# arnab39/equiadapt

Hardware: AMD Instinct MI355X
Metric: canonicalize+invert images/sec (224x224 C8) (higher is better)
Workload: dtype f32 (resampling / FFT / accumulation in fp32; the network's channel contraction as 2xfp16 split of every fp32 operand (within one fp32 ulp), 3 exact products, fp32 accumulate -- closer to fp64 than the fp32 matrix instruction, see step_ms_by_gemm_form); 1 GPU; configs[1]: 224x224x3 synthetic, C8, GroupEquivariantImageCanonicalization + ESCNNEquivariantNetwork in e2cnn's LAYER SHAPES (32 fields x 8 = 256 ch, k5, 3 layers, crop 0.8, resize 96) with this repository's own filter-bank parameterisation (bilinear-rotated banks; e2cnn's steerable basis is not restated -- e2cnn-trained weights enter via load_exported_dense), forward, then invert_canonicalization; batch_per_gpu=256, global_batch=256, parallelism=dp1 (no collective in the forward path)

## Files before the change

### equiadapt_amd/_lib.py

```python
import ctypes
import os
import subprocess
import threading

_HERE = os.path.dirname(os.path.abspath(__file__))
ROOT = os.path.dirname(_HERE)
CSRC = os.path.join(_HERE, "csrc")
SO_PATH = os.environ.get("EQA_LIB") or os.path.join(CSRC, "libeqa_hip.so")
SOURCES = [os.path.join(CSRC, f) for f in ("group_action.hip", "crop_resize.hip", "nearest_action.hip", "pooling.hip", "batchnorm.hip", "winograd.hip", "lift_conv.hip", "lift_conv_wide.hip", "lift_wgrad.hip", "pointcloud.hip", "vnsmall_fwd.hip", "nbody_frame.hip", "vnsmall_train.hip", "vnsmall_tail.hip", "fftconv.hip", "fft_filter.hip", "lift_fft.hip", "cgemm3m.hip", "cgemm3m_bf16.hip", "cgemm3m_c16.hip", "smallconv.hip", "planegemm.hip", "convnet_train.hip", "fourier_act.hip", "field_norm.hip", "nbody.hip", "vn_act.hip", "gconv1x1.hip", "steer_lift.hip")]
HEADERS = [os.path.join(CSRC, "eqa_common.hpp"), os.path.join(CSRC, "vn_common.hpp"), os.path.join(CSRC, "fourier_field.hpp"), os.path.join(CSRC, "fft48.inc"), os.path.join(CSRC, "fft_common.inc"), os.path.join(CSRC, "cgemm3m_common.inc")]
INCLUDE = os.path.join(ROOT, "include")

ABI_VERSION = 3

_c_f = ctypes.POINTER(ctypes.c_float)
_c_i = ctypes.POINTER(ctypes.c_int32)
_vp = ctypes.c_void_p
_int = ctypes.c_int

SIGNATURES = {
    "eqa_abi_version": (_int, []),
    "eqa_set_option": (_int, [_int, _int]),
    "eqa_get_option": (_int, [_int]),
    "eqa_fold_edge_pad_workspace_bytes": (ctypes.c_int64, [_int] * 4),
    "eqa_fold_edge_pad": (_int, [_vp, _vp, _vp, _int, _int, _int, _int, _vp]),
    "eqa_canon_transform_fwd": (_int, [_vp, _vp, _vp, _vp, _vp] + [_int] * 6 + [_vp]),
    "eqa_invert_action_fwd": (_int, [_vp, _vp, _vp, _vp, _vp, _vp] + [_int] * 6 + [_vp]),
    "eqa_group_action_pair": (_int, [_vp] * 4 + [_int, _int] + [_vp] * 5 + [_int, _int, _vp] + [_int] * 4 + [_vp]),
    "eqa_orbit_expand_fwd": (_int, [_vp, _vp, _vp, _vp] + [_int] * 5 + [_vp]),
    "eqa_group_action_fwd": (_int, [_vp, _vp, _vp, _vp, _vp, _vp] + [_int] * 12 + [_vp]),
    "eqa_group_action_fwd_hint": (_int, [_vp, _vp, _vp, _vp, _vp, _vp] + [_int] * 13 + [_vp]),
    "eqa_crop_resize_aa": (_int, [_vp] * 6 + [_int] * 9 + [_vp]),
    "eqa_mask_action_nearest": (_int, [_vp] * 5 + [_int] * 4 + [_vp]),
    "eqa_mask_action_nearest_planes": (_int, [_vp] * 5 + [_int] * 4 + [_vp]),
    "eqa_boxes_action": (_int, [_vp] * 5 + [_int, ctypes.c_float, _int, _vp]),
    "eqa_image_action_nearest": (_int, [_vp] * 5 + [_int] * 10 + [_vp]),
    "eqa_group_action_bwd_tiles": (_int, [_int, _int]),
    "eqa_group_action_bwd": (_int, [_vp] * 8 + [_int] * 12 + [_vp]),
    "eqa_group_action_bwd_theta": (_int, [_vp] * 8 + [_int] * 12 + [_vp]),
    "eqa_group_pool_workspace_bytes": (ctypes.c_int64, [_int] * 4),
    "eqa_group_pool_argmax": (_int, [_vp, _vp, _vp, _vp] + [_int] * 4 + [_vp]),
    "eqa_window_sums": (_int, [_vp, _vp, _vp, _int, _vp] + [_int] * 5 + [_vp]),
    "eqa_bn_partial_blocks": (ctypes.c_int64, [ctypes.c_int64]),
    "eqa_bn_stats_nhwc": (_int, [_vp, _vp, ctypes.c_int64, _int, _vp]),
    "eqa_bn_relu_dropout_nhwc": (_int, [_vp, _vp, _vp, _vp, ctypes.c_int64, _int, ctypes.c_float, ctypes.c_uint32, _vp]),
    "eqa_bn_bwd_reduce_nhwc": (_int, [_vp] * 5 + [ctypes.c_float, _vp, ctypes.c_int64, _int, _vp, _vp, ctypes.c_uint32, _vp]),
    "eqa_bn_bwd_apply_nhwc": (_int, [_vp] * 8 + [ctypes.c_float, _vp, ctypes.c_int64, _int, _vp, _vp, ctypes.c_uint32, _vp]),
    "eqa_window_sums_nhwc_act": (_int, [_vp, _vp, _vp, _int, ctypes.c_float, ctypes.c_uint32, _vp, _vp] + [_int] * 5 + [_vp]),
    "eqa_bn_bwd_reduce_nhwc_wsgrad": (_int, [_vp] * 4 + [ctypes.c_float, _vp] + [_int] * 5 + [_vp, _vp, ctypes.c_uint32, _vp]),
    "eqa_bn_bwd_apply_nhwc_wsgrad": (_int, [_vp] * 7 + [ctypes.c_float, _vp] + [_int] * 5 + [_vp, _vp, ctypes.c_uint32, _vp]),
    "eqa_vn_blocks": (_int, [_int]),
    "eqa_vn_knn": (_int, [_vp, _vp, _int, _int, _int, _vp]),
    "eqa_vn_convpos_stats": (_int, [_vp, _vp, _vp, _vp, _int, _int, _int, _vp]),
    "eqa_vn_convpos_fwd": (_int, [_vp] * 7 + [_int, _int, _int, _vp]),
    "eqa_vn_convpos_bwd_reduce": (_int, [_vp] * 10 + [_int, _int, _int, _vp]),
    "eqa_vn_convpos_bwd_apply": (_int, [_vp] * 12 + [_int, _int, _int, _vp]),
    "eqa_vn_convpos_max_fwd": (_int, [_vp] * 9 + [_int, _int, _int, _vp]),
    "eqa_vn_convpos_max_bwd_reduce": (_int, [_vp] * 11 + [_int, _int, _int, _vp]),
    "eqa_vn_convpos_max_bwd_apply": (_int, [_vp] * 13 + [_int, _int, _int, _vp]),
    "eqa_vn_tail_blocks": (_int, [_int]),
    "eqa_vn_tail_partial_floats": (_int, [_int]),
    "eqa_vn_tail_pass": (_int, [_int] + [_vp] * 8 + [_int, _int, _vp]),
    "eqa_vn_bn_finalize": (_int, [_vp, _int, _int, _int, ctypes.c_int64] + [_vp] * 5 + [ctypes.c_float, ctypes.c_float, _vp, _vp]),
    "eqa_vn_bn_bwd_finalize": (_int, [_vp, _int, _int, _int, ctypes.c_int64, _vp, _vp, _vp]),
    "eqa_window_grad_table": (_int, [_vp, _vp] + [_int] * 5 + [_vp]),
    "eqa_window_sums_gemv_bwd_workspace_bytes": (ctypes.c_int64, [_int, _int]),
    "eqa_window_sums_gemv_bwd": (_int, [_vp] * 6 + [_int, _int, _int, ctypes.c_double, _vp]),
    "eqa_window_sums_gemv": (_int, [_vp, _vp, _vp, _int, _int, _int, ctypes.c_double, ctypes.c_double, _vp]),
    "eqa_lift_conv_nhwc": (_int, [_vp, _vp, _vp, _int, _vp] + [_int] * 7 + [_vp]),
    "eqa_lift_conv_grouped": (_int, [_vp, _vp, _vp, _int, _vp] + [_int] * 7 + [_vp]),
    "eqa_lift_conv_stats_rows": (_int, [_int] * 7),
    "eqa_lift_conv_nhwc_stats": (_int, [_vp, _vp, _vp, _vp] + [_int] * 7 + [_vp]),
    "eqa_lift_conv_wgrad_supported": (_int, [_int] * 7),
    "eqa_lift_conv_wgrad_workspace_bytes": (ctypes.c_int64, [_int] * 7),
    "eqa_lift_conv_wgrad_nhwc": (_int, [_vp, _vp, _vp, _vp] + [_int] * 7 + [_vp]),
    "eqa_plane_gemm_supported": (_int, [_int, _int]),
    "eqa_plane_gemm": (_int, [_vp, _vp, _vp, ctypes.c_longlong, _int, _int, _int, _vp]),
    "eqa_winograd_f2k5_input": (_int, [_vp, _vp, _vp, _int, _int, _int, _int, _int, _vp]),
    "eqa_winograd_f2k5_output": (_int, [_vp, _vp, _int, _vp, _int, _int, _int, _int, _vp]),
    "eqa_winograd_f4k5_input": (_int, [_vp, _vp, _vp, _int, _int, _int, _int, _int, _vp]),
    "eqa_winograd_f4k5_output": (_int, [_vp, _vp, _int, _vp, _int, _int, _int, _int, _vp]),
    "eqa_winograd_f2k5_input_padded": (_int, [_vp, _vp, _int, _int, _int, _int, _int, _vp]),
    "eqa_winograd_f4k5_input_padded": (_int, [_vp, _vp, _int, _int, _int, _int, _int, _vp]),
    "eqa_winograd_f2k5_output_adjoint": (_int, [_vp, _vp, _int, _int, _int, _int, _vp]),
    "eqa_winograd_f4k5_output_adjoint": (_int, [_vp, _vp, _int, _int, _int, _int, _vp]),
# ... 30 lines not shown
    "eqa_fft48k5_filter_spectra3m_c16": (_int, [_vp, _vp, _int, _int, _int, _vp]),
    "eqa_fft48_filter_spectra3m_c16": (_int, [_vp, _vp, _int, _int, _int, _int, _vp]),
    "eqa_fft48_cgemm3m_c16": (_int, [_vp, _vp, _vp, ctypes.c_int64, _int, _int, _vp]),
    "eqa_fft48_wgrad3m_c16_supported": (_int, [_int, _int]),
    "eqa_fft48_wgrad3m_c16": (_int, [_vp, _vp, _vp, ctypes.c_int64, _int, _int, _vp]),
    "eqa_fft48k5_group": (_int, [_int, _int]),
    "eqa_fft48k5_workspace_bytes": (ctypes.c_int64, [_int] * 4),
    "eqa_fft48k5_input": (_int, [_vp, _vp, _vp, _vp] + [_int] * 5 + [_vp]),
    "eqa_fft48k5_input_grouped": (_int, [_vp, _vp, _vp, _vp] + [_int] * 5 + [_vp]),
    "eqa_fft48k5_input_grouped_supported": (_int, [_int]),
    "eqa_lift5_fft48k5_input_supported": (_int, [_int] * 4),
    "eqa_lift5_fft48k5_input": (_int, [_vp, _vp, _vp, _int, _vp] + [_int] * 4 + [_vp]),
    "eqa_lift5_fft48k5_input_dcmax": (_int, [_vp, _vp, _vp, _int, _vp, _vp] + [_int] * 4 + [_vp]),
    "eqa_lift5_pieces_f16_bytes": (ctypes.c_int64, [_int]),
    "eqa_absmax_slots": (_int, [_vp, ctypes.c_int64, _vp, _vp]),
    "eqa_lift5_fft48k5_input_f16x2": (_int, [_vp, _vp, ctypes.c_float, _vp, _int, _vp, _int, _vp, _vp] + [_int] * 4 + [_vp]),
    "eqa_lift5_pieces_bytes": (ctypes.c_int64, [_int]),
    "eqa_lift5_fft48k5_input_bf16x3": (_int, [_vp, _vp, _vp, _int, _vp] + [_int] * 4 + [_vp]),
    "eqa_fft48k5_output": (_int, [_vp, _vp, _vp, _int, _vp] + [_int] * 4 + [_vp]),
    "eqa_fft48k5_output_stats_rows": (ctypes.c_int64, [_int] * 4),
    "eqa_fft48k5_output_stats": (_int, [_vp, _vp, _vp, _vp] + [_int] * 4 + [_vp]),
    "eqa_fft48k5_output_sums": (_int, [_vp, _vp, _vp, _int, _vp, _vp] + [_int] * 5 + [_vp]),
    "eqa_fft48_supported": (_int, [_int]),
    "eqa_fft48_tiles": (ctypes.c_int64, [_int, _int]),
    "eqa_fft48_workspace_bytes": (ctypes.c_int64, [_int] * 5),
    "eqa_fft48_filter_spectra": (_int, [_vp, _vp, _int, _int, _int, _int, _vp]),
    "eqa_fft48_filter_spectra3m": (_int, [_vp, _vp, _int, _int, _int, _int, _vp]),
    "eqa_fft48_input": (_int, [_vp, _vp, _vp, _vp] + [_int] * 6 + [_vp]),
    "eqa_fft48_grad_transform": (_int, [_vp, _vp, _vp] + [_int] * 5 + [_vp]),
    "eqa_fft48_output": (_int, [_vp, _vp, _vp, _int, _vp] + [_int] * 5 + [_vp]),
    "eqa_fft48_input_grad": (_int, [_vp, _vp, _vp] + [_int] * 5 + [_vp]),
    "eqa_fft48_filter_grad": (_int, [_vp, _vp, _int, _int, _int, _int, _vp]),
    "eqa_conv_s2_supported": (_int, [_int] * 5),
    "eqa_conv_s2": (_int, [_vp, _vp, _vp, _int, _vp] + [_int] * 8 + [_vp]),
    "eqa_conv_s2_wgrad_supported": (_int, [_int] * 5),
    "eqa_conv_s2_wgrad_workspace_bytes": (ctypes.c_int64, [_int] * 8),
    "eqa_conv_s2_wgrad": (_int, [_vp] * 4 + [_int] * 8 + [_vp]),
    "eqa_conv_s2_dgrad_supported": (_int, [_int] * 4),
    "eqa_conv_s2_dgrad": (_int, [_vp] * 3 + [_int] * 7 + [_vp]),
    "eqa_bn_act_fwd": (_int, [_vp] * 5 + [ctypes.c_int64, _int, _int, _vp]),
    "eqa_bn_act_partial_blocks": (ctypes.c_int64, [ctypes.c_int64]),
    "eqa_bn_act_stats": (_int, [_vp, _vp, ctypes.c_int64, _int, _vp]),
    "eqa_bn_act_finalize": (_int, [_vp, ctypes.c_int64, _int, _vp, _vp, ctypes.c_double, ctypes.c_double] + [_vp] * 6 + [_vp]),
    "eqa_bn_act_bwd_finalize": (_int, [_vp, ctypes.c_int64, _int] + [_vp] * 7 + [_vp]),
    "eqa_bn_act_bwd_reduce": (_int, [_vp] * 8 + [ctypes.c_int64, _int, _int, _vp]),
    "eqa_bn_act_bwd_apply": (_int, [_vp] * 11 + [ctypes.c_int64, _int, _int, _vp]),
    "eqa_affine_relu_rows": (_int, [_vp, _vp, _vp, _vp, ctypes.c_int64, _int, _vp]),
    "eqa_cosine_group_activations": (_int, [_vp, _vp, _vp, _int, _int, _int, ctypes.c_float, _vp]),
    "eqa_bias_relu_nhwc": (_int, [_vp, _vp, ctypes.c_int64, _int, _vp]),
    "eqa_window_sums_nhwc_workspace_bytes": (ctypes.c_int64, [_int] * 4),
    "eqa_window_sums_nhwc": (_int, [_vp, _vp, _vp, _int, _vp, _vp] + [_int] * 5 + [_vp]),
    "eqa_window_sums_bwd_expand_nhwc": (_int, [_vp, _vp] + [_int] * 5 + [_vp]),
    "eqa_group_argmax": (_int, [_vp, _vp, _int, _int, _vp]),
    "eqa_vnsmall_workspace_bytes": (ctypes.c_int64, [_int, _int]),
    "eqa_vnsmall_fwd": (_int, [_vp, _vp, _vp, _vp, _int, _int, _int, _int, _vp]),
    "eqa_vnsmall_canonicalize": (_int, [_vp] * 6 + [_int] * 4 + [_vp]),
    "eqa_so3_rotate": (_int, [_vp, _vp, _vp, _int, _int, _int, _vp]),
    "eqa_gram_schmidt": (_int, [_vp, _vp, _int, _vp]),
    "eqa_gram_schmidt_bwd": (_int, [_vp, _vp, _vp, _int, _vp]),
    "eqa_modified_gram_schmidt": (_int, [_vp, _vp, _int, _vp]),
    "eqa_rigid_rows": (_int, [_vp, _vp, _vp, _vp, _int, _int, _vp]),
    "eqa_nbody_frame_fwd": (_int, [_vp] * 7 + [_int, _vp]),
    "eqa_nbody_frame_bwd": (_int, [_vp] * 12 + [_int, _vp]),
    "eqa_rigid_rows_bwd": (_int, [_vp] * 5 + [_int, _vp]),
    "eqa_fourier_elu_fwd": (_int, [_vp, _vp, _vp, _vp, ctypes.c_longlong, _int, _vp]),
    "eqa_fourier_elu_bwd": (_int, [_vp, _vp, _vp, _vp, _vp, ctypes.c_longlong, _int, _vp]),
    "eqa_field_norm_max_fields": (_int, []),
    "eqa_field_norm_blocks": (ctypes.c_longlong, [ctypes.c_longlong, _int]),
    "eqa_field_norm_stats": (_int, [_vp, _vp, ctypes.c_longlong, _int, _vp]),
    "eqa_field_norm_elu_bwd_reduce": (_int, [_vp] * 5 + [ctypes.c_longlong, _int, _vp]),
    "eqa_field_norm_elu_bwd_apply": (_int, [_vp] * 6 + [ctypes.c_longlong, _int, _vp]),
    "eqa_vndeepsets_param_count": (_int, [_int] * 3),
    "eqa_vndeepsets_bwd_blocks": (_int, [_int]),
    "eqa_nbody_adjacency": (_int, [_vp, _vp, ctypes.c_longlong, _int, _vp, _vp, _vp]),
    "eqa_vndeepsets_fwd": (_int, [_vp] * 7 + [_int] * 5 + [ctypes.c_float] + [_int] * 3 + [_vp]),
    "eqa_vndeepsets_train_fwd": (_int, [_vp] * 9 + [_int] * 5 + [ctypes.c_float] + [_int] * 3 + [_vp]),
    "eqa_vndeepsets_bwd": (_int, [_vp] * 10 + [_int] * 5 + [ctypes.c_float] + [_int] * 3 + [_vp]),
    "eqa_vn_act_max_channels": (_int, []),
    "eqa_vn_act_bwd_blocks": (_int, [ctypes.c_longlong]),
    "eqa_vn_act_fwd": (_int, [_vp] * 3 + [_int, _int, ctypes.c_longlong, _int, _int, ctypes.c_float, _vp]),
    "eqa_vn_act_bwd": (_int, [_vp] * 5 + [_int, _int, ctypes.c_longlong, _int, _int, ctypes.c_float, _vp]),
    "eqa_gconv1x1_supported": (_int, [ctypes.c_longlong, _int, _int]),
    "eqa_gconv1x1_nhwc": (_int, [_vp] * 6 + [_int, _vp, ctypes.c_longlong, _int, _int, _vp]),
    "eqa_gconv1x1_wgrad_supported": (_int, [ctypes.c_longlong, _int, _int]),
    "eqa_gconv1x1_wgrad_workspace_bytes": (ctypes.c_longlong, [ctypes.c_longlong, _int, _int]),
    "eqa_gconv1x1_wgrad": (_int, [_vp] * 5 + [ctypes.c_longlong, _int, _int, _vp]),
    "eqa_steer_lift_supported": (_int, [_int] * 3),
    "eqa_steer_lift_packed_floats": (ctypes.c_int64, [_int] * 3),
    "eqa_steer_lift_stat_rows": (ctypes.c_longlong, [_int]),
    "eqa_steer_lift_fwd": (_int, [_vp] * 4 + [_int] * 6 + [_vp]),
    "eqa_steer_lift_wgrad_workspace_bytes": (ctypes.c_int64, [_int] * 3),
    "eqa_steer_lift_wgrad": (_int, [_vp] * 4 + [_int] * 6 + [_vp]),
}

_lock = threading.Lock()
_lib = None


def source_hash(*names: str) -> str:
    import hashlib

    h = hashlib.sha1()
    for path in [os.path.join(CSRC, n) for n in names] + HEADERS:
        with open(path, "rb") as f:
            h.update(f.read())
    return h.hexdigest()[:16]
# ... 128 lines not shown
```

### equiadapt_amd/csrc/crop_resize.hip

```cpp
#include "eqa_common.hpp"

namespace {

constexpr int kAaBand = 8;
#ifndef EQA_AA_WIDE_MIN_K
#define EQA_AA_WIDE_MIN_K 8
#endif
constexpr int kAaMaxK = 20;

__global__ __launch_bounds__(kThreads) void crop_resize_aa_kernel(const float* __restrict__ x, float* __restrict__ y,
                                                                 const float* __restrict__ wx, const int32_t* __restrict__ x0,
                                                                 const float* __restrict__ wy, const int32_t* __restrict__ y0,
                                                                 int H, int W, int OH, int OW, int K, int max_rows) {
  extern __shared__ __attribute__((aligned(16))) float aa_tmp[];
  const int plane = blockIdx.y;
  const int r0 = blockIdx.x * kAaBand, r1 = min(r0 + kAaBand, OH);
  const int ybeg = y0[r0];
  const int yend = min(y0[r1 - 1] + K, H);
  const int nrows = min(yend - ybeg, max_rows);
  const float* src = x + (size_t)plane * H * W;
  const int rows_par = kThreads / OW;
  if (rows_par >= 1) {
    const int ox = threadIdx.x % OW, rsub = threadIdx.x / OW;
    if (rsub < rows_par) {
// ... 278 lines not shown
  auto wload = [&](int yc) {
    const int t = ybeg + yc + wq - ys_w;
    const bool ok = wr < nr_out && t >= 0 && t < K && yc + wq < span;
    return ok ? wy[(size_t)(r0 + wr) * K + min(max(t, 0), K - 1)] : 0.0f;
  };
  auto add8 = [&](const float4 (&v)[kAaStreamRows], float wv) {
#pragma unroll
    for (int q = 0; q < kAaStreamRows; ++q) {
#pragma unroll
      for (int r = 0; r < kAaBand; ++r) {
        const float w = __builtin_bit_cast(float, __builtin_amdgcn_readlane(__builtin_bit_cast(int, wv), 8 * q + r));
        acc[r].x += w * v[q].x; acc[r].y += w * v[q].y; acc[r].z += w * v[q].z; acc[r].w += w * v[q].w;
      }
    }
  };
  static_assert(kAaStreamRows == 8 && kAaBand == 8, "one weight per lane: 8 rows of a trip x 8 output rows = 64 lanes");
  float4 va[kAaStreamRows], vb[kAaStreamRows];
  float wa, wb = 0.0f;
  load8(va, 0);
  wa = wload(0);
  for (int yc = 0; yc < span; yc += 2 * kAaStreamRows) {
    if (yc + kAaStreamRows < span) { load8(vb, yc + kAaStreamRows); wb = wload(yc + kAaStreamRows); }
    add8(va, wa);
    if (yc + 2 * kAaStreamRows < span) { load8(va, yc + 2 * kAaStreamRows); wa = wload(yc + 2 * kAaStreamRows); }
    if (yc + kAaStreamRows < span) add8(vb, wb);
  }
  float* dst = y + (size_t)plane * OH * OW;
#pragma unroll
  for (int half = 0; half < 2; ++half) {
    if (e < xlen) {
#pragma unroll
      for (int rr = 0; rr < kAaBand / 2; ++rr) {
        float* lrow = aa_rows + rr * row_stride;
        const float4 v = acc[half * (kAaBand / 2) + rr];
        lrow[pos(e)] = v.x; lrow[pos(e + 1)] = v.y; lrow[pos(e + 2)] = v.z; lrow[pos(e + 3)] = v.w;
      }
    }
    __syncthreads();
    for (int idx = threadIdx.x; idx < (kAaBand / 2) * OW; idx += kThreads) {
      const int rr = idx / OW, ox = idx - rr * OW;
      const int r = half * (kAaBand / 2) + rr;
      if (r < nr_out) {
        const float* row = aa_rows + rr * row_stride;
        const int xs = x0[ox] - xbeg;
        float a = 0.0f;
        for (int j = 0; j < K; ++j) a += wx[ox * K + j] * row[pos(min(xs + j, xlen - 1))];
        dst[(size_t)(r0 + r) * OW + ox] = a;
      }
    }
    __syncthreads();
  }
}

}

extern "C" {

int eqa_crop_resize_aa(const float* x, float* y, const float* wx, const int32_t* x0, const float* wy, const int32_t* y0,
                       int planes, int H, int W, int OH, int OW, int K, int max_rows, int x_begin, int x_span, void* stream) {
  if (!x || !y || !wx || !x0 || !wy || !y0 || planes < 0 || H <= 0 || W <= 0 || OH <= 0 || OW <= 0 || K <= 0 || max_rows <= 0)
    return EQA_ERR_INVALID_ARG;
  const size_t lds = (size_t)max_rows * OW * sizeof(float);
  if (lds > 96 * 1024 || planes > 65535) return EQA_ERR_UNSUPPORTED;
  if (planes == 0) return EQA_OK;
  const dim3 grid((OH + kAaBand - 1) / kAaBand, planes);
  if (K > EQA_AA_WIDE_MIN_K && x_span > 0 && x_begin >= 0 && x_begin + x_span <= W) {
    const int stride = (x_span + OW / 2) / OW;
    const int pad_shift = (stride >= 2 && (stride & 1) == 0) ? __builtin_ctz((unsigned)stride) : 0;
    const int row_stride = x_span + (pad_shift ? (x_span >> pad_shift) : 0) + 1;
    const size_t row_bytes = (size_t)row_stride * sizeof(float);
    const int rpi = (int)std::min<size_t>(8, lds + row_bytes <= 96 * 1024 ? (96 * 1024 - lds) / row_bytes : 0);
    const size_t lds2 = lds + (size_t)rpi * row_bytes;
    static const bool stream_off = [] { const char* e = getenv("EQA_AA_STREAM"); return e && e[0] == '0'; }();
    if (!stream_off && x_span <= 4 * kThreads && (x_span & 3) == 0 && (x_begin & 3) == 0 && (W & 3) == 0 && (((uintptr_t)x) & 15) == 0 &&
        (size_t)(kAaBand / 2) * row_bytes <= 64 * 1024) {
      hipLaunchKernelGGL(crop_resize_aa_stream_kernel, grid, dim3(kThreads), (kAaBand / 2) * row_bytes, (hipStream_t)stream, x, y, wx, x0, wy,
                         y0, H, W, OH, OW, K, x_begin, x_span, pad_shift, row_stride);
      return launch_status();
    }
    if (rpi >= 1) {
      hipLaunchKernelGGL(crop_resize_aa_wide_kernel, grid, dim3(kThreads), lds2, (hipStream_t)stream, x, y, wx, x0, wy, y0, H, W, OH,
                         OW, K, max_rows, x_begin, x_span, pad_shift, row_stride, rpi);
      return launch_status();
    }
  }
  static const bool staged_off = [] { const char* e = getenv("EQA_AA_STAGED"); return e && e[0] == '0'; }();
  if (!staged_off && K <= EQA_AA_WIDE_MIN_K && (W & 3) == 0 && (((uintptr_t)x) & 15) == 0 && x_span > 0 && x_begin >= 0 &&
      x_begin + x_span <= W) {
    const int xb = x_begin & ~3, xl = std::min(W, (x_begin + x_span + 3) & ~3) - xb;
    static const int band_env = [] { const char* e = getenv("EQA_AA_BAND"); return e ? atoi(e) : 0; }();
    int band = band_env == 16 ? 16 : (band_env == 8 ? 8 : (OH >= 64 ? 16 : 8));
    auto staged_lds = [&](int bnd) { return ((size_t)(bnd / kAaBand) * max_rows * (xl + OW) + bnd * (EQA_AA_WIDE_MIN_K + 1)) * sizeof(float); };
    if (band == 16 && band_env != 16 && (staged_lds(16) > 64 * 1024 || 16 * K > kThreads)) band = 8;
    const int cap_rows = (band / kAaBand) * max_rows;
    const size_t lds3 = staged_lds(band);
    if (lds3 <= 64 * 1024 && band * K <= kThreads) {
      static const int per_cu = [] { const char* e = getenv("EQA_AA_BLOCKS_PER_CU"); return e ? std::max(1, atoi(e)) : 12; }();
      const int nbands = (OH + band - 1) / band;
      const int groups = std::max(1, (std::min(planes, (256 * per_cu + nbands - 1) / nbands) + kXcd - 1) / kXcd);
      const bool few = cap_rows <= 20;
#define EQA_AA_STAGED(K_)                                                                                                              \
  case K_:                                                                                                                             \
    if (band == 16)                                                                                                                    \
      hipLaunchKernelGGL((crop_resize_aa_staged_kernel<K_, 16, 10>), dim3(kXcd, nbands, groups), dim3(kThreads), lds3, (hipStream_t)stream, x, \
                         y, wx, x0, wy, y0, planes, H, W, OH, OW, cap_rows, xb, xl);                                                   \
    else if (few)                                                                                                                      \
      hipLaunchKernelGGL((crop_resize_aa_staged_kernel<K_, 8, 5>), dim3(kXcd, nbands, groups), dim3(kThreads), lds3, (hipStream_t)stream, x,  \
                         y, wx, x0, wy, y0, planes, H, W, OH, OW, cap_rows, xb, xl);                                                   \
    else                                                                                                                               \
// ... 19 lines not shown
```

### equiadapt_amd/csrc/fftconv.hip

```cpp
#include <cstdlib>

#include "eqa_common.hpp"

namespace {

#include "fft_common.inc"

typedef float f32x2 __attribute__((ext_vector_type(2)));
__device__ __forceinline__ void fft_ldg2(const float2* p, float& re, float& im) {
  const f32x2 v = __builtin_nontemporal_load(reinterpret_cast<const f32x2*>(p));
  re = v[0];
  im = v[1];
}

__device__ __forceinline__ void fft_load_column(const float2* __restrict__ p, size_t fpitch, bool edge, float (&re)[kFftN],
                                                float (&im)[kFftN]) {
#pragma unroll
  for (int ky = 0; ky < kFftH; ++ky) fft_ldg2(p + ky * fpitch, re[ky], im[ky]);
  const float2* base2 = edge ? p + (size_t)(kFftH - 2) * fpitch : p + (size_t)kFftH * fpitch;
  const ptrdiff_t step2 = edge ? -(ptrdiff_t)fpitch : (ptrdiff_t)fpitch;
  const unsigned flip = edge ? 0x80000000u : 0u;
#pragma unroll
  for (int ky = kFftH; ky < kFftN; ++ky) {
    fft_ldg2(base2 + (ky - kFftH) * step2, re[ky], im[ky]);
// ... 974 lines not shown

int eqa_fft48k5_input_grouped_supported(int C) { return C > 0 && C % kFusCh == 0 && !fft_two_pass(); }

int eqa_fft48k5_input_grouped(const float* x, float* T, float* V, const float* in_bias, int in_relu, int nimg, int H, int W, int C,
                              void* stream) {
  if (!fft_input_args_ok(x, T, V, nimg, H, W, C, 5)) return EQA_ERR_INVALID_ARG;
  if (!eqa_fft48k5_input_grouped_supported(C)) return EQA_ERR_UNSUPPORTED;
  if (nimg == 0) return EQA_OK;
  FftFwdOpts opt;
  opt.x_grouped = 1;
  opt.may_pipe = true;
  return FftK<5>::forward(x, T, V, in_bias, in_relu, nimg, H, W, C, fft_tiles_k(H, 5), fft_tiles_k(W, 5), kFftN, (hipStream_t)stream, opt);
}

int eqa_fft48k5_grad_transform(const float* dy, float* T, float* G, int nimg, int OH, int OW, int C, void* stream) {
  if (!fft_map_args_ok(dy, T, G, nimg, OH, OW, C)) return EQA_ERR_INVALID_ARG;
  if (nimg == 0) return EQA_OK;
  return FftK<5>::forward(dy, T, G, nullptr, 0, nimg, OH, OW, C, fft_ntiles(OH, kFftO), fft_ntiles(OW, kFftO), kFftO, (hipStream_t)stream);
}

int eqa_fft48k5_input_grad(const float* Cg, float* T2, float* dx, int nimg, int H, int W, int C, void* stream) {
  if (!fft_input_args_ok(Cg, T2, dx, nimg, H, W, C, 5)) return EQA_ERR_INVALID_ARG;
  if (nimg == 0) return EQA_OK;
  return FftK<5>::input_grad(Cg, T2, dx, nimg, H, W, C, (hipStream_t)stream);
}

int eqa_fft48k5_output(const float* Mo, float* T2, const float* bias, int relu, float* y, int nimg, int OH, int OW, int C,
                       void* stream) {
  if (!fft_map_args_ok(Mo, T2, y, nimg, OH, OW, C)) return EQA_ERR_INVALID_ARG;
  if (nimg == 0) return EQA_OK;
  FftInvOpts opt;
  opt.may_pipe = true;
  return FftK<5>::output<0>(Mo, T2, bias, relu, y, nimg, OH, OW, C, (hipStream_t)stream, opt);
}

int64_t eqa_fft48k5_output_stats_rows(int nimg, int OH, int OW, int C) {
  if (nimg <= 0 || OH <= 0 || OW <= 0 || C <= 0) return 0;
  int64_t rows = 0;
  FftInvOpts opt;
  opt.may_pipe = true;
  opt.stats_rows = &rows;
  return FftK<5>::output<0>(nullptr, nullptr, nullptr, 0, nullptr, nimg, OH, OW, C, nullptr, opt) == EQA_OK ? rows : 0;
}

int eqa_fft48k5_output_stats(const float* Mo, float* T2, float* y, double* partial, int nimg, int OH, int OW, int C, void* stream) {
  if (!fft_map_args_ok(Mo, T2, y, nimg, OH, OW, C) || !partial) return EQA_ERR_INVALID_ARG;
  if (nimg == 0) return EQA_OK;
  FftInvOpts opt;
  opt.may_pipe = true;
  opt.stats = partial;
  return FftK<5>::output<0>(Mo, T2, nullptr, 0, y, nimg, OH, OW, C, (hipStream_t)stream, opt);
}

int eqa_fft48k5_output_sums(const float* Mo, float* T2, const float* bias, int relu, double* S, void* workspace, int nimg,
                            int OH, int OW, int C, int k_next, void* stream) {
  if (!fft_map_args_ok(Mo, T2, S, nimg, OH, OW, C) || !workspace || k_next <= 0) return EQA_ERR_INVALID_ARG;
  const int nb = k_next - 1;
  if ((nb != 4 && nb != 2) || OH < 2 * nb + 1 || OW < 2 * nb + 1 || k_next > kMaxWinK || nimg > 65535) return EQA_ERR_UNSUPPORTED;
  if (nimg == 0) return EQA_OK;
  hipStream_t st = (hipStream_t)stream;
  float* part = (float*)workspace;
  int form = 0;
  FftInvOpts opt;
  opt.may_pipe = true;
  opt.form = &form;
  const int rc = nb == 4 ? FftK<5>::output<4>(Mo, T2, bias, relu, part, nimg, OH, OW, C, st, opt)
                         : FftK<5>::output<2>(Mo, T2, bias, relu, part, nimg, OH, OW, C, st, opt);
  if (rc != EQA_OK) return rc;
  const int sub = form ? fft_ntiles(OW, kFftO) : 1;
  const int per_row = form == 3 ? kPipeCons / 64 : form;
  const int nseg = form ? 2 * nb + per_row * fft_ntiles(OH, kFftO) : OH;
  return eqa::launch_window_sums_nhwc_finalize(part, S, nimg, C, k_next, nseg * sub, st, sub);
}

int eqa_fft48_supported(int ksize) { return fft_ksize_ok(ksize) ? 1 : 0; }

int64_t eqa_fft48_tiles(int n, int ksize) { return fft_ksize_ok(ksize) ? fft_tiles_k(n, ksize) : 0; }

int64_t eqa_fft48_workspace_bytes(int nimg, int rows, int cols, int C, int ksize) {
  if (nimg <= 0 || rows <= 0 || cols <= 0 || C <= 0 || !fft_ksize_ok(ksize)) return 0;
  return fft_workspace_bytes(nimg, rows, cols, C, kFftN + 1 - ksize);
}

int eqa_fft48_input(const float* x, float* T, float* V, const float* in_bias, int in_relu, int nimg, int H, int W, int C, int ksize,
                    void* stream) {
  if (!fft_input_args_ok(x, T, V, nimg, H, W, C, ksize)) return EQA_ERR_INVALID_ARG;
  if (nimg == 0) return EQA_OK;
  EQA_FFT_K(ksize, FftK, K_::forward(x, T, V, in_bias, in_relu, nimg, H, W, C, fft_tiles_k(H, ksize), fft_tiles_k(W, ksize), kFftN,
                                     (hipStream_t)stream));
}

int eqa_fft48_grad_transform(const float* dy, float* T, float* G, int nimg, int OH, int OW, int C, int ksize, void* stream) {
  if (!fft_map_args_ok(dy, T, G, nimg, OH, OW, C) || !fft_ksize_ok(ksize)) return EQA_ERR_INVALID_ARG;
  if (nimg == 0) return EQA_OK;
  EQA_FFT_K(ksize, FftK, K_::forward(dy, T, G, nullptr, 0, nimg, OH, OW, C, fft_ntiles(OH, K_::O), fft_ntiles(OW, K_::O), K_::O,
                                     (hipStream_t)stream));
}

int eqa_fft48_output(const float* Mo, float* T2, const float* bias, int relu, float* y, int nimg, int OH, int OW, int C, int ksize,
                     void* stream) {
  if (!fft_map_args_ok(Mo, T2, y, nimg, OH, OW, C) || !fft_ksize_ok(ksize)) return EQA_ERR_INVALID_ARG;
  if (nimg == 0) return EQA_OK;
  EQA_FFT_K(ksize, FftK, K_::template output<0>(Mo, T2, bias, relu, y, nimg, OH, OW, C, (hipStream_t)stream));
}

int eqa_fft48_input_grad(const float* Cg, float* T2, float* dx, int nimg, int H, int W, int C, int ksize, void* stream) {
  if (!fft_input_args_ok(Cg, T2, dx, nimg, H, W, C, ksize)) return EQA_ERR_INVALID_ARG;
  if (nimg == 0) return EQA_OK;
  EQA_FFT_K(ksize, FftK, K_::input_grad(Cg, T2, dx, nimg, H, W, C, (hipStream_t)stream));
}

}
```

### equiadapt_amd/csrc/pooling.hip

```cpp
#include "eqa_common.hpp"

namespace {


constexpr int kPoolSplitTarget = 2048;


template <bool VEC>
__global__ __launch_bounds__(kThreads) void group_pool_partial_kernel(const float* __restrict__ feat,
                                                                     double* __restrict__ partial, int Cf, int G,
                                                                     int HW, int cps, int splits) {
  extern __shared__ __attribute__((aligned(16))) double acc[];
  const int s = blockIdx.x, b = blockIdx.y;
  const int tid = threadIdx.x, lane = tid & 63, wave = tid >> 6;
  for (int k = tid; k < 4 * G; k += kThreads) acc[k] = 0.0;
  __syncthreads();
  const int c_lo = s * cps, c_hi = min(c_lo + cps, Cf);
  const int planes = (c_hi - c_lo) * G;
  const float* base = feat + ((size_t)b * Cf + c_lo) * G * HW;
  for (int p = wave; p < planes; p += 4) {
    const float* pl = base + (size_t)p * HW;
    float v0 = 0.f, v1 = 0.f, v2 = 0.f, v3 = 0.f;
    if (VEC) {
      const float4* p4 = reinterpret_cast<const float4*>(pl);
      const int n4 = HW >> 2;
      for (int k = lane; k < n4; k += 64) {
        const float4 t = p4[k];
        v0 += t.x; v1 += t.y; v2 += t.z; v3 += t.w;
      }
    } else {
      for (int k = lane; k < HW; k += 64) v0 += pl[k];
    }
    const float tot = wave_sum_f((v0 + v1) + (v2 + v3));
    if (lane == 0) acc[wave * G + (p % G)] += (double)tot;
  }
  __syncthreads();
  if (tid < G) partial[((size_t)b * splits + s) * G + tid] = (acc[tid] + acc[G + tid]) + (acc[2 * G + tid] + acc[3 * G + tid]);
}

__device__ __forceinline__ void wave_argmax_store(float v, int g, int G, int32_t* out) {
  int idx = (g < G) ? g : 0x7fffffff;
  float val = (g < G) ? v : -INFINITY;
  bool isn = (g < G) && (v != v);
#pragma unroll
  for (int o = 32; o > 0; o >>= 1) {
    const float ov = __shfl_xor(val, o, 64);
    const int oi = __shfl_xor(idx, o, 64);
    const bool on = __shfl_xor((int)isn, o, 64) != 0;
    bool take;
    if (on != isn) take = on;
    else if (on) take = oi < idx;
    else take = (ov > val) || (ov == val && oi < idx);
    if (take) { val = ov; idx = oi; isn = on; }
  }
  if (g == 0) *out = idx;
}

__global__ __launch_bounds__(kThreads) void group_pool_finalize_kernel(const double* __restrict__ partial,
                                                                      float* __restrict__ act,
                                                                      int32_t* __restrict__ gidx, int B, int G,
                                                                      int splits, double inv_count) {
  const int wave = threadIdx.x >> 6, lane = threadIdx.x & 63;
  const int b = blockIdx.x * 4 + wave;
  if (b >= B) return;
  for (int g0 = 0; g0 < G; g0 += 64) {
    const int g = g0 + lane;
    float a = 0.f;
    if (g < G) {
      double sum = 0.0;
      for (int s = 0; s < splits; ++s) sum += partial[((size_t)b * splits + s) * G + g];
      a = (float)(sum * inv_count);
      act[(size_t)b * G + g] = a;
    }
    if (G <= 64 && gidx) wave_argmax_store(a, g, G, gidx + b);
  }
}

__global__ __launch_bounds__(kThreads) void group_argmax_kernel(const float* __restrict__ act, int32_t* __restrict__ gidx,
                                                               int B, int G) {
  const int wave = threadIdx.x >> 6, lane = threadIdx.x & 63;
  const int b = blockIdx.x * 4 + wave;
  if (b >= B) return;
  const float a = lane < G ? act[(size_t)b * G + lane] : 0.f;
  wave_argmax_store(a, lane, G, gidx + b);
}

int pool_splits(int B, int Cf) {
  int s = (kPoolSplitTarget + B - 1) / B;
  if (s > Cf) s = Cf;
  if (s < 1) s = 1;
  return s;
}


template <bool VEC>
__global__ __launch_bounds__(kThreads) void window_sums_kernel(const float* __restrict__ x, const float* __restrict__ scale,
                                                              const float* __restrict__ shift, int relu,
                                                              double* __restrict__ out, int C, int H, int W, int k) {
  extern __shared__ __attribute__((aligned(16))) float ws_smem[];
  const int HW = H * W;
  float* sp = ws_smem;
  double* cs = reinterpret_cast<double*>(ws_smem + ((HW + 3) & ~3));
  const int plane = blockIdx.x;
  const int c = plane % C;
  const float sc = scale ? scale[c] : 1.0f, sh = shift ? shift[c] : 0.0f;
  const float* p = x + (size_t)plane * HW;
  const int tid = threadIdx.x;
// ... 143 lines not shown
        t1.x += c3.x; t1.y += c3.y; t1.z += c3.z; t1.w += c3.w;
      }
      for (; xc + xs < W; xc += 2 * xs) {
        const ws_f4 r0 = raw(y, xc), r1 = raw(y, xc + xs);
        const float4 a = act(r0, y, xc), c2 = act(r1, y, xc + xs);
        t0.x += a.x; t0.y += a.y; t0.z += a.z; t0.w += a.w;
        t1.x += c2.x; t1.y += c2.y; t1.z += c2.z; t1.w += c2.w;
      }
      if (xc < W) { const float4 a = ld(y, xc); t0.x += a.x; t0.y += a.y; t0.z += a.z; t0.w += a.w; }
      acc[0].x += t0.x + t1.x; acc[0].y += t0.y + t1.y; acc[0].z += t0.z + t1.z; acc[0].w += t0.w + t1.w;
#pragma unroll
      for (int j = 0; j < MAXB; ++j) {
        if (j < nb && psub == 0) {
          if ((j & 3) == wave) { const float4 a = ld(y, j); acc[1 + j].x += a.x; acc[1 + j].y += a.y; acc[1 + j].z += a.z; acc[1 + j].w += a.w; }
          const int xr = W - nb + j;
          if ((xr & 3) == wave) {
            const float4 a = ld(y, xr);
            acc[1 + MAXB + j].x += a.x; acc[1 + MAXB + j].y += a.y;
            acc[1 + MAXB + j].z += a.z; acc[1 + MAXB + j].w += a.w;
          }
        }
      }
    }
    auto put = [&](int i, const float4& v) {
      float* o = part + ((((size_t)b * nseg + s) * Q + q) * 4) * nval + i;
      o[0] = v.x; o[nval] = v.y; o[2 * nval] = v.z; o[3 * nval] = v.w;
    };
    if (P > 1) {
      for (int off = 32; off >= Q; off >>= 1) {
        acc[0].x += __shfl_down(acc[0].x, off); acc[0].y += __shfl_down(acc[0].y, off);
        acc[0].z += __shfl_down(acc[0].z, off); acc[0].w += __shfl_down(acc[0].w, off);
      }
    }
    const bool owner = on && psub == 0;
    __syncthreads();
    s_tot[wave][lane] = acc[0];
#pragma unroll
    for (int j = 0; j < MAXB; ++j) {
      if (j < nb && owner) {
        if ((j & 3) == wave) put(1 + j, acc[1 + j]);
        if (((W - nb + j) & 3) == wave) put(1 + nb + j, acc[1 + MAXB + j]);
      }
    }
    __syncthreads();
    if (wave == 0 && owner) {
      const float4 a = s_tot[0][lane], b2 = s_tot[1][lane], c2 = s_tot[2][lane], d = s_tot[3][lane];
      put(0, make_float4((a.x + b2.x) + (c2.x + d.x), (a.y + b2.y) + (c2.y + d.y), (a.z + b2.z) + (c2.z + d.z), (a.w + b2.w) + (c2.w + d.w)));
    }
  }
}

constexpr int kFinThreads = 320;

template <int KW, int MAXB = kWsSmallBorder>
__global__ __launch_bounds__(kFinThreads) void window_sums_nhwc_finalize_kernel(const float* __restrict__ part, double* __restrict__ out,
                                                                            int B, int C, int k_rt, int nseg, int sub) {
  constexpr int kFinVals = 1 + 2 * MAXB;
  const int k = KW ? KW : k_rt;
  __shared__ double s_tot[kFinCh * kFinVals];
  __shared__ float s_brd[2 * MAXB][kFinCh * kFinVals];
  const int b = blockIdx.y;
  const int c0 = blockIdx.x * kFinCh;
  const int nch = min(kFinCh, C - c0);
  const int nb = k - 1, nval = 1 + 2 * nb;
  const int run = nch * nval;
  const float* base = part + ((size_t)b * nseg * C + c0) * nval;
  const size_t seg_stride = (size_t)C * nval;
  for (int e = threadIdx.x; e < run; e += blockDim.x) {
    const float* q = base + e;
    double acc = 0.0;
    int s = 0;
    if (sub <= 2) {
      float v[2 * MAXB][2];
#pragma unroll
      for (int i = 0; i < 2 * MAXB; ++i)
#pragma unroll
        for (int t = 0; t < 2; ++t) v[i][t] = (i < 2 * nb && t < sub) ? q[(size_t)(i * sub + t) * seg_stride] : 0.0f;
#pragma unroll
      for (int i = 0; i < 2 * MAXB; ++i) {
        if (i < 2 * nb) {
          const float w = sub == 2 ? v[i][0] + v[i][1] : v[i][0];
          s_brd[i][e] = w;
          acc += (double)w;
        }
      }
      s = 2 * nb;
    } else {
      for (; s < 2 * nb; ++s) {
        float v = q[(size_t)(s * sub) * seg_stride];
        for (int t = 1; t < sub; ++t) v += q[(size_t)(s * sub + t) * seg_stride];
        s_brd[s][e] = v;
        acc += (double)v;
      }
    }
    s *= sub;
    for (; s + 8 <= nseg; s += 8) {
      float v[8];
#pragma unroll
      for (int j = 0; j < 8; ++j) v[j] = q[(size_t)(s + j) * seg_stride];
#pragma unroll
      for (int j = 0; j < 8; ++j) acc += (double)v[j];
    }
    if (s < nseg) {
      float v[8];
#pragma unroll
      for (int j = 0; j < 8; ++j) v[j] = s + j < nseg ? q[(size_t)(s + j) * seg_stride] : 0.0f;
#pragma unroll
      for (int j = 0; j < 8; ++j)
        if (s + j < nseg) acc += (double)v[j];
    }
    s_tot[e] = acc;
  }
  __syncthreads();
  const int kk = k * k;
#ifdef EQA_FIN_NOPHASE2
  if (threadIdx.x < nch * kk && s_tot[0] == 12345.0) out[0] = 1.0;
  if (true) return;
#endif
  for (int it = threadIdx.x; it < nch * kk; it += blockDim.x) {
    const int cl = it / kk, uv = it - cl * kk;
    const int u = uv / k, v = uv - u * k;
    if constexpr (KW > 0) {
      constexpr int NB = KW - 1;
      float p0[NB], pc[NB][NB];
      double tc[NB];
#pragma unroll
      for (int r = 0; r < NB; ++r) p0[r] = s_brd[r < u ? r : NB + r][cl * nval];
#pragma unroll
      for (int j = 0; j < NB; ++j) {
        const int i = j < v ? 1 + j : 1 + NB + j;
        tc[j] = s_tot[cl * nval + i];
#pragma unroll
        for (int r = 0; r < NB; ++r) pc[j][r] = s_brd[r < u ? r : NB + r][cl * nval + i];
      }
      double a = s_tot[cl * nval];
#pragma unroll
      for (int r = 0; r < NB; ++r) a -= (double)p0[r];
#pragma unroll
      for (int j = 0; j < NB; ++j) {
        a -= tc[j];
#pragma unroll
        for (int r = 0; r < NB; ++r) a += (double)pc[j][r];
      }
      out[((size_t)b * C + c0) * kk + it] = a;
    } else {
      auto P = [&](int s, int i) { return (double)s_brd[s][cl * nval + i]; };
      double a = s_tot[cl * nval];
      for (int r = 0; r < nb; ++r) a -= r < u ? P(r, 0) : P(nb + r, 0);
      for (int j = 0; j < nb; ++j) {
        const int i = j < v ? 1 + j : 1 + nb + j;
        a -= s_tot[cl * nval + i];
        for (int r = 0; r < nb; ++r) a += r < u ? P(r, i) : P(nb + r, i);
      }
      out[((size_t)b * C + c0) * kk + it] = a;
    }
  }
}

constexpr int kGemvMaxE = 16;

template <int THREADS, int EMAX, int COLS>
__global__ __launch_bounds__(THREADS) void sums_gemv_kernel(const double* __restrict__ S, const double* __restrict__ Wm,
                                                            float* __restrict__ act, int K, int E, double scale, double shift) {
  __shared__ double s_red[THREADS / 64][kGemvMaxE];
  const int b = blockIdx.x;
  const double* sb = S + (size_t)b * K;
  double acc[kGemvMaxE];
#pragma unroll
  for (int e = 0; e < kGemvMaxE; ++e) acc[e] = 0.0;
  for (int j = threadIdx.x; j < K; j += COLS * THREADS) {
    double s[COLS], w[COLS][EMAX];
#pragma unroll
    for (int u = 0; u < COLS; ++u) {
      const bool in = j + u * THREADS < K;
      s[u] = in ? sb[j + u * THREADS] : 0.0;
#pragma unroll
      for (int e = 0; e < EMAX; ++e) w[u][e] = (in && e < E) ? Wm[(size_t)e * K + j + u * THREADS] : 0.0;
    }
#pragma unroll
    for (int u = 0; u < COLS; ++u)
#pragma unroll
      for (int e = 0; e < EMAX; ++e)
        if (e < E && j + u * THREADS < K) acc[e] += s[u] * w[u][e];
  }
  const int lane = threadIdx.x & 63, wave = threadIdx.x >> 6;
#pragma unroll
  for (int e = 0; e < kGemvMaxE; ++e) {
    double v = acc[e];
#pragma unroll
    for (int off = 32; off > 0; off >>= 1) v += __shfl_down(v, off, 64);
    if (lane == 0) s_red[wave][e] = v;
  }
  __syncthreads();
  if (threadIdx.x < E) {
    double v = 0.0;
    for (int w = 0; w < THREADS / 64; ++w) v += s_red[w][threadIdx.x];
    act[(size_t)b * E + threadIdx.x] = (float)(v * scale + shift);
  }
}


__global__ __launch_bounds__(kThreads) void affine_relu_rows_kernel(const float* __restrict__ h, const float* __restrict__ scale,
                                                                   const float* __restrict__ shift, float* __restrict__ z, size_t n_vec,
                                                                   int Dq) {
  const size_t i0 = (size_t)blockIdx.x * kThreads + threadIdx.x, stride = (size_t)gridDim.x * kThreads;
  QuadWalk w(i0, stride, Dq);
  for (size_t i = i0; i < n_vec; i += stride, w.next()) {
    const int q = (int)w.q;
    const float4 v = reinterpret_cast<const float4*>(h)[i];
    const float4 sc = reinterpret_cast<const float4*>(scale)[q], sh = reinterpret_cast<const float4*>(shift)[q];
    reinterpret_cast<float4*>(z)[i] = make_float4(fmaxf(v.x * sc.x + sh.x, 0.f), fmaxf(v.y * sc.y + sh.y, 0.f),
                                                  fmaxf(v.z * sc.z + sh.z, 0.f), fmaxf(v.w * sc.w + sh.w, 0.f));
  }
}

__global__ __launch_bounds__(kThreads) void cosine_group_activations_kernel(const float* __restrict__ v, const float* __restrict__ ref,
                                                                           float* __restrict__ act, int B, int G, int V, float eps) {
  const int lane = threadIdx.x & 63;
  const int r = blockIdx.x * (kThreads / 64) + (threadIdx.x >> 6);
  if (r >= G * B) return;
  float rr = 0.f, vv = 0.f;
  for (int k = lane; k < V; k += 64) {
    const float a = ref[k], x = v[(size_t)r * V + k];
    rr += a * a;
    vv += x * x;
  }
  rr = wave_sum_f(rr);
  vv = wave_sum_f(vv);
  const float inv_r = 1.0f / fmaxf(sqrtf(rr), eps), inv_v = 1.0f / fmaxf(sqrtf(vv), eps);
  float dot = 0.f;
  for (int k = lane; k < V; k += 64) dot += (ref[k] * inv_r) * (v[(size_t)r * V + k] * inv_v);
  dot = wave_sum_f(dot);
  if (lane == 0) act[(size_t)(r % B) * G + r / B] = dot;
}

}

int eqa::launch_window_sums_nhwc_finalize(const float* part, double* S, int B, int C, int k, int nseg, hipStream_t stream, int sub) {
  if (B > 65535) return EQA_ERR_UNSUPPORTED;
  const dim3 fgrid((C + kFinCh - 1) / kFinCh, B);
  const dim3 fblock(std::min(C, kFinCh) * (2 * k - 1) > kThreads ? kFinThreads : kThreads);
  if (k == 5)
    hipLaunchKernelGGL(window_sums_nhwc_finalize_kernel<5>, fgrid, fblock, 0, stream, part, S, B, C, k, nseg, sub);
  else if (k == 3)
    hipLaunchKernelGGL(window_sums_nhwc_finalize_kernel<3>, fgrid, fblock, 0, stream, part, S, B, C, k, nseg, sub);
  else if (k - 1 <= kWsSmallBorder)
    hipLaunchKernelGGL(window_sums_nhwc_finalize_kernel<0>, fgrid, fblock, 0, stream, part, S, B, C, k, nseg, sub);
  else
    hipLaunchKernelGGL((window_sums_nhwc_finalize_kernel<0, kWsMaxBorder>), fgrid, fblock, 0, stream, part, S, B, C, k, nseg, sub);
  return launch_status();
}

namespace {
// ... 106 lines not shown
  if (vec)
    hipLaunchKernelGGL((group_pool_partial_kernel<true>), dim3(used, B), dim3(kThreads), lds, st, feat, partial, Cf, G, HW, cps, used);
  else
    hipLaunchKernelGGL((group_pool_partial_kernel<false>), dim3(used, B), dim3(kThreads), lds, st, feat, partial, Cf, G, HW, cps, used);
  if (hipGetLastError() != hipSuccess) return EQA_ERR_LAUNCH;
  const double inv_count = 1.0 / ((double)Cf * (double)HW);
  hipLaunchKernelGGL(group_pool_finalize_kernel, dim3((B + 3) / 4), dim3(kThreads), 0, st, partial, act, gidx, B, G, used, inv_count);
  return launch_status();
}

int eqa_group_argmax(const float* act, int32_t* gidx, int B, int G, void* stream) {
  if (B == 0 && G > 0 && G <= 64) return EQA_OK;
  if (!act || !gidx || B < 0 || G <= 0) return EQA_ERR_INVALID_ARG;
  if (G > 64) return EQA_ERR_UNSUPPORTED;
  hipLaunchKernelGGL(group_argmax_kernel, dim3((B + 3) / 4), dim3(kThreads), 0, (hipStream_t)stream, act, gidx, B, G);
  return launch_status();
}

int eqa_window_sums(const float* x, const float* scale, const float* shift, int relu, double* out, int B, int C, int H,
                    int W, int k, void* stream) {
  if (!x || !out || B < 0 || C <= 0 || H <= 0 || W <= 0 || k <= 0 || k > H || k > W) return EQA_ERR_INVALID_ARG;
  if (k > kMaxWinK) return EQA_ERR_UNSUPPORTED;
  const size_t lds = (size_t)((H * W + 3) & ~3) * sizeof(float) + (size_t)k * W * sizeof(double);
  if (lds > 64 * 1024 || (long long)B * C > 0x7fffffffLL) return EQA_ERR_UNSUPPORTED;
  if (B == 0) return EQA_OK;
  const bool vec = ((H * W) % 4 == 0) && (((uintptr_t)x & 15) == 0);
  hipStream_t st = (hipStream_t)stream;
  if (vec)
    hipLaunchKernelGGL((window_sums_kernel<true>), dim3((unsigned)(B * C)), dim3(kThreads), lds, st, x, scale, shift, relu, out, C, H, W, k);
  else
    hipLaunchKernelGGL((window_sums_kernel<false>), dim3((unsigned)(B * C)), dim3(kThreads), lds, st, x, scale, shift, relu, out, C, H, W, k);
  return launch_status();
}

int eqa_window_sums_gemv(const double* S, const double* Wm, float* act, int B, int K, int E, double scale, double shift,
                         void* stream) {
  if (B < 0 || K <= 0 || E <= 0) return EQA_ERR_INVALID_ARG;
  if (B == 0) return EQA_OK;
  if (!S || !Wm || !act) return EQA_ERR_INVALID_ARG;
  if (E > kGemvMaxE) return EQA_ERR_UNSUPPORTED;
  const int per_thread = (K + kThreads - 1) / kThreads;
  if (E <= 8 && per_thread > 5)
    hipLaunchKernelGGL((sums_gemv_kernel<kThreads, 8, 9>), dim3(B), dim3(kThreads), 0, (hipStream_t)stream, S, Wm, act, K, E, scale, shift);
  else if (E <= 8 && per_thread > 2)
    hipLaunchKernelGGL((sums_gemv_kernel<kThreads, 8, 5>), dim3(B), dim3(kThreads), 0, (hipStream_t)stream, S, Wm, act, K, E, scale, shift);
  else if (E <= 8)
    hipLaunchKernelGGL((sums_gemv_kernel<kThreads, 8, 2>), dim3(B), dim3(kThreads), 0, (hipStream_t)stream, S, Wm, act, K, E, scale, shift);
  else
    hipLaunchKernelGGL((sums_gemv_kernel<kThreads, kGemvMaxE, 5>), dim3(B), dim3(kThreads), 0, (hipStream_t)stream, S, Wm, act, K, E, scale,
                       shift);
  return launch_status();
}

int eqa_affine_relu_rows(const float* h, const float* scale, const float* shift, float* z, int64_t rows, int D, void* stream) {
  if (!h || !scale || !shift || !z || rows < 0 || D <= 0) return EQA_ERR_INVALID_ARG;
  if (D % 4 != 0 || (((uintptr_t)h | (uintptr_t)z | (uintptr_t)scale | (uintptr_t)shift) & 15)) return EQA_ERR_UNSUPPORTED;
  if (rows == 0) return EQA_OK;
  const size_t n_vec = (size_t)rows * (D / 4);
  const unsigned blocks = (unsigned)std::min<size_t>((n_vec + kThreads - 1) / kThreads, 8192);
  hipLaunchKernelGGL(affine_relu_rows_kernel, dim3(blocks), dim3(kThreads), 0, (hipStream_t)stream, h, scale, shift, z, n_vec, D / 4);
  return launch_status();
}

int eqa_cosine_group_activations(const float* v, const float* ref, float* act, int B, int G, int V, float eps, void* stream) {
  if (!v || !ref || !act || B < 0 || G <= 0 || V <= 0) return EQA_ERR_INVALID_ARG;
  if (B == 0) return EQA_OK;
  if ((int64_t)B * G > 0x7fffffff) return EQA_ERR_UNSUPPORTED;
  const int rows = B * G, per = kThreads / 64;
  hipLaunchKernelGGL(cosine_group_activations_kernel, dim3((rows + per - 1) / per), dim3(kThreads), 0, (hipStream_t)stream, v, ref, act, B,
                     G, V, eps);
  return launch_status();
}

int eqa_bias_relu_nhwc(float* x, const float* bias, int64_t n_pixels, int C, void* stream) {
  if (!x || !bias || n_pixels < 0 || C <= 0) return EQA_ERR_INVALID_ARG;
  if (C % 4 != 0 || (((uintptr_t)x | (uintptr_t)bias) & 15)) return EQA_ERR_UNSUPPORTED;
  if (n_pixels == 0) return EQA_OK;
  const size_t n_vec = (size_t)n_pixels * (C / 4);
  const unsigned blocks = (unsigned)((n_vec + kThreads - 1) / kThreads < 8192 ? (n_vec + kThreads - 1) / kThreads : 8192);
  hipLaunchKernelGGL(bias_relu_nhwc_kernel, dim3(blocks), dim3(kThreads), 0, (hipStream_t)stream, x, bias, n_vec, C / 4);
  return launch_status();
}

int eqa_window_sums_bwd_expand_nhwc(const float* table, float* dx, int B, int H, int W, int C, int k, void* stream) {
  if (!table || !dx || B < 0 || H <= 0 || W <= 0 || C <= 0 || k <= 0 || H < 2 * k - 1 || W < 2 * k - 1) return EQA_ERR_INVALID_ARG;
  if (C % 4 != 0 || (((uintptr_t)table | (uintptr_t)dx) & 15) || (size_t)B * H > 0x7fffffffULL) return EQA_ERR_UNSUPPORTED;
  if (B == 0) return EQA_OK;
  hipLaunchKernelGGL(window_sums_bwd_expand_kernel, dim3((unsigned)((size_t)B * H)), dim3(kThreads), 0, (hipStream_t)stream, table,
                     dx, H, W, C / 4, k - 1);
  return launch_status();
}

static int ws_nhwc_bands(int H, int k) {
  const int interior = H - 2 * (k - 1);
  int nb = (interior + 9) / 10;
  if (nb < 1) nb = 1;
  return nb;
}

int64_t eqa_window_sums_nhwc_workspace_bytes(int B, int C, int H, int k) {
  if (B <= 0 || C <= 0 || H <= 0 || k <= 0) return 0;
  const int nseg = 2 * (k - 1) + ws_nhwc_bands(H, k);
  return (int64_t)B * nseg * C * (1 + 2 * (k - 1)) * (int64_t)sizeof(float);
}

static int window_sums_nhwc_impl(const float* x, const float* scale, const float* shift, int relu, float drop_p, uint32_t seed, double* out,
// ... 88 lines not shown
```

### equiadapt_amd/images/canonicalization/discrete_group.py

```python
import math
from typing import Any, Dict, List, Optional, Tuple, Union

import torch
import torch.nn.functional as F

from equiadapt_amd import ops
from equiadapt_amd.common.basecanonicalization import DiscreteGroupCanonicalization
from equiadapt_amd.images import geometry
from equiadapt_amd.images.transforms import CenterCrop, EdgePad, Resize
from equiadapt_amd.images.utils import (
    canonicalize_masks,
    device_tables,
    canonicalize_boxes,
    flip_boxes,
    flip_masks,
    get_action_on_image_features,
    rotate_boxes,
    rotate_masks,
)



def _get(hyperparams: Any, name: str):
    if isinstance(hyperparams, dict):
        return hyperparams[name]
    return getattr(hyperparams, name)

class _CanonTransformFn(torch.autograd.Function):

    @staticmethod
    def forward(ctx, x, rotation, reflection, gidx, theta, flags, pad, num_rotations):
        ctx.save_for_backward(x, gidx, theta, flags if flags is not None else torch.empty(0))
        ctx.pad, ctx.num_rotations, ctx.has_flags = pad, num_rotations, flags is not None
        return ops.canon_transform(x, gidx, theta, flags, pad)

    @staticmethod
    def backward(ctx, grad_y):
        x, gidx, theta, flags = ctx.saved_tensors
        flags = flags if ctx.has_flags else None
        pad, N = ctx.pad, ctx.num_rotations
        need_x, need_rot, need_ref = ctx.needs_input_grad[0], ctx.needs_input_grad[1], ctx.needs_input_grad[2]
        grad_y = grad_y.contiguous()
        gx = g_rot = g_ref = None
        if need_x or need_rot:
            gx, g_ang = ops.group_action_bwd(x, grad_y, gidx, theta, flags, None, pad, (pad, pad), need_x, need_rot)
            if need_rot:
                g_rot = -g_ang
        if need_ref:
            ridx = gidx % N
            y0 = ops.canon_transform(x, ridx, theta, flags, pad)
            y1 = ops.canon_transform(x, ridx + N, theta, flags, pad)
            g_ref = (grad_y * (y1 - y0)).sum(dim=(1, 2, 3))
        return gx, g_rot, g_ref, None, None, None, None, None


class DiscreteGroupImageCanonicalization(DiscreteGroupCanonicalization):

    def __init__(self, canonicalization_network: torch.nn.Module, canonicalization_hyperparams: Any, in_shape: tuple):
        super().__init__(canonicalization_network)
        self.beta = _get(canonicalization_hyperparams, "beta")
        assert len(in_shape) == 3, "Input shape should be in the format (channels, height, width)"
        self.in_shape = tuple(int(s) for s in in_shape)
        is_grayscale = self.in_shape[0] == 1
        self.pad_size = 0 if is_grayscale else math.ceil(self.in_shape[-1] * 0.5)
        self.pad = torch.nn.Identity() if is_grayscale else EdgePad(self.pad_size)
        self.crop = torch.nn.Identity() if is_grayscale else CenterCrop((self.in_shape[-2], self.in_shape[-1]))
        self.crop_canonization = (
            torch.nn.Identity() if is_grayscale else CenterCrop((
                math.ceil(self.in_shape[-2] * _get(canonicalization_hyperparams, "input_crop_ratio")),
                math.ceil(self.in_shape[-1] * _get(canonicalization_hyperparams, "input_crop_ratio"))))
        )
        self.resize_canonization = (
            torch.nn.Identity() if is_grayscale else Resize(size=_as_size(_get(canonicalization_hyperparams, "resize_shape")))
        )
        self._consts: Dict[str, torch.Tensor] = {}


    def _group_constants(self, device: torch.device) -> Tuple[torch.Tensor, Optional[torch.Tensor]]:
        key = f"{device}:{self.num_rotations}:{self.group_type}"
        hit = self._consts.get(key)
        if hit is None:
            angles = geometry.group_angles(self.num_rotations)
            if self.group_type == "roto-reflection":
                rot = torch.cat([angles, angles], dim=0)
                ref = torch.cat([torch.zeros(self.num_rotations), torch.ones(self.num_rotations)], dim=0)
                hit = (rot.to(device), ref.to(device))
            else:
                hit = (angles.to(device), None)
            self._consts[key] = hit
        return hit

    def groupactivations_to_groupelement(self, group_activations: torch.Tensor,
                                         group_index: Optional[torch.Tensor] = None) -> dict:
        if group_index is None:
            group_index = self.group_index(group_activations)
        rot_comp, ref_comp = self._group_constants(group_activations.device)
        if not self.training and self.gradient_trick == "straight_through":
            element = {"rotation": torch.index_select(rot_comp, 0, group_index)}
            if ref_comp is not None:
                element["reflection"] = torch.index_select(ref_comp, 0, group_index)
            element["group_index"] = group_index
            return element
        onehot = self.groupactivations_to_groupelementonehot(group_activations, group_index)
        if self.gradient_trick != "straight_through":
            group_index = onehot.detach().argmax(dim=-1).to(torch.int32)
        element = {"rotation": torch.sum(onehot * rot_comp, dim=-1)}
        if ref_comp is not None:
            element["reflection"] = torch.sum(onehot * ref_comp, dim=-1)
        element["group_index"] = group_index
        return element

    def get_group_activations(self, x: torch.Tensor) -> torch.Tensor:
        raise NotImplementedError(
            "get_group_activations is not implemented for the DiscreteGroupImageCanonicalization class")

    def get_groupelement(self, x: torch.Tensor) -> Dict[str, torch.Tensor]:
        group_activations = self.get_group_activations(x)
        group_index = self.group_index(group_activations)
        element = self.groupactivations_to_groupelement(group_activations, group_index)
        if not hasattr(self, "canonicalization_info_dict"):
            self.canonicalization_info_dict = {}
        self.canonicalization_info_dict["group_index"] = element.pop("group_index")
        self.canonicalization_info_dict["argmax_index"] = group_index
        self.canonicalization_info_dict["group_element"] = element
        self.canonicalization_info_dict["group_activations"] = group_activations
        return element

    def transformations_before_canonicalization_network_forward(self, x: torch.Tensor) -> torch.Tensor:
        crop, resize = self.crop_canonization, self.resize_canonization
        if (x.is_cuda and x.dtype == torch.float32 and not (torch.is_grad_enabled() and x.requires_grad) and isinstance(resize, Resize)
                and resize.antialias):
            from equiadapt_amd.images.transforms import resized_output_size

            out_hw = resized_output_size(crop.size, resize.size)
            if tuple(out_hw) == tuple(x.shape[-2:]) == tuple(crop.size):
                return x
            key = (tuple(x.shape[-2:]), crop.size, out_hw, str(x.device))
            tabs = self._consts.get(key)
            if tabs is None:
                t = geometry.aa_resize_tables(tuple(x.shape[-2:]), crop.size, out_hw)
                tabs = tuple(v.to(x.device) if isinstance(v, torch.Tensor) else v for v in t)
                self._consts[key] = tabs
            return ops.crop_resize_aa(x, tabs, out_hw)
        return resize(crop(x))


    def canonicalize(self, x: torch.Tensor, targets: Optional[List] = None, **kwargs: Any
                     ) -> Union[torch.Tensor, Tuple[torch.Tensor, List]]:
        self.device = x.device
        element = self.get_groupelement(x)
        gidx = self.canonicalization_info_dict["group_index"]
        reflections = "reflection" in element
        H, W = x.shape[-2:]
        pad = self.pad_size
        theta, flags = device_tables("canonicalize", self.num_rotations, reflections, (H + 2 * pad, W + 2 * pad), x.device)
        x = _CanonTransformFn.apply(x, element["rotation"], element.get("reflection"), gidx, theta, flags, pad,
                                    self.num_rotations)

        if targets:
            image_width = x.shape[-1]
            box_list = [t_["boxes"] for t_ in targets]
            counts = [int(b.shape[0]) for b in box_list]
            if sum(counts) > 0 and all(b.is_cuda and b.dim() == 2 and b.shape[1] == 4 and b.dtype == torch.float32 for b in box_list) \
                    and element["rotation"].dtype == torch.float32:
                for t_, nb in zip(targets, canonicalize_boxes(box_list, element["rotation"].detach(), image_width, reflections)):
                    t_["boxes"] = nb
            else:
                if reflections:
                    for t in range(len(targets)):
                        targets[t]["boxes"] = flip_boxes(targets[t]["boxes"], image_width)
                for t in range(len(targets)):
                    targets[t]["boxes"] = rotate_boxes(targets[t]["boxes"], element["rotation"][t], image_width)
            masks = [t_["masks"] for t_ in targets]
            if all(m.is_cuda and m.dtype == torch.uint8 and m.dim() == 3 and m.shape[-2:] == masks[0].shape[-2:] for m in masks):
                new = canonicalize_masks(masks, gidx, self.num_rotations, flip_all=reflections)
                for t in range(len(targets)):
                    targets[t]["masks"] = new[t]
            else:
                rot_host = element["rotation"].detach().cpu()
                for t in range(len(targets)):
                    m = flip_masks(targets[t]["masks"]) if reflections else targets[t]["masks"]
                    targets[t]["masks"] = rotate_masks(m, -rot_host[t].item())
            return x, targets
        return x

    def invert_canonicalization(self, x_canonicalized_out: torch.Tensor, **kwargs: Any) -> torch.Tensor:
        induced_rep_type = kwargs.get("induced_rep_type", "regular")
        element = dict(self.canonicalization_info_dict["group_element"])
        element["group_index"] = self.canonicalization_info_dict["group_index"]
        return get_action_on_image_features(
            feature_map=x_canonicalized_out,
            group_info_dict=self.group_info_dict,
            group_element_dict=element,
            induced_rep_type=induced_rep_type,
        )


def _as_size(resize_shape: Any):
    if isinstance(resize_shape, int):
        return resize_shape
    return tuple(int(s) for s in resize_shape)


def _num_group(group_type: str, num_rotations: int) -> int:
    return num_rotations if group_type == "rotation" else 2 * num_rotations


class GroupEquivariantImageCanonicalization(DiscreteGroupImageCanonicalization):

    def __init__(self, canonicalization_network: torch.nn.Module, canonicalization_hyperparams: Any, in_shape: tuple):
        super().__init__(canonicalization_network, canonicalization_hyperparams, in_shape)
        self.group_type = canonicalization_network.group_type
        self.num_rotations = canonicalization_network.num_rotations
        self.num_group = _num_group(self.group_type, self.num_rotations)
        self.group_info_dict = {"num_rotations": self.num_rotations, "num_group": self.num_group}

    def get_group_activations(self, x: torch.Tensor) -> torch.Tensor:
        x = self.transformations_before_canonicalization_network_forward(x)
        return self.canonicalization_network(x)


class OptimizedGroupEquivariantImageCanonicalization(DiscreteGroupImageCanonicalization):

    def __init__(self, canonicalization_network: torch.nn.Module, canonicalization_hyperparams: Any, in_shape: tuple):
        super().__init__(canonicalization_network, canonicalization_hyperparams, in_shape)
        self.group_type = _get(canonicalization_hyperparams, "group_type")
        self.num_rotations = _get(canonicalization_hyperparams, "num_rotations")
        self.artifact_err_wt = _get(canonicalization_hyperparams, "artifact_err_wt")
        self.num_group = _num_group(self.group_type, self.num_rotations)
        self.out_vector_size = canonicalization_network.out_vector_size
        size = _get(canonicalization_hyperparams, "resize_shape")
        self.group_augment_size = int(size)
        gray = self.in_shape[0] == 1
        self.group_augment_pad = 0 if gray else math.ceil(self.group_augment_size * 0.5)
        self.crop_group_augment = torch.nn.Identity() if gray else CenterCrop(self.group_augment_size)
        self.pad_group_augment = torch.nn.Identity() if gray else EdgePad(self.group_augment_pad)
        self.reference_vector = torch.nn.Parameter(
            torch.randn(1, self.out_vector_size), requires_grad=_get(canonicalization_hyperparams, "learn_ref_vec"))
        self.group_info_dict = {"num_rotations": self.num_rotations, "num_group": self.num_group}

    def group_augment(self, x: torch.Tensor) -> torch.Tensor:
        s = x.shape[-1]
        pad = self.group_augment_pad
        theta, flags = device_tables("orbit", self.num_rotations, self.group_type == "roto-reflection",
                                     (s + 2 * pad, s + 2 * pad), x.device)
        return ops.orbit_expand(x, theta, flags, pad)

    def _rotate_batch(self, x: torch.Tensor, rot_index: torch.Tensor, sign: float) -> torch.Tensor:
        s = x.shape[-1]
        pad = self.group_augment_pad
        theta = geometry.rotation_theta(sign * geometry.group_angles(self.num_rotations) * 1.0, (s + 2 * pad, s + 2 * pad))
        return ops.group_action(x, rot_index.to(torch.int32), theta.to(x.device), None, None, pad, (s, s), (pad, pad))

    def get_group_activations(self, x: torch.Tensor) -> torch.Tensor:
        x = self.transformations_before_canonicalization_network_forward(x)
        x_augmented = self.group_augment(x)
        vector_out = self.canonicalization_network(x_augmented)
        self.canonicalization_info_dict = {"vector_out": vector_out}

        if self.artifact_err_wt:
            rot_idx = torch.randint(0, self.num_rotations, (x_augmented.shape[0],), device=x.device)
            x_dummy = self._rotate_batch(x_augmented, rot_idx, -1.0)
            x_dummy = self._rotate_batch(x_dummy, rot_idx, +1.0)
            vector_out_dummy = self.canonicalization_network(x_dummy)
            self.canonicalization_info_dict.update({"vector_out_dummy": vector_out_dummy})

        if vector_out.is_cuda and vector_out.dtype == torch.float32 and not torch.is_grad_enabled():
            return ops.cosine_group_activations(vector_out, self.reference_vector.detach(), self.num_group)
        scalar_out = F.cosine_similarity(self.reference_vector.repeat(vector_out.shape[0], 1), vector_out)
        return scalar_out.reshape(self.num_group, -1).T

    def get_optimization_specific_loss(self) -> torch.Tensor:
        vectors = self.canonicalization_info_dict["vector_out"]
        artifact = 0
        if self.artifact_err_wt:
# ... 6 lines not shown
```

### equiadapt_amd/images/canonicalization_networks/escnn_networks.py

```python
import os
from typing import List, Sequence

import torch
import torch.nn as nn
import torch.nn.functional as F

from equiadapt_amd.images.canonicalization_networks.custom_group_equivariant_layers import (
    RotationEquivariantConv,
    RotationEquivariantConvLift,
    RotoReflectionEquivariantConv,
    RotoReflectionEquivariantConvLift,
)
from equiadapt_amd import ops
from equiadapt_amd.common.derived import DerivedCache, bn_eval_affine, refuse_e2cnn_state_dict
from equiadapt_amd.common.utils import update_running_stats
from equiadapt_amd.images.canonicalization_networks import fftconv, winograd
from equiadapt_amd.images.canonicalization_networks.pooling import (
    WindowSumsFunction,
    WindowSumsLinearFn,
    conv_then_group_pool,
    group_pool,
    window_grad_table,
    window_sums_to_activations,
)
from equiadapt_amd.images.canonicalization_networks.steerable_networks import ESCNNSteerableNetwork


class _InnerBatchNorm(nn.BatchNorm3d):
    """Per-field batch norm over (batch, group, space) of a (B, fields, G, H, W) map."""


class LiftConvFunction(torch.autograd.Function):

    @staticmethod
    def forward(ctx, x, bank, with_stats=False):
        ctx.save_for_backward(x, bank)
        k = bank.shape[-1]
        if not ops.lift_conv_supported(bank.shape[1], bank.shape[-2], k, bank.shape[0]):
            if with_stats:
                raise ValueError("LiftConvFunction: with_stats needs a shape eqa_lift_conv_nhwc_stats takes (gate on ops.lift_conv_supported)")
            return ops.lift_conv_wide(x, ops.pack_lift_weights_wide(bank.detach()), None, False, bank.shape[-2], k)
        wpk = ops.pack_lift_weights(bank.detach())
        if with_stats:
            y, part = ops.lift_conv_nhwc_stats(x, wpk, bank.shape[-2], k)
            ctx.mark_non_differentiable(part)
            return y, part
        return ops.lift_conv_nhwc(x, wpk, None, False, bank.shape[-2], k)

    @staticmethod
    def backward(ctx, dy, *_):
        x, bank = ctx.saved_tensors
        dy = dy.contiguous(memory_format=torch.channels_last)
        dx = torch.nn.grad.conv2d_input(x.shape, bank, dy) if ctx.needs_input_grad[0] else None
        dbank = None
        if ctx.needs_input_grad[1]:
            kh, kw = bank.shape[-2], bank.shape[-1]
            if ops.lift_conv_wgrad_supported(x, bank.shape[0], kh, kw):
                dbank = ops.lift_conv_wgrad_nhwc(x, dy, kh, kw)
            elif ops.lift_conv_wide_supported(bank.shape[1], kh, kw, bank.shape[0]) and x.shape[0] > 0:
                dbank = ops.lift_conv_wide_wgrad(x, dy, kh, kw)
            else:
                dbank = torch.nn.grad.conv2d_weight(x, bank.shape, dy)
        return dx, dbank, None


def _moments(s1, s2, n, bn, conv_bias):
    mean = s1 / n
    var = (s2 / n - mean * mean).clamp_min(0.0)
    with torch.no_grad():
        full_mean = mean if conv_bias is None else mean + conv_bias.double()
        update_running_stats(bn, full_mean, var * (n / max(n - 1, 1)))
    return mean.float(), var.float()


# ... 100 lines not shown
        return self.conv.weight

    def mean_response_weights(self) -> torch.Tensor:
        w = self.conv.weight
        return self._cache.get("weff", (w,), lambda: w.detach().view(self.out_channels, self.num_group_elements, -1).double().sum(0))

    def mean_bias_value(self):
        b = self.conv.bias
        if b is None:
            return 0.0

        def build():
            m = b.detach().double().view(self.out_channels, self.num_group_elements).mean(0)
            return float(m[0].item()) if bool((m == m[0]).all().item()) else m

        return self._cache.get("bias_mean", (b,), build)

    def supports_linear_tail(self) -> bool:
        return self.stride == 1 and self.padding == 0 and self.kernel_size <= ops.MAX_WINDOW_K

    def forward(self, x: torch.Tensor) -> torch.Tensor:
        return self.conv(x)


class ESCNNEquivariantNetwork(nn.Module):
    def __init__(self, in_shape: tuple, out_channels: int, kernel_size: int, group_type: str = "rotation",
                 num_rotations: int = 4, num_layers: int = 1):
        super().__init__()
        self.in_channels = in_shape[0]
        self.out_channels = out_channels
        self.kernel_size = kernel_size
        self.group_type = group_type
        self.num_rotations = num_rotations
        if group_type == "rotation":
            lift, conv = RotationEquivariantConvLift, RotationEquivariantConv
        elif group_type == "roto-reflection":
            lift, conv = RotoReflectionEquivariantConvLift, RotoReflectionEquivariantConv
        else:
            raise ValueError("group_type must be rotation or roto-reflection for now.")
        self.num_group_elements = num_rotations if group_type == "rotation" else 2 * num_rotations

        def block() -> List[nn.Module]:
            return [_InnerBatchNorm(out_channels, momentum=0.9), nn.ReLU(inplace=True), nn.Dropout(p=0.5)]

        mods: List[nn.Module] = [lift(self.in_channels, out_channels, kernel_size, num_rotations, device="cpu")]
        mods += block()
        for _ in range(num_layers - 2):
            mods.append(conv(out_channels, out_channels, kernel_size, num_rotations, device="cpu"))
            mods += block()
        mods.append(conv(out_channels, out_channels, kernel_size, num_rotations, device="cpu"))
        self.eqv_network = nn.Sequential(*mods)
        self._dense: Sequence = ()
        self._cache = DerivedCache()

    def _load_from_state_dict(self, state_dict, prefix, *args, **kwargs):
        refuse_e2cnn_state_dict(
            state_dict, prefix + "eqv_network.", "ESCNNEquivariantNetwork",
            "equiadapt_amd.ESCNNEquivariantNetwork parameterises its layers by rotated filter banks and cannot load it by key; "
            "export the trained layers on the e2cnn side (R2Conv.export() -> nn.Conv2d, InnerBatchNorm.export() -> nn.BatchNorm2d) "
            "and pass them to load_exported_dense(convs, norms).", (".expanded_bias",))
        return super()._load_from_state_dict(state_dict, prefix, *args, **kwargs)

    def load_exported_dense(self, convs: Sequence[nn.Conv2d], norms: Sequence[nn.BatchNorm2d]) -> None:
        n_conv = sum(1 for m in self.eqv_network if hasattr(m, "expanded_weights"))
        if len(convs) != n_conv or len(norms) != n_conv - 1:
            raise ValueError(f"expected {n_conv} convs and {n_conv - 1} norms")
        E = self.num_group_elements
        cin = self.in_channels
        for i, cv in enumerate(convs):
            if cv.in_channels != cin:
                raise ValueError(f"exported conv {i} takes {cv.in_channels} channels, the network feeds it {cin}")
            cin = cv.out_channels
        for i, bn in enumerate(norms):
            if bn.num_features != convs[i].out_channels:
                raise ValueError(f"exported norm {i} has {bn.num_features} features, conv {i} produces {convs[i].out_channels}")
        self._dense = (nn.ModuleList(_DenseConv(cv, E, i == 0) for i, cv in enumerate(convs)), nn.ModuleList(norms))
        self._cache.clear()

    def export_dense(self):
        E = self.num_group_elements
        convs, norms = [], []
        with torch.no_grad():
            for m in self.eqv_network:
                if hasattr(m, "expanded_weights"):
                    bank = m.expanded_weights().detach()
                    cv = nn.Conv2d(bank.shape[1], bank.shape[0], m.kernel_size, m.stride, m.padding, bias=m.bias is not None)
                    cv = cv.to(bank.device)
                    cv.weight.copy_(bank)
                    if m.bias is not None:
                        cv.bias.copy_(m.bias.detach().repeat_interleave(E))
                    convs.append(cv)
                elif isinstance(m, _InnerBatchNorm):
                    bn = nn.BatchNorm2d(m.num_features * E, eps=m.eps, momentum=m.momentum).to(m.weight.device)
                    for name in ("weight", "bias", "running_mean", "running_var"):
                        getattr(bn, name).copy_(getattr(m, name).repeat_interleave(E))
                    norms.append(bn.eval())
        return convs, norms

    def _layers(self):
        if self._dense:
            return list(self._dense[0]), list(self._dense[1])
        mods = list(self.eqv_network)
        return [m for m in mods if hasattr(m, "expanded_weights")], [m for m in mods if isinstance(m, _InnerBatchNorm)]

    def _folded(self, conv, bn):
        def build():
# ... 7 lines not shown
            return bank.contiguous(memory_format=torch.channels_last), bias.contiguous()

        return self._cache.get(conv, (conv.weights, conv.bias, bn.weight, bn.bias, bn.running_mean, bn.running_var), build)

    @staticmethod
    def _plain_5x5(conv) -> bool:
        return not conv.lifting and conv.kernel_size == 5 and conv.stride == 1 and conv.padding == 0

    @staticmethod
    def _lift_kernel(conv, bank, h, narrow_unchecked: bool = False):
        if not conv.lifting or os.environ.get("EQA_LIFT_MFMA", "1") == "0":
            return None
        k, (cout, cin) = conv.kernel_size, bank.shape[:2]
        unit = conv.stride == 1 and conv.padding == 0
        if (unit or narrow_unchecked) and ops.lift_conv_supported(cin, k, k, cout):
            return "narrow"
        if (unit and h.is_contiguous(memory_format=torch.channels_last) and h.shape[-2] >= k and h.shape[-1] >= k
                and ops.lift_conv_wide_supported(cin, k, k, cout)):
            return "wide"
        return None

    def _route(self, i, h, bank, convs, nhwc):
        conv, tail = convs[i], convs[-1]
        cout, cin = bank.shape[:2]
        k, kt = conv.kernel_size, tail.kernel_size
        last_before_tail = i == len(convs) - 2
        if nhwc and self._plain_5x5(conv) and fftconv.applicable(h, cin, cout):
            return "fft5", (last_before_tail and kt in (3, 5) and tail.supports_linear_tail() and min(h.shape[-2:]) - 4 >= 2 * kt - 1), 0
        if (nhwc and not conv.lifting and k != 5 and conv.stride == 1 and conv.padding == 0
                and h.is_contiguous(memory_format=torch.channels_last) and fftconv.applicable_k(h.shape, cin, cout, k, h.device)):
            return "fftk", False, 0
        if nhwc and self._plain_5x5(conv) and winograd.applicable(h, cin, cout):
            m = winograd.tile_for(h)
            if last_before_tail and not winograd.sums_applicable(h, kt, m) and winograd.sums_applicable(h, kt, 2):
                m = 2
            return "wino", last_before_tail and winograd.sums_applicable(h, kt, m), m
        lift = self._lift_kernel(conv, bank, h) if nhwc else None
        if lift == "narrow":
            nxt = convs[i + 1] if i + 1 < len(convs) - 1 else None
            if nxt is not None and self._plain_5x5(nxt):
                if fftconv.lift_fused_applicable(h.shape, bank.shape, nxt.out_channels * nxt.num_group_elements, h.device):
                    return "lift_fused", False, 0
                if fftconv.grouped_applicable((h.shape[0], cout, h.shape[2] - k + 1, h.shape[3] - k + 1), cout, cout, h.device):
                    return "lift_grouped", False, 0
            return "lift", False, 0
        return ("lift_wide" if lift == "wide" else "lib"), False, 0

    def _forward_inference(self, x: torch.Tensor) -> torch.Tensor:
        convs, norms = self._layers()
        tail = convs[-1]
        nhwc = (self.out_channels * self.num_group_elements) % 4 == 0
        h = x.contiguous(memory_format=torch.channels_last) if nhwc else x
        pending = None
        for i, (conv, bn) in enumerate(zip(convs[:-1], norms)):
            bank, bias = self._folded(conv, bn)
            route, sums, m = self._route(i, h, bank, convs, nhwc)
            k, (H, W) = conv.kernel_size, h.shape[-2:]
            last_before_tail, shift = i == len(convs) - 2, None
            if route != "fft5" and isinstance(h, (fftconv.GroupedMap, fftconv.LiftedInput)):
                h = h.materialize()
            if route in ("fft5", "fftk", "wino"):
                in_bias, pending = pending, None
                sums_k = tail.kernel_size if sums else 0
                if route == "wino":
                    U = self._cache.derived(conv, (conv, "wino", m), lambda: winograd.transform_filters(bank, m))
                    h = winograd.conv5x5(h, U, bias, relu=True, in_bias=in_bias, in_relu=in_bias is not None, sums_k=sums_k)
                else:
                    Bf = self._cache.derived(conv, (conv, "fft"), lambda: fftconv.spectra_for_k(bank))
                    if route == "fft5":
                        h = fftconv.conv5x5(h, Bf, bias, True, in_bias, in_bias is not None, sums_k=sums_k)
                    else:
                        h = fftconv.conv_kxk(h, Bf, k, bias, True, in_bias, in_bias is not None)
            else:
                if pending is not None:
                    ops.bias_relu_nhwc_(h, pending)
                    pending = None
                if route == "lift_fused":
                    operand = {}
                    form = fftconv.LiftedInput.form_operand()
                    if form is not None:
                        operand[form[1]] = self._cache.derived(conv, (conv, form[0]), lambda: form[2](bank))
                    h = fftconv.LiftedInput(h, bank, bias, True, **operand)
                elif route != "lib":
                    pack = ops.pack_lift_weights_wide if route == "lift_wide" else ops.pack_lift_weights
                    wpk = self._cache.derived(conv, (conv, "lift"), lambda: pack(bank))
                    if route == "lift_grouped":
                        h = fftconv.GroupedMap(ops.lift_conv_grouped(h, wpk, bias, True, k, k))
                    else:
                        h = (ops.lift_conv_wide if route == "lift_wide" else ops.lift_conv_nhwc)(h, wpk, bias, True, k, k)
                else:
                    h = F.conv2d(h, bank)
                    if last_before_tail:
                        shift = bias
                    elif nhwc and h.is_contiguous(memory_format=torch.channels_last):
                        pending = bias
                    else:
                        h = torch.relu_(h + bias[None, :, None, None])
            if sums:
                return window_sums_to_activations(h, tail, H - k + 1, W - k + 1)
            if last_before_tail:
                return conv_then_group_pool(h, tail, shift=shift, relu=shift is not None)
        raise AssertionError("unreachable: the network always has at least two convolutions")

    @staticmethod
    def _inner_bn(h: torch.Tensor, bn: nn.BatchNorm3d, E: int, conv_bias) -> torch.Tensor:
        Bn, C, H, W = h.shape
        Fd = C // E
        if bn.training or bn.running_mean is None:
            s1 = h.sum(dim=(0, 2, 3), dtype=torch.float64).view(Fd, E).sum(1)
            s2 = (h * h).sum(dim=(0, 2, 3), dtype=torch.float64).view(Fd, E).sum(1)
            mean, var = _moments(s1, s2, Bn * E * H * W, bn, conv_bias)
        else:
            mean = bn.running_mean if conv_bias is None else bn.running_mean - conv_bias
            var = bn.running_var
        scale = bn.weight * torch.rsqrt(var + bn.eps)
        shift = bn.bias - mean * scale
        return h * scale.repeat_interleave(E)[None, :, None, None] + shift.repeat_interleave(E)[None, :, None, None]

    def _train_route(self, li, h, bank, convs, bn):
        conv, kt = convs[li], convs[-1].kernel_size
        cout, cin = bank.shape[:2]
        k = conv.kernel_size
        fused = os.environ.get("EQA_TRAIN_FUSED_BN", "1") != "0"
        want_stats = (fused and os.environ.get("EQA_TRAIN_EPILOGUE_STATS", "1") != "0" and (bn.training or bn.running_mean is None))
        lift = self._lift_kernel(conv, bank, h, narrow_unchecked=True)
        with_stats = False
        if not conv.lifting and k == 5 and winograd.applicable(h, cin, cout):
            route, with_stats = "wino", want_stats and winograd.Conv5x5Function.stats_supported(h, bank)
        elif (not conv.lifting and k != 5
              and fftconv.applicable_k(h.shape, cin, cout, k, h.device, h.is_contiguous(memory_format=torch.channels_last))):
            route = "fftk"
        elif lift == "narrow":
            route, with_stats = "lift", want_stats and ops.lift_conv_stats_supported(h.shape, k, k, cout)
        else:
            route = "lift_wide" if lift == "wide" else "lib"
        OH, OW = h.shape[-2] - k + 1, h.shape[-1] - k + 1
        if (fused and li == len(convs) - 2 and os.environ.get("EQA_TRAIN_FUSED_TAIL", "1") != "0" and kt <= ops.MAX_WINDOW_K
                and OH > 2 * (kt - 1) and OW > 2 * (kt - 1) and h.shape[0] <= 65535):
            return route, with_stats, "fused_tail"
        return route, with_stats, "fused" if fused else "ops"

    def _forward_training(self, x: torch.Tensor) -> torch.Tensor:
        convs, norms = self._layers()
        drops = [m for m in self.eqv_network if isinstance(m, nn.Dropout)]
        E = self.num_group_elements
        h = x.contiguous(memory_format=torch.channels_last)
        tail = convs[-1]
        S = None
        for li, (conv, bn, drop) in enumerate(zip(convs[:-1], norms, drops)):
            bank = conv.expanded_weights()
            route, with_stats, block = self._train_route(li, h, bank, convs, bn)
            if route == "wino":
                h = winograd.Conv5x5Function.apply(h, bank, winograd.tile_for(h), with_stats)
            elif route == "fftk":
                h = fftconv.ConvKxKFunction.apply(h, bank)
            elif route in ("lift", "lift_wide"):
                h = LiftConvFunction.apply(h, bank, with_stats)
            else:
                h = F.conv2d(h, bank.contiguous(memory_format=torch.channels_last))
                if not h.is_contiguous(memory_format=torch.channels_last):
                    block = "ops"
            h, part = h if with_stats else (h, None)
            if block == "fused_tail":
                S = InnerBnReluDropoutWindowSums.apply(h, bn.weight, bn.bias, bn, E, conv.bias, drop.p, drop.training, tail.kernel_size, part)
            elif block == "fused":
                h = InnerBnReluDropout.apply(h, bn.weight, bn.bias, bn, E, conv.bias, drop.p, drop.training, part)
            else:
                h = F.dropout(torch.relu(self._inner_bn(h, bn, E, conv.bias)), drop.p, drop.training)
        k, O = tail.kernel_size, tail.out_channels
        H, W = h.shape[-2:]
        if S is None:
            S = WindowSumsFunction.apply(h, k)
        weff = tail.expanded_weights().view(O, E, -1).double().sum(0)
        if S.is_cuda and S.dtype == torch.float64 and E <= 16 and os.environ.get("EQA_WS_TABLE_KERNEL", "1") != "0":
            act = WindowSumsLinearFn.apply(S.flatten(1), weff, 1.0 / float(O * (H - k + 1) * (W - k + 1)))
        else:
            act = S.flatten(1) @ weff.t() / float(O * (H - k + 1) * (W - k + 1))
        if tail.bias is not None:
            act = act + tail.bias.double().mean()
        hidden_bias = [c.bias.sum() for c in convs[:-1] if c.bias is not None]
        if hidden_bias:
            act = act + 0.0 * torch.stack(hidden_bias).sum().double()
        return act.float()

    def _training_fast_path_ok(self, x: torch.Tensor) -> bool:
        if self._dense or not x.is_cuda or x.dtype != torch.float32 or os.environ.get("EQA_TRAIN_FAST", "1") == "0":
            return False
        if (self.out_channels * self.num_group_elements) % 4 != 0:
            return False
        convs = [m for m in self.eqv_network if hasattr(m, "expanded_weights")]
        if len(convs) < 2 or any(c.stride != 1 or c.padding != 0 for c in convs) or not convs[-1].supports_linear_tail():
            return False
        hw = x.shape[-2] - (self.kernel_size - 1) * (len(convs) - 1)
        k = convs[-1].kernel_size
        return hw >= 2 * k - 1 and x.shape[-1] - (self.kernel_size - 1) * (len(convs) - 1) >= 2 * k - 1 and hw * hw <= 12288

    def forward(self, x: torch.Tensor) -> torch.Tensor:
        if (self.training or torch.is_grad_enabled()) and self._training_fast_path_ok(x):
            return self._forward_training(x)
        if not self.training and not torch.is_grad_enabled() and x.is_cuda and x.dtype == torch.float32:
            convs, norms = self._layers()
            shrink = (self.kernel_size - 1) * (len(convs) - 1)
            oh, ow = x.shape[-2] - shrink, x.shape[-1] - shrink
            if (convs[-1].supports_linear_tail() and 0 < oh and 0 < ow and oh * ow <= 12288
                    and all(n.running_mean is not None and not n.training for n in norms)
                    and all(c.stride == 1 and c.padding == 0 and c.kernel_size == self.kernel_size for c in convs)):
                return self._forward_inference(x)
        if self._dense:
            convs, norms = self._dense
            for i, cv in enumerate(convs):
                x = cv(x)
                if i < len(norms):
                    x = F.relu(norms[i](x))
            fm = x.reshape(x.shape[0], self.out_channels, self.num_group_elements, x.shape[-2], x.shape[-1])
        else:
            fm = self.eqv_network(x)
        return group_pool(fm)


from equiadapt_amd.images.canonicalization_networks.wrn_networks import (
    ESCNNWideBasic,
    ESCNNWideBottleneck,
    ESCNNWRNEquivariantNetwork,
)
```

### equiadapt_amd/images/canonicalization_networks/fftconv.py

```python
import math
import os
from typing import Optional

import torch

from equiadapt_amd import _lib, ops
from equiadapt_amd.ops import _timed

N, NH, OUT = 48, 25, 44
F = N * (NH - 2) + 2 * NH
ENABLED = os.environ.get("EQA_CONV5_FFT", "1") != "0"
MIN_TILES = int(os.environ.get("EQA_FFT_MIN_TILES", "32"))
TRAIN_FORWARD = os.environ.get("EQA_FFT_TRAIN", "1") != "0"
GEMM = os.environ.get("EQA_FFT_GEMM", "3m")
GEMM_PIECES = os.environ.get("EQA_FFT_GEMM_PIECES", "auto")
AUTO_MIN_CIN = int(os.environ.get("EQA_FFT_GEMM_AUTO_MIN_CIN", "128"))
AUTO_MIN_CIN_H3 = int(os.environ.get("EQA_FFT_GEMM_AUTO_MIN_CIN_H3", "64"))
DCMAX_SLOTS = 256
LAST_FORM = None
GEMM_C16 = os.environ.get("EQA_FFT_GEMM_C16", "1") != "0"
LAST_CONTRACTION = None
LAST_WGRAD = None


def f16_form_takes(cin: int, cout: int) -> bool:
    return cout % 128 == 0 and cin % 32 == 0


def gemm_form(cin: int, cout: int, bounded: bool = False) -> str:
    if GEMM_PIECES in ("f32", "9", "6"):
        return GEMM_PIECES
    if bounded and f16_form_takes(cin, cout) and (GEMM_PIECES == "h3" or cin >= AUTO_MIN_CIN_H3):
        return "h3"
    return "6" if cin >= AUTO_MIN_CIN and cout % 128 == 0 else "f32"


def f16_scale(t: torch.Tensor) -> float:
    mx = float(t.abs().max().item())
    ex = 14 - math.frexp(mx)[1] if 0.0 < mx < float("inf") else 0
    return math.ldexp(1.0, max(-100, min(100, ex)))


class Spectra3M:

    __slots__ = ("data", "cin", "cout", "_pieces", "_pieces_f16")

    def __init__(self, data: torch.Tensor, cin: int, cout: int):
        self.data, self.cin, self.cout, self._pieces, self._pieces_f16 = data, cin, cout, None, None

    def pieces_f16(self):
        if self._pieces_f16 is None:
            lib = _lib.load()
# ... 113 lines not shown


def freq_index():
    ky = torch.arange(N).repeat_interleave(NH - 2)
    kx = torch.arange(1, NH - 1).repeat(N)
    eky = torch.arange(NH).repeat_interleave(2)
    ekx = torch.tensor([0, NH - 1]).repeat(NH)
    return torch.cat([ky, eky]), torch.cat([kx, ekx])


def tiles_k(n: int, k: int) -> int:
    o = N + 1 - k
    return 0 if n < k else (n - (k - 1) + o - 1) // o


def tiles(n: int) -> int:
    return tiles_k(n, 5)


def _stands_for_channels_last(self, memory_format=torch.contiguous_format) -> bool:
    return memory_format == torch.channels_last


class GroupedMap:

    def __init__(self, data: torch.Tensor):
        assert data.dim() == 5 and data.shape[-1] == 16 and data.is_contiguous()
        self.data = data
        self.shape = torch.Size((data.shape[0], data.shape[1] * 16, data.shape[2], data.shape[3]))
        self.device, self.dtype, self.is_cuda = data.device, data.dtype, data.is_cuda

    def data_ptr(self) -> int:
        return self.data.data_ptr()

    def to_channels_last(self) -> torch.Tensor:
        n, g, h, w, _ = self.data.shape
        return self.data.permute(0, 1, 4, 2, 3).reshape(n, g * 16, h, w).contiguous(memory_format=torch.channels_last)

    materialize, is_contiguous = to_channels_last, _stands_for_channels_last


class LiftedInput:

    def __init__(self, x: torch.Tensor, bank: torch.Tensor, bias: Optional[torch.Tensor], relu: bool, pieces: Optional[torch.Tensor] = None,
                 pieces_f16=None):
        assert x.dim() == 4 and x.shape[1] == 3 and bank.shape[1:] == (3, 5, 5)
        self.x = x.contiguous(memory_format=torch.channels_last)
        self.bank = bank.contiguous(memory_format=torch.channels_last)
        self.bias, self.relu = (bias.contiguous() if bias is not None else None), bool(relu)
        self.shape = torch.Size((x.shape[0], bank.shape[0], x.shape[2] - 4, x.shape[3] - 4))
        self.device, self.dtype, self.is_cuda = x.device, x.dtype, x.is_cuda
        self._pieces = pieces
        self._pieces_f16 = pieces_f16

    @staticmethod
    def split_f16(bank: torch.Tensor):
        w = bank.float()
        C = w.shape[0]
        scale = f16_scale(w)
        wp = torch.zeros(C, 5, 8, 4, dtype=torch.float32, device=w.device)
        wp[:, :, 1:6, :3] = w.permute(0, 2, 3, 1) * scale
        chunks = wp.reshape(C, 5, 4, 8)
        h1 = chunks.half()
        h2 = (chunks - h1.float()).half()
        return torch.stack([h1, h2], dim=1).contiguous(), scale

    @staticmethod
    def split_bf16(bank: torch.Tensor) -> torch.Tensor:
        w = bank.float()
        C = w.shape[0]
        wp = torch.zeros(C, 5, 6, 4, dtype=torch.float32, device=w.device)
        wp[:, :, :5, :3] = w.permute(0, 2, 3, 1)
        chunks = torch.zeros(C, 16, 8, dtype=torch.float32, device=w.device)
        chunks[:, :15] = wp.reshape(C, 5, 3, 8).reshape(C, 15, 8)
        p0 = chunks.bfloat16()
        r1 = chunks - p0.float()
        p1 = r1.bfloat16()
        p2 = (r1 - p1.float()).bfloat16()
        assert torch.equal((p0.float() + p1.float()) + p2.float(), chunks), "the three bf16 pieces of a weight must add up exactly"
        return torch.stack([p0, p1, p2], dim=1).contiguous()

    @classmethod
    def form_operand(cls):
        return {"h2": ("lifth", "pieces_f16", cls.split_f16), "bf16x3": ("liftp", "pieces", cls.split_bf16)}.get(LIFT_FFT_FORM)

    def pieces_f16(self):
        if self._pieces_f16 is None:
            self._pieces_f16 = self.split_f16(self.bank)
        return self._pieces_f16

    def pieces(self) -> torch.Tensor:
        if self._pieces is None:
            self._pieces = self.split_bf16(self.bank)
        return self._pieces

    def spectra_into(self, V: torch.Tensor, B, st: int) -> Optional[torch.Tensor]:
        lib = _lib.load()
        nimg, C, H, W = self.shape
        dims = (nimg, H + 4, W + 4, C, st)
        px, pV = self.x.data_ptr(), V.data_ptr()
        p_b = self.bias.data_ptr() if self.bias is not None else None
        want_dc = self.relu and isinstance(B, Spectra3M) and gemm_form(B.cin, B.cout, True) == "h3"
        vbound = None
        if LIFT_FFT_FORM == "h2" and px % 16 == 0:
            wh, w_scale = self.pieces_f16()
            xbound = torch.empty(DCMAX_SLOTS, dtype=torch.float32, device=self.device)
            _lib.check(lib.eqa_absmax_slots(px, self.x.numel(), xbound.data_ptr(), st), "eqa_absmax_slots")
            if want_dc:
                vbound = torch.empty(DCMAX_SLOTS, dtype=torch.float32, device=self.device)
            _lib.check(lib.eqa_lift5_fft48k5_input_f16x2(px, wh.data_ptr(), w_scale, xbound.data_ptr(), DCMAX_SLOTS, p_b, int(self.relu), pV,
                                                         vbound.data_ptr() if want_dc else None, *dims), "eqa_lift5_fft48k5_input_f16x2")
        elif LIFT_FFT_FORM == "bf16x3":
            _lib.check(lib.eqa_lift5_fft48k5_input_bf16x3(px, self.pieces().data_ptr(), p_b, int(self.relu), pV, *dims),
                       "eqa_lift5_fft48k5_input_bf16x3")
        elif want_dc:
            vbound = torch.empty(DCMAX_SLOTS, dtype=torch.float32, device=self.device)
            _lib.check(lib.eqa_lift5_fft48k5_input_dcmax(px, self.bank.data_ptr(), p_b, 1, pV, vbound.data_ptr(), *dims),
                       "eqa_lift5_fft48k5_input_dcmax")
        else:
            _lib.check(lib.eqa_lift5_fft48k5_input(px, self.bank.data_ptr(), p_b, int(self.relu), pV, *dims), "eqa_lift5_fft48k5_input")
        return vbound

    def materialize(self) -> torch.Tensor:
        return ops.lift_conv_nhwc(self.x, ops.pack_lift_weights(self.bank), self.bias, self.relu, 5, 5)

    is_contiguous = _stands_for_channels_last


LIFT_FFT_FORM = os.environ.get("EQA_LIFT_FFT_FORM", "h2")
LIFT_FFT_FUSED_DEFAULT = "1"


def lift_fused_applicable(x_shape, bank_shape, cout_next: int, device) -> bool:
    if os.environ.get("EQA_LIFT_FFT_FUSED", LIFT_FFT_FUSED_DEFAULT) == "0" or len(x_shape) != 4:
        return False
    C, Cin, kh, kw = bank_shape
    if not _lib.load().eqa_lift5_fft48k5_input_supported(Cin, kh, kw, C):
        return False
    out_shape = (x_shape[0], C, x_shape[2] - 4, x_shape[3] - 4)
    return x_shape[2] >= 5 and x_shape[3] >= 5 and grouped_applicable(out_shape, C, cout_next, device)


def _tiles_pay(shape, cin: int, cout: int, max_waste: float) -> bool:
    if shape[1] != cin or (not gemm3m_supported(cin, cout) and ops.plane_gemm_supported(cin, cout)):
        return False
    H, W = shape[-2:]
    if H < 16 or W < 16 or shape[0] * tiles(H) * tiles(W) < MIN_TILES:
        return False
    return tiles(H) * OUT <= max_waste * (H - 4) and tiles(W) * OUT <= max_waste * (W - 4)


def grouped_applicable(shape, cin: int, cout: int, device, max_waste: float = 1.12) -> bool:
    if not (ENABLED and device.type == "cuda" and len(shape) == 4 and cin % 16 == 0):
        return False
    if os.environ.get("EQA_FFT_GROUPED", "1") == "0" or not _lib.load().eqa_fft48k5_input_grouped_supported(cin):
        return False
    return _tiles_pay(shape, cin, cout, max_waste)


def applicable(x: torch.Tensor, cin: int, cout: int, max_waste: float = 1.12) -> bool:
    if isinstance(x, (GroupedMap, LiftedInput)):
        return grouped_applicable(x.shape, cin, cout, x.device, max_waste)
    if not (ENABLED and x.is_cuda and x.dtype == torch.float32 and x.dim() == 4 and x.is_contiguous(memory_format=torch.channels_last)):
# ... 50 lines not shown

def _transform(name: str, k: int, *args) -> None:
    lib = _lib.load()
    if k == 5:
        _lib.check(getattr(lib, "eqa_fft48k5_" + name)(*args), "eqa_fft48k5_" + name)
    else:
        _lib.check(getattr(lib, "eqa_fft48_" + name)(*args[:-1], k, args[-1]), "eqa_fft48_" + name)


def _workspace(k: int, nimg: int, rows: int, out_cols: int, C: int, device) -> torch.Tensor:
    lib = _lib.load()
    nbytes = lib.eqa_fft48k5_workspace_bytes(nimg, rows, out_cols, C) if k == 5 else lib.eqa_fft48_workspace_bytes(nimg, rows, out_cols, C, k)
    return torch.empty(max(nbytes, 4) // 4, dtype=torch.float32, device=device)


def applicable_k(x_shape, cin: int, cout: int, k: int, device, channels_last: bool = True) -> bool:
    if not (ENABLED and k in KSIZES and k != 5 and device.type == "cuda" and channels_last and len(x_shape) == 4 and x_shape[1] == cin):
        return False
    if os.environ.get("EQA_FFT_ANYK", "1") == "0":
        return False
    nimg, _, H, W = x_shape
    if H < max(16, k) or W < max(16, k) or nimg * tiles_k(H, k) * tiles_k(W, k) < 8:
        return False
    oh, ow = H - k + 1, W - k + 1
    t = tiles_k(H, k) * tiles_k(W, k)
    fft_us = t * (F * 8 * (cin + cout) * 2.2 / 4.0e6 + F * 6 * cin * cout / 100e6)
    direct_us = oh * ow * k * k * 2 * cin * cout / 110e6
    return fft_us * 1.3 < direct_us


def spectra_for_k(bank: torch.Tensor, correlate: bool = True):
    k = bank.shape[-1]
    if k == 5:
        return spectra_for(bank, correlate)
    lib = _lib.load()
    Cout, Cin = bank.shape[:2]
    assert bank.is_cuda and bank.dtype == torch.float32 and bank.shape[-2] == k and lib.eqa_fft48_supported(k)
    st = ops._stream()
    with torch.cuda.device(bank.device):
        if gemm3m_supported(Cin, Cout):
            B3 = torch.empty(lib.eqa_fft48k5_spectra3m_floats(Cin, Cout), dtype=torch.float32, device=bank.device)
            _lib.check(lib.eqa_fft48_filter_spectra3m(bank.contiguous().data_ptr(), B3.data_ptr(), Cout, Cin, k, int(correlate), st),
                       "eqa_fft48_filter_spectra3m")
            return Spectra3M(B3, Cin, Cout)
        if gemm3m_c16_supported(Cin, Cout):
            return filter_spectra3m_c16(bank, correlate)
        B = torch.empty((F, 2 * Cin, 2 * Cout), dtype=torch.float32, device=bank.device)
        _lib.check(lib.eqa_fft48_filter_spectra(bank.contiguous().data_ptr(), B.data_ptr(), Cout, Cin, k, int(correlate), st),
                   "eqa_fft48_filter_spectra")
        return B


def conv_kxk(x: torch.Tensor, B, k: int, bias: Optional[torch.Tensor], relu: bool, in_bias: Optional[torch.Tensor] = None,
             in_relu: bool = False, keep_V: Optional[list] = None, sums_k: int = 0, stats: Optional[list] = None) -> torch.Tensor:
    lib = _lib.load()
    nimg, Cin, H, W = x.shape
    if isinstance(B, (Spectra3M, Spectra3MC16)):
        Cout = B.cout
        assert B.cin == Cin
    else:
        Cout = B.shape[2] // 2
        assert B.shape == (F, 2 * Cin, 2 * Cout)
    assert k == 5 or not (sums_k or stats is not None or isinstance(x, (GroupedMap, LiftedInput))), "k = 5 only"
    OH, OW = H - k + 1, W - k + 1
    TX = tiles_k(W, k)
    M = nimg * tiles_k(H, k) * TX
    dev = x.device
    st = ops._stream()
    V = spectra_buffer(M, 2 * Cin, dev)
    p_bias = bias.data_ptr() if bias is not None else None
    vbound = None
    with torch.cuda.device(dev):
        if isinstance(x, LiftedInput):
            assert in_bias is None and not in_relu
            with _timed("lift_fft_input"):
                vbound = x.spectra_into(V, B, st)
        else:
            T = _workspace(k, nimg, H, OW, Cin, dev)
            with _timed("fft_input"):
                _transform("input_grouped" if isinstance(x, GroupedMap) else "input", k, x.data_ptr(), T.data_ptr(), V.data_ptr(),
                           in_bias.data_ptr() if in_bias is not None else None, int(in_relu), nimg, H, W, Cin, st)
            del T
        with _timed("fft_gemm"):
            Mo = contract(V, B, M, vbound)
        if keep_V is not None:
            keep_V.append(V)
        del V
        T2 = _workspace(k, nimg, OH, OW, Cout, dev)
        if sums_k:
            S = torch.empty((nimg, Cout, sums_k, sums_k), dtype=torch.float64, device=dev)
            ws = torch.empty(nimg * OH * TX * Cout * (2 * sums_k - 1), dtype=torch.float32, device=dev)
            with _timed("fft_output_sums"):
                _lib.check(lib.eqa_fft48k5_output_sums(Mo.data_ptr(), T2.data_ptr(), p_bias, int(relu), S.data_ptr(), ws.data_ptr(),
                                                       nimg, OH, OW, Cout, sums_k, st), "eqa_fft48k5_output_sums")
            return S
        y = torch.empty((nimg, Cout, OH, OW), dtype=torch.float32, device=dev, memory_format=torch.channels_last)
        if stats is not None:
            assert bias is None and not relu
            part = torch.empty((lib.eqa_fft48k5_output_stats_rows(nimg, OH, OW, Cout), Cout, 2), dtype=torch.float64, device=dev)
            with _timed("fft_output"):
                _lib.check(lib.eqa_fft48k5_output_stats(Mo.data_ptr(), T2.data_ptr(), y.data_ptr(), part.data_ptr(), nimg, OH, OW, Cout, st),
                           "eqa_fft48k5_output_stats")
            stats.append(part)
            return y
        with _timed("fft_output"):
            _transform("output", k, Mo.data_ptr(), T2.data_ptr(), p_bias, int(relu), y.data_ptr(), nimg, OH, OW, Cout, st)
        return y


def conv5x5(x: torch.Tensor, B: torch.Tensor, bias: Optional[torch.Tensor], relu: bool,
            in_bias: Optional[torch.Tensor] = None, in_relu: bool = False, sums_k: int = 0,
            keep_V: Optional[list] = None, stats: Optional[list] = None) -> torch.Tensor:
    return conv_kxk(x, B, 5, bias, relu, in_bias, in_relu, keep_V, sums_k, stats)


def grad_spectra(dy: torch.Tensor, k: int = 5) -> torch.Tensor:
    nimg, Cout, OH, OW = dy.shape
    M = nimg * tiles_k(OH + k - 1, k) * tiles_k(OW + k - 1, k)
    T = _workspace(k, nimg, OH, OW, Cout, dy.device)
    G = spectra_buffer(M, 2 * Cout, dy.device)
    with torch.cuda.device(dy.device):
        _transform("grad_transform", k, dy.data_ptr(), T.data_ptr(), G.data_ptr(), nimg, OH, OW, Cout, ops._stream())
    return G


def wgrad_c16_admitted(M: int, cin: int, cout: int) -> bool:
    if not (GEMM_C16 and _lib.load().eqa_fft48_wgrad3m_c16_supported(cin, cout)):
        return False
    pad = (-(-cin // 32) * 32) * (-(-cout // 32) * 32)
    return 3 * pad < 4 * cin * cout or (M <= 72 and min(cin, cout) >= 48)


def filter_grad_k(V: torch.Tensor, dy: torch.Tensor, cin: int, k: int, G: Optional[torch.Tensor] = None) -> torch.Tensor:
    lib = _lib.load()
    nimg, Cout, OH, OW = dy.shape
    dev = dy.device
    M = V.shape[1]
    assert V.shape == (F, M, 2 * cin) and M == nimg * tiles_k(OH + k - 1, k) * tiles_k(OW + k - 1, k)
    st = ops._stream()
    if G is None:
        G = grad_spectra(dy, k)
    dbank = torch.empty((Cout, cin, k, k), dtype=torch.float32, device=dev)
    with torch.cuda.device(dev):
        global LAST_WGRAD
        wgrad3m = GEMM == "3m" and os.environ.get("EQA_FFT_WGRAD3M", "1") != "0"
        LAST_WGRAD = ("3m" if wgrad3m and lib.eqa_fft48k5_wgrad3m_supported(cin, Cout) else
                      "c16" if wgrad3m and wgrad_c16_admitted(M, cin, Cout) else "lib")
        packed = LAST_WGRAD != "lib"
        if packed:
            D = torch.empty((F, cin, 2, Cout), dtype=torch.float32, device=dev)
            if LAST_WGRAD == "3m":
                _lib.check(lib.eqa_fft48k5_wgrad3m(V.data_ptr(), G.data_ptr(), D.data_ptr(), M, cin, Cout, st), "eqa_fft48k5_wgrad3m")
            else:
                _lib.check(lib.eqa_fft48_wgrad3m_c16(V.data_ptr(), G.data_ptr(), D.data_ptr(), M, cin, Cout, st), "eqa_fft48_wgrad3m_c16")
        else:
            D = torch.bmm(V.transpose(1, 2), G)
        if k != 5:
            _lib.check(lib.eqa_fft48_filter_grad(D.data_ptr(), dbank.data_ptr(), Cout, cin, k, int(packed), st), "eqa_fft48_filter_grad")
        elif packed:
            _lib.check(lib.eqa_fft48k5_filter_grad3m(D.data_ptr(), dbank.data_ptr(), Cout, cin, st), "eqa_fft48k5_filter_grad3m")
        else:
            _lib.check(lib.eqa_fft48k5_filter_grad(D.data_ptr(), dbank.data_ptr(), Cout, cin, st), "eqa_fft48k5_filter_grad")
    return dbank


def filter_grad(V: torch.Tensor, dy: torch.Tensor, cin: int, G: Optional[torch.Tensor] = None) -> torch.Tensor:
# ... 44 lines not shown
```

### equiadapt_amd/images/canonicalization_networks/pooling.py

```python
import os

import torch

from equiadapt_amd import _lib, ops


class _GroupPoolFn(torch.autograd.Function):
    @staticmethod
    def forward(ctx, feature_map: torch.Tensor) -> torch.Tensor:
        ctx.shape = tuple(feature_map.shape)
        act, _ = ops.group_pool_argmax(feature_map, want_index=False)
        return act

    @staticmethod
    def backward(ctx, grad_act: torch.Tensor):
        B, C, G, H, W = ctx.shape
        return (grad_act / float(C * H * W))[:, None, :, None, None].expand(B, C, G, H, W)


def group_pool(feature_map: torch.Tensor) -> torch.Tensor:
    if feature_map.dtype != torch.float32:
        return torch.mean(feature_map, dim=(1, 3, 4))
    return _GroupPoolFn.apply(feature_map)


def conv_then_group_pool(h: torch.Tensor, layer, scale=None, shift=None, relu: bool = False) -> torch.Tensor:
    k, E, O = layer.kernel_size, layer.num_group_elements, layer.out_channels
    B, _, H, W = h.shape
    S = ops.window_sums(h, k, scale, shift, relu)
    return window_sums_to_activations(S, layer, H, W)


def window_sums_to_activations(S: torch.Tensor, layer, H: int, W: int) -> torch.Tensor:
    k, O = layer.kernel_size, layer.out_channels
    weff = layer.mean_response_weights()
    scale = 1.0 / float(O * (H - k + 1) * (W - k + 1))
    if S.is_cuda and weff.shape[0] <= 16 and not torch.is_grad_enabled():
        return ops.window_sums_gemv(S.flatten(1), weff, scale, layer.mean_bias_value())
    act = S.flatten(1) @ weff.t() * scale
    if layer.bias is not None:
        mb = layer.mean_bias_value()
        act = act + (mb if isinstance(mb, float) else mb.to(act.device))
    return act.float()


class WindowSumsLinearFn(torch.autograd.Function):

    @staticmethod
    def forward(ctx, S, weff, scale):
        S, weff = S.contiguous(), weff.contiguous()
        ctx.save_for_backward(S, weff)
        ctx.scale = scale
        return ops.window_sums_gemv(S, weff, scale, 0.0)

    @staticmethod
    @torch.autograd.function.once_differentiable
    def backward(ctx, dact):
        S, weff = ctx.saved_tensors
        dS, dW = ops.window_sums_gemv_bwd(dact.float().contiguous(), weff, S, ctx.scale, ctx.needs_input_grad[0], ctx.needs_input_grad[1])
        return dS, dW, None


def window_grad_table(dS: torch.Tensor, H: int, W: int, k: int) -> torch.Tensor:
    nb, dev = k - 1, dS.device
    if (dS.is_cuda and dS.dtype == torch.float64 and k <= ops.MAX_WINDOW_K and dS.shape[0] <= 65535 and H >= 2 * nb + 1 and W >= 2 * nb + 1
            and os.environ.get("EQA_WS_TABLE_KERNEL", "1") != "0"):
        return ops.window_grad_table(dS.contiguous(), H, W)

    def mask(n):
        rep = torch.cat([torch.arange(nb), torch.tensor([nb]), torch.arange(n - nb, n)]).to(dev)
        u = torch.arange(k, device=dev)
        return ((u[None, :] <= rep[:, None]) & (rep[:, None] <= u[None, :] + (n - k))).to(dS.dtype)

    return torch.einsum("tu,bcuv,sv->btsc", mask(H), dS, mask(W)).float().contiguous()


class WindowSumsFunction(torch.autograd.Function):

    @staticmethod
    def forward(ctx, x, k):
        ctx.k, ctx.shape = k, x.shape
        ctx.channels_last = x.is_contiguous(memory_format=torch.channels_last)
        return ops.window_sums(x, k)

    @staticmethod
    def backward(ctx, dS):
        k = ctx.k
        B, C, H, W = ctx.shape
        table = window_grad_table(dS, H, W, k)
        if table.is_cuda and C % 4 == 0:
            g = torch.empty((B, H, W, C), dtype=torch.float32, device=table.device)
            with torch.cuda.device(table.device):
                st = _lib.load().eqa_window_sums_bwd_expand_nhwc(table.data_ptr(), g.data_ptr(), B, H, W, C, k, ops._stream())
            _lib.check(st, "eqa_window_sums_bwd_expand_nhwc")
        else:
            def cls(n):
# ... 9 lines not shown
```

### equiadapt_amd/ops.py

```python
from typing import Optional, Tuple

import torch

from equiadapt_amd import _lib


MAX_WINDOW_K = 10
VNSMALL_PARAMS = 1310
VNSMALL_PARAMS_MAX = 1751


def _stream() -> int:
    return _raw_stream(_current_device())


try:
    _raw_stream, _current_device = torch._C._cuda_getCurrentRawStream, torch._C._cuda_getDevice
except AttributeError:
    def _raw_stream(_dev):
        return torch.cuda.current_stream().cuda_stream

    def _current_device():
        return 0


class KernelTimer:

    active: "Optional[KernelTimer]" = None

    def __init__(self):
        self.events = {}

    def __enter__(self):
        KernelTimer.active = self
        return self

    def __exit__(self, *exc):
        KernelTimer.active = None

    def summary(self):
        torch.cuda.synchronize()
        return {k: (len(v), sum(a.elapsed_time(b) for a, b in v) / len(v)) for k, v in self.events.items()}


class _timed:
    def __init__(self, name: str):
        self.t = KernelTimer.active
        self.name = name

    def __enter__(self):
        if self.t is not None:
            self.a = torch.cuda.Event(enable_timing=True)
            self.b = torch.cuda.Event(enable_timing=True)
            self.a.record()

    def __exit__(self, *exc):
        if self.t is not None:
# ... 272 lines not shown
        st = lib.eqa_so3_rotate(x.data_ptr(), R.data_ptr(), y.data_ptr(), B, N, int(transpose), _stream())
    _lib.check(st, "eqa_so3_rotate")
    return y


def gram_schmidt(v: torch.Tensor) -> torch.Tensor:
    lib = _lib.load()
    v = _need(v, "vectors")
    if v.dim() != 3 or v.shape[1:] != (3, 3):
        raise ValueError("gram_schmidt expects (B,3,3)")
    out = torch.empty_like(v)
    with torch.cuda.device(v.device):
        st = lib.eqa_gram_schmidt(v.data_ptr(), out.data_ptr(), v.shape[0], _stream())
    _lib.check(st, "eqa_gram_schmidt")
    return out


def _vnsmall_args(what: str, x: torch.Tensor, params: torch.Tensor, pooling: str):
    x = _need(x, "point_cloud")
    params = _need(params, "params")
    B, three, N = x.shape
    if pooling not in ("mean", "max"):
        raise ValueError(f"Pooling type {pooling} not supported")
    if three != 3 or params.numel() != (VNSMALL_PARAMS if pooling == "mean" else VNSMALL_PARAMS_MAX):
        raise ValueError(f"{what} expects x:(B,3,N) and {VNSMALL_PARAMS} (mean) / {VNSMALL_PARAMS_MAX} (max) packed parameters")
    return x, params, B, N


def vnsmall_forward(x: torch.Tensor, params: torch.Tensor, k: int = 20, pooling: str = "mean") -> torch.Tensor:
    lib = _lib.load()
    x, params, B, N = _vnsmall_args("vnsmall_forward", x, params, pooling)
    out = torch.empty((B, 3, 3), dtype=torch.float32, device=x.device)
    ws = torch.empty((max(lib.eqa_vnsmall_workspace_bytes(B, N), 4) // 4,), dtype=torch.float32, device=x.device)
    with torch.cuda.device(x.device), _timed("vnsmall_fwd"):
        st = lib.eqa_vnsmall_fwd(x.data_ptr(), params.data_ptr(), out.data_ptr(), ws.data_ptr(), B, N, k, int(pooling == "max"), _stream())
    _lib.check(st, "eqa_vnsmall_fwd")
    return out


def vnsmall_canonicalize(x: torch.Tensor, params: torch.Tensor, k: int = 20, pooling: str = "mean"):
    lib = _lib.load()
    x, params, B, N = _vnsmall_args("vnsmall_canonicalize", x, params, pooling)
    vec = torch.empty((B, 3, 3), dtype=torch.float32, device=x.device)
    R = torch.empty((B, 3, 3), dtype=torch.float32, device=x.device)
    y = torch.empty_like(x)
    ws = torch.empty((max(lib.eqa_vnsmall_workspace_bytes(B, N), 4) // 4,), dtype=torch.float32, device=x.device)
    with torch.cuda.device(x.device), _timed("vnsmall_fwd"):
        st = lib.eqa_vnsmall_canonicalize(x.data_ptr(), params.data_ptr(), vec.data_ptr(), R.data_ptr(), y.data_ptr(), ws.data_ptr(),
                                          B, N, k, int(pooling == "max"), _stream())
    _lib.check(st, "eqa_vnsmall_canonicalize")
    return vec, R, y


def crop_resize_aa(x: torch.Tensor, tables, out_hw: Tuple[int, int]) -> torch.Tensor:
    lib = _lib.load()
    x = _need(x, "x")
    wx, x0, wy, y0, K, max_rows, x_begin, x_span = tables
    B, C, H, W = x.shape
    y = torch.empty((B, C, out_hw[0], out_hw[1]), dtype=torch.float32, device=x.device)
    with torch.cuda.device(x.device), _timed("crop_resize_aa"):
        st = lib.eqa_crop_resize_aa(x.data_ptr(), y.data_ptr(), wx.data_ptr(), x0.data_ptr(), wy.data_ptr(), y0.data_ptr(),
                                    B * C, H, W, out_hw[0], out_hw[1], K, max_rows, x_begin, x_span, _stream())
    _lib.check(st, "eqa_crop_resize_aa")
    return y


def mask_action_nearest(masks: torch.Tensor, eidx: torch.Tensor, rtheta: torch.Tensor, flags: Optional[torch.Tensor]) -> torch.Tensor:
    lib = _lib.load()
    masks = _need(masks, "masks", torch.uint8)
    eidx = _need(eidx, "eidx", torch.int32)
    rtheta = _need(rtheta, "rtheta")
    flags, p_flags = _opt(flags, "flags", torch.int32)
    n, H, W = masks.shape
    out = torch.empty_like(masks)
    with torch.cuda.device(masks.device), _timed("mask_action"):
        st = lib.eqa_mask_action_nearest(masks.data_ptr(), out.data_ptr(), eidx.data_ptr(), rtheta.data_ptr(), p_flags,
                                         rtheta.shape[0], n, H, W, _stream())
    _lib.check(st, "eqa_mask_action_nearest")
    return out


_plane_tables: dict = {}


def mask_action_nearest_planes(mask_list, eidx: torch.Tensor, rtheta: torch.Tensor, flags: Optional[torch.Tensor]) -> torch.Tensor:
    lib = _lib.load()
    eidx = _need(eidx, "eidx", torch.int32)
    rtheta = _need(rtheta, "rtheta")
    flags, p_flags = _opt(flags, "flags", torch.int32)
    masks = [_need(m, "masks", torch.uint8) for m in mask_list]
    H, W = masks[0].shape[-2:]
    ptrs = tuple(m.data_ptr() + k * H * W for m in masks for k in range(m.shape[0]))
    n = len(ptrs)
    dev = masks[0].device
    key = (ptrs, str(dev))
    table = _plane_tables.get(key)
    if table is None:
        if len(_plane_tables) >= 64:
            _plane_tables.clear()
        table = torch.tensor(ptrs, dtype=torch.int64).to(dev)
        _plane_tables[key] = table
    out = torch.empty((n, H, W), dtype=torch.uint8, device=dev)
    with torch.cuda.device(dev), _timed("mask_action"):
        st = lib.eqa_mask_action_nearest_planes(table.data_ptr(), out.data_ptr(), eidx.data_ptr(), rtheta.data_ptr(), p_flags,
                                                rtheta.shape[0], n, H, W, _stream())
    _lib.check(st, "eqa_mask_action_nearest_planes")
    return out


def boxes_action(boxes: torch.Tensor, img_of_box: torch.Tensor, rotation_deg: torch.Tensor, width: float,
                 flip_all: bool) -> Tuple[torch.Tensor, Optional[torch.Tensor]]:
    lib = _lib.load()
    boxes = _need(boxes, "boxes")
    img_of_box = _need(img_of_box, "img_of_box", torch.int32)
    rotation_deg = _need(rotation_deg, "rotation_deg")
    out = torch.empty_like(boxes)
    flipped = torch.empty_like(boxes) if flip_all else None
# ... 224 lines not shown


def affine_relu_rows(h: torch.Tensor, scale: torch.Tensor, shift: torch.Tensor) -> torch.Tensor:
    lib = _lib.load()
    h, scale, shift = _need(h, "h"), _need(scale, "scale"), _need(shift, "shift")
    rows, D = h.shape
    z = torch.empty_like(h)
    with torch.cuda.device(h.device):
        st = lib.eqa_affine_relu_rows(h.data_ptr(), scale.data_ptr(), shift.data_ptr(), z.data_ptr(), rows, D, _stream())
    _lib.check(st, "eqa_affine_relu_rows")
    return z


def cosine_group_activations(v: torch.Tensor, ref: torch.Tensor, num_group: int, eps: float = 1e-8) -> torch.Tensor:
    lib = _lib.load()
    v, ref = _need(v, "vector_out"), _need(ref.reshape(-1), "reference_vector")
    R, V = v.shape
    if R % num_group or ref.numel() != V:
        raise ValueError("cosine_group_activations expects (G*B, V) embeddings and a (V) reference vector")
    B = R // num_group
    act = torch.empty((B, num_group), dtype=torch.float32, device=v.device)
    with torch.cuda.device(v.device):
        st = lib.eqa_cosine_group_activations(v.data_ptr(), ref.data_ptr(), act.data_ptr(), B, num_group, V, float(eps), _stream())
    _lib.check(st, "eqa_cosine_group_activations")
    return act


def bias_relu_nhwc_(x: torch.Tensor, bias: torch.Tensor) -> torch.Tensor:
    lib = _lib.load()
    if not (x.is_cuda and x.dtype == torch.float32 and x.is_contiguous(memory_format=torch.channels_last)):
        raise RuntimeError("bias_relu_nhwc_ expects a channels-last fp32 tensor on the device")
    bias = _need(bias, "bias")
    B, C, H, W = x.shape
    with torch.cuda.device(x.device), _timed("bias_relu"):
        st = lib.eqa_bias_relu_nhwc(x.data_ptr(), bias.data_ptr(), B * H * W, C, _stream())
    _lib.check(st, "eqa_bias_relu_nhwc")
    return x


def window_sums_gemv(S: torch.Tensor, weff: torch.Tensor, scale: float, shift) -> torch.Tensor:
    lib = _lib.load()
    S = _need(S, "S", torch.float64)
    weff = _need(weff, "weff", torch.float64)
    B, K = S.shape
    E = weff.shape[0]
    act = torch.empty((B, E), dtype=torch.float32, device=S.device)
    sh = shift if isinstance(shift, float) else 0.0
    with torch.cuda.device(S.device), _timed("sums_gemv"):
        st = lib.eqa_window_sums_gemv(S.data_ptr(), weff.data_ptr(), act.data_ptr(), B, K, E, float(scale), sh, _stream())
    _lib.check(st, "eqa_window_sums_gemv")
    if not isinstance(shift, float):
        act += shift.to(torch.float32)
    return act


def window_sums_gemv_bwd(dact: torch.Tensor, weff: torch.Tensor, S: torch.Tensor, scale: float, need_dS: bool, need_dW: bool):
    lib = _lib.load()
    dact = _need(dact, "dact")
    weff, S = _need(weff, "weff", torch.float64), _need(S, "S", torch.float64)
    B, K = S.shape
    E = weff.shape[0]
    dS = torch.empty_like(S) if need_dS else None
    dW = torch.empty_like(weff) if need_dW else None
    ws = torch.empty((max(lib.eqa_window_sums_gemv_bwd_workspace_bytes(K, E), 8) // 8,), dtype=torch.float64, device=S.device) if need_dW else None
    with torch.cuda.device(S.device), _timed("sums_gemv_bwd"):
        st = lib.eqa_window_sums_gemv_bwd(dact.data_ptr(), weff.data_ptr(), S.data_ptr(), dS.data_ptr() if need_dS else None,
                                          dW.data_ptr() if need_dW else None, ws.data_ptr() if need_dW else None, B, K, E, float(scale), _stream())
    _lib.check(st, "eqa_window_sums_gemv_bwd")
    return dS, dW


def window_grad_table(dS: torch.Tensor, H: int, W: int) -> torch.Tensor:
    lib = _lib.load()
    dS = _need(dS, "dS", torch.float64)
    B, C, k, _ = dS.shape
    T = 2 * (k - 1) + 1
    table = torch.empty((B, T, T, C), dtype=torch.float32, device=dS.device)
    with torch.cuda.device(dS.device), _timed("window_grad_table"):
        st = lib.eqa_window_grad_table(dS.data_ptr(), table.data_ptr(), B, C, H, W, k, _stream())
    _lib.check(st, "eqa_window_grad_table")
    return table


def plane_gemm_supported(cin: int, cout: int) -> bool:
    return bool(_lib.load().eqa_plane_gemm_supported(cin, cout))


def pack_plane_gemm_weights(U: torch.Tensor) -> torch.Tensor:
    P, Cin, Cout = U.shape
    t = U.float().reshape(P, Cin // 16, 2, 2, 4, Cout // 32, 32)
    return t.permute(0, 1, 5, 2, 3, 6, 4).contiguous()


def plane_gemm(V: torch.Tensor, Upk: torch.Tensor, M: torch.Tensor, tiles: int) -> None:
    lib = _lib.load()
    V, Upk, M = _need(V, "V"), _need(Upk, "Upk"), _need(M, "M")
    P, Cin = V.shape[1], V.shape[2]
    Cout = M.shape[2]
    with torch.cuda.device(V.device):
        st = lib.eqa_plane_gemm(V.data_ptr(), Upk.data_ptr(), M.data_ptr(), tiles, P, Cin, Cout, _stream())
    _lib.check(st, "eqa_plane_gemm")


def lift_conv_supported(cin: int, kh: int, kw: int, cout: int) -> bool:
    return kh in (3, 5) and 9 <= kw * cin <= 15 and cout % 16 == 0

# ... 682 lines not shown
```

### include/eqa_hip.h

```cpp
#ifndef EQA_HIP_H
#define EQA_HIP_H

#include <stdint.h>

#ifdef __cplusplus
extern "C" {
#endif

#define EQA_OK 0
#define EQA_ERR_INVALID_ARG (-1)
#define EQA_ERR_LAUNCH (-2)
#define EQA_ERR_UNSUPPORTED (-3)

#define EQA_FLIP_SRC 1
#define EQA_FLIP_DST 2

#define EQA_ABI_VERSION 3
int eqa_abi_version(void);

int eqa_set_option(int key, int value);
int eqa_get_option(int key);

int eqa_canon_transform_fwd(const float* x, float* y, const int32_t* gidx, const float* theta,
                            const int32_t* flags, int num_elements, int B, int C, int H, int W, int pad,
                            void* stream);

int eqa_invert_action_fwd(const float* f, float* out, const int32_t* gidx, const float* theta,
                          const int32_t* flags, const int32_t* chan_map, int num_elements, int G, int B, int C,
                          int H, int W, void* stream);

int eqa_group_action_pair(const float* x, float* y, const float* theta_canon, const int32_t* flags_canon, int pad, int C,
                          const float* f, float* out, const float* theta_inv, const int32_t* flags_inv,
                          const int32_t* chan_map, int G, int Cf, const int32_t* gidx, int num_elements, int B, int H,
                          int W, void* stream);

int eqa_orbit_expand_fwd(const float* x, float* y, const float* theta, const int32_t* flags, int num_elements,
                         int B, int C, int S, int pad, void* stream);

int eqa_group_action_fwd(const float* src, float* dst, const int32_t* gidx, const float* theta,
                         const int32_t* flags, const int32_t* chan_map, int num_elements, int G, int n_out,
                         int B, int C, int H, int W, int pad, int OH, int OW, int top, int left, void* stream);
int eqa_group_action_fwd_hint(const float* src, float* dst, const int32_t* gidx, const float* theta, const int32_t* flags,
                              const int32_t* chan_map, int num_elements, int G, int n_out, int B, int C, int H, int W,
                              int pad, int OH, int OW, int top, int left, int max_window, void* stream);

int eqa_crop_resize_aa(const float* x, float* y, const float* wx, const int32_t* x0, const float* wy, const int32_t* y0,
                       int planes, int H, int W, int OH, int OW, int K, int max_rows, int x_begin, int x_span, void* stream);

int eqa_mask_action_nearest(const uint8_t* m, uint8_t* out, const int32_t* eidx, const float* rtheta, const int32_t* flags,
                            int num_elements, int n_masks, int H, int W, void* stream);
int eqa_mask_action_nearest_planes(const uint8_t* const* planes, uint8_t* out, const int32_t* eidx, const float* rtheta,
                                   const int32_t* flags, int num_elements, int n_masks, int H, int W, void* stream);

int eqa_boxes_action(const float* boxes, const int32_t* img_of_box, const float* rotation_deg, float* flipped, float* out,
                     int n, float width, int flip_all, void* stream);

int eqa_image_action_nearest(const float* x, float* out, const int32_t* eidx, const float* rtheta, const int32_t* flags,
                             int num_elements, int n_planes, int src_mod, int H, int W, int pad, int OH, int OW, int top,
                             int left, void* stream);

int64_t eqa_fold_edge_pad_workspace_bytes(int planes, int H, int W, int pad);
int eqa_fold_edge_pad(const float* gframe, float* gsrc, void* workspace, int planes, int H, int W, int pad, void* stream);
int eqa_group_action_bwd_tiles(int OH, int OW);
int eqa_group_action_bwd(const float* src, const float* grad_out, const int32_t* gidx, const float* theta,
                         const int32_t* flags, const int32_t* chan_map, float* grad_src, float* grad_angle_partial,
                         int num_elements, int G, int n_out, int B, int C, int H, int W, int pad, int OH, int OW,
                         int top, int left, void* stream);
int eqa_group_action_bwd_theta(const float* src, const float* grad_out, const int32_t* gidx, const float* theta,
                               const int32_t* flags, const int32_t* chan_map, float* grad_src, float* grad_theta_partial,
                               int num_elements, int G, int n_out, int B, int C, int H, int W, int pad, int OH, int OW,
                               int top, int left, void* stream);

int64_t eqa_group_pool_workspace_bytes(int B, int Cf, int G, int HW);
int eqa_group_pool_argmax(const float* feat, float* act, int32_t* gidx, void* workspace, int B, int Cf, int G,
                          int HW, void* stream);

int eqa_window_sums(const float* x, const float* scale, const float* shift, int relu, double* out, int B, int C, int H,
                    int W, int k, void* stream);

int eqa_conv_s2_supported(int Cin, int Cout, int K, int pad, int planar);
int eqa_conv_s2(const float* x, const float* wp, const float* bias, int gelu, float* y, int B, int Cin, int H, int W, int Cout, int K,
                int pad, int planar, void* stream);
int eqa_conv_s2_wgrad_supported(int Cin, int Cout, int K, int pad, int planar);
int64_t eqa_conv_s2_wgrad_workspace_bytes(int B, int Cin, int H, int W, int Cout, int K, int pad, int planar);
int eqa_conv_s2_wgrad(const float* x, const float* dz, float* dw, void* workspace, int B, int Cin, int H, int W, int Cout, int K, int pad,
                      int planar, void* stream);
int eqa_conv_s2_dgrad_supported(int Cin, int Cout, int K, int pad);
int eqa_conv_s2_dgrad(const float* dz, const float* wd, float* dx, int B, int Cin, int H, int W, int Cout, int K, int pad, void* stream);
int eqa_bn_act_fwd(const float* z, const float* scale, const float* shift, const float* rowscale, float* y, int64_t npix, int C, int act,
                   void* stream);
int64_t eqa_bn_act_partial_blocks(int64_t npix);
int eqa_bn_act_stats(const float* z, double* partial, int64_t npix, int C, void* stream);
int eqa_bn_act_finalize(const double* partial, int64_t npix, int C, const float* gamma, const float* beta, double eps, double momentum,
                        float* running_mean, float* running_var, float* scale, float* shift, float* mean, float* rstd, void* stream);
int eqa_bn_act_bwd_finalize(const double* partial, int64_t npix, int C, const float* gamma, const float* rstd, float* dgamma, float* dbeta,
                            float* gscale, float* m1, float* m2, void* stream);
int eqa_bn_act_bwd_reduce(const float* gy, const float* z, const float* scale, const float* shift, const float* mean, const float* rstd,
                          const float* rowscale, double* partial, int64_t npix, int C, int act, void* stream);
int eqa_bn_act_bwd_apply(const float* gy, const float* z, const float* scale, const float* shift, const float* mean, const float* rstd,
                         const float* rowscale, const float* gscale, const float* m1, const float* m2, float* dz, int64_t npix, int C,
// ... 77 lines not shown
int64_t eqa_fft48k5_tile_pitch(int64_t tiles);
int eqa_fft48k5_frequencies(void);
int eqa_fft48k5_filter_spectra(const float* bank, float* B, int Cout, int Cin, int correlate, void* stream);
int eqa_fft48k5_cgemm3m_supported(int Cin, int Cout);
int64_t eqa_fft48k5_spectra3m_floats(int Cin, int Cout);
int eqa_fft48k5_filter_spectra3m(const float* bank, float* B3, int Cout, int Cin, int correlate, void* stream);
int eqa_fft48k5_cgemm3m(const float* V, const float* B3, float* Mo, int64_t M, int Cin, int Cout, void* stream);
int64_t eqa_fft48k5_spectra3m_bf16_bytes(int Cin, int Cout);
int eqa_fft48k5_spectra3m_split(const float* B3, void* Bp, int Cin, int Cout, void* stream);
int eqa_fft48k5_cgemm3m_bf16x3(const float* V, const void* Bp, float* Mo, int64_t M, int Cin, int Cout, int terms, void* stream);
int64_t eqa_fft48k5_spectra3m_f16_bytes(int Cin, int Cout);
int eqa_fft48k5_spectra3m_split_f16(const float* B3, void* Bh, int Cin, int Cout, float b_scale, void* stream);
int eqa_fft48k5_cgemm3m_f16x2(const float* V, const void* Bh, float* Mo, int64_t M, int Cin, int Cout, const float* vbound, int nbound,
                              float b_scale, void* stream);
int eqa_fft48k5_wgrad3m_supported(int Cin, int Cout);
int eqa_fft48k5_wgrad3m(const float* V, const float* G, float* D, int64_t M, int Cin, int Cout, void* stream);
int eqa_fft48k5_filter_grad3m(const float* D, float* dbank, int Cout, int Cin, void* stream);
int eqa_fft48_cgemm3m_c16_supported(int Cin, int Cout);
int64_t eqa_fft48_spectra3m_c16_floats(int Cin, int Cout);
int eqa_fft48k5_filter_spectra3m_c16(const float* bank, float* B3, int Cout, int Cin, int correlate, void* stream);
int eqa_fft48_filter_spectra3m_c16(const float* bank, float* B3, int Cout, int Cin, int ksize, int correlate, void* stream);
int eqa_fft48_cgemm3m_c16(const float* V, const float* B3, float* Mo, int64_t M, int Cin, int Cout, void* stream);
int eqa_fft48_wgrad3m_c16_supported(int Cin, int Cout);
int eqa_fft48_wgrad3m_c16(const float* V, const float* G, float* D, int64_t M, int Cin, int Cout, void* stream);
int eqa_fft48k5_group(int C, int side);
int64_t eqa_fft48k5_workspace_bytes(int nimg, int rows, int out_cols, int C);
int eqa_fft48k5_input(const float* x, float* T, float* V, const float* in_bias, int in_relu, int nimg, int H, int W, int C,
                      void* stream);
int eqa_fft48k5_input_grouped_supported(int C);
int eqa_fft48k5_input_grouped(const float* x, float* T, float* V, const float* in_bias, int in_relu, int nimg, int H, int W, int C,
                              void* stream);
int eqa_lift5_fft48k5_input_supported(int Cin, int KH, int KW, int Cout);
int eqa_lift5_fft48k5_input(const float* x, const float* bank, const float* bias, int relu, float* V, int nimg, int H0, int W0, int Cout,
                            void* stream);
#define EQA_LIFT5_DCMAX_SLOTS 256
int eqa_lift5_fft48k5_input_dcmax(const float* x, const float* bank, const float* bias, int relu, float* V, float* dcmax, int nimg, int H0,
                                  int W0, int Cout, void* stream);
int64_t eqa_lift5_pieces_f16_bytes(int Cout);
int eqa_absmax_slots(const float* x, int64_t n, float* slots, void* stream);
int eqa_lift5_fft48k5_input_f16x2(const float* x, const void* wpieces, float w_scale, const float* xbound, int nxbound, const float* bias,
                                  int relu, float* V, float* dcmax, int nimg, int H0, int W0, int Cout, void* stream);
int64_t eqa_lift5_pieces_bytes(int Cout);
int eqa_lift5_fft48k5_input_bf16x3(const float* x, const void* wpieces, const float* bias, int relu, float* V, int nimg, int H0, int W0,
                                   int Cout, void* stream);
int eqa_fft48k5_output(const float* Mo, float* T2, const float* bias, int relu, float* y, int nimg, int OH, int OW, int C,
                       void* stream);
int64_t eqa_fft48k5_output_stats_rows(int nimg, int OH, int OW, int C);
int eqa_fft48k5_output_stats(const float* Mo, float* T2, float* y, double* partial, int nimg, int OH, int OW, int C, void* stream);
int eqa_fft48k5_grad_transform(const float* dy, float* T, float* G, int nimg, int OH, int OW, int C, void* stream);
int eqa_fft48k5_filter_grad(const float* D, float* dbank, int Cout, int Cin, void* stream);
int eqa_fft48k5_input_grad(const float* Cg, float* T2, float* dx, int nimg, int H, int W, int C, void* stream);
int eqa_fft48k5_output_sums(const float* Mo, float* T2, const float* bias, int relu, double* S, void* workspace, int nimg,
                            int OH, int OW, int C, int k_next, void* stream);

int eqa_fft48_supported(int ksize);
int64_t eqa_fft48_tiles(int n, int ksize);
int64_t eqa_fft48_workspace_bytes(int nimg, int rows, int out_cols, int C, int ksize);
int eqa_fft48_filter_spectra(const float* bank, float* B, int Cout, int Cin, int ksize, int correlate, void* stream);
int eqa_fft48_filter_spectra3m(const float* bank, float* B3, int Cout, int Cin, int ksize, int correlate, void* stream);
int eqa_fft48_input(const float* x, float* T, float* V, const float* in_bias, int in_relu, int nimg, int H, int W, int C, int ksize,
                    void* stream);
int eqa_fft48_grad_transform(const float* dy, float* T, float* G, int nimg, int OH, int OW, int C, int ksize, void* stream);
int eqa_fft48_output(const float* Mo, float* T2, const float* bias, int relu, float* y, int nimg, int OH, int OW, int C, int ksize,
                     void* stream);
int eqa_fft48_input_grad(const float* Cg, float* T2, float* dx, int nimg, int H, int W, int C, int ksize, void* stream);
int eqa_fft48_filter_grad(const float* D, float* dbank, int Cout, int Cin, int ksize, int packed, void* stream);

int eqa_group_argmax(const float* act, int32_t* gidx, int B, int G, void* stream);

int eqa_so3_rotate(const float* x, const float* R, float* y, int B, int N, int transpose, void* stream);

#define EQA_VNSMALL_PARAMS 1310
#define EQA_VNSMALL_PARAMS_MAX 1751
int64_t eqa_vnsmall_workspace_bytes(int B, int N);
int eqa_vnsmall_fwd(const float* x, const float* params, float* out, void* workspace, int B, int N, int k, int pooling,
                    void* stream);
int eqa_vnsmall_canonicalize(const float* x, const float* params, float* vectors, float* R, float* y, void* workspace, int B, int N,
                             int k, int pooling, void* stream);

int eqa_vn_blocks(int N);
int eqa_vn_knn(const float* x, int32_t* idx, int B, int N, int k, void* stream);
int eqa_vn_convpos_stats(const float* x, const int32_t* idx, const float* Wf, float* partial, int B, int N, int k, void* stream);
int eqa_vn_convpos_fwd(const float* x, const int32_t* idx, const float* Wf, const float* Wd, const float* scale, const float* shift,
                       float* pooled, int B, int N, int k, void* stream);
int eqa_vn_convpos_bwd_reduce(const float* x, const int32_t* idx, const float* Wf, const float* Wd, const float* scale,
                              const float* shift, const float* mean, const float* rstd, const float* gpool, float* partial, int B,
                              int N, int k, void* stream);
int eqa_vn_convpos_bwd_apply(const float* x, const int32_t* idx, const float* Wf, const float* Wd, const float* scale,
                             const float* shift, const float* mean, const float* rstd, const float* m1, const float* m2,
                             const float* gpool, float* partial, int B, int N, int k, void* stream);

int eqa_vn_convpos_max_fwd(const float* x, const int32_t* idx, const float* Wf, const float* Wd, const float* scale,
                           const float* shift, const float* Wp, float* pooled, uint8_t* sel, int B, int N, int k, void* stream);
int eqa_vn_convpos_max_bwd_reduce(const float* x, const int32_t* idx, const float* Wf, const float* Wd, const float* scale,
                                  const float* shift, const float* mean, const float* rstd, const float* gpool,
                                  const uint8_t* sel, float* partial, int B, int N, int k, void* stream);
int eqa_vn_convpos_max_bwd_apply(const float* x, const int32_t* idx, const float* Wf, const float* Wd, const float* scale,
                                 const float* shift, const float* mean, const float* rstd, const float* m1, const float* m2,
                                 const float* gpool, const uint8_t* sel, float* partial, int B, int N, int k, void* stream);

int eqa_vn_tail_blocks(int N);
int eqa_vn_tail_partial_floats(int pass);
int eqa_vn_tail_pass(int pass, const float* pooled, const float* weights, const float* stat, const float* red, const float* mask,
                     const float* gout, float* partial, float* g_pooled, int B, int N, void* stream);
int eqa_vn_bn_finalize(const float* partial, int nblk, int stride, int C, long long M, const float* gamma, const float* beta,
                       float* running_mean, float* running_var, long long* num_batches_tracked, float momentum, float eps, float* stat,
// ... 69 lines not shown
```

Before: 70920 images/s.

## Fuse crop-resize with NHWC output and absmax, and fuse window-sums tail with argmax

Adds an NHWC crop+antialiased-resize kernel that prefetches rows into registers, writes channel-interleaved output and records per-block absmax slots, so the downstream f16-split lift conv can skip a separate layout pass and absmax reduction. It also splits the final conv's window-sum path into a partials kernel plus a fused tail kernel that finalizes the sums, applies the mean-response GEMV, takes the group argmax and emits rotation/reflection in one launch. The goal is fewer launches and less memory traffic in the head and tail of the canonicalization forward. Both paths are on by default through environment flags and fall back to the old path when shapes are unsupported.

```diff
diff --git a/equiadapt_amd/_lib.py b/equiadapt_amd/_lib.py
--- a/equiadapt_amd/_lib.py
+++ b/equiadapt_amd/_lib.py
@@ -31,6 +31,8 @@
     "eqa_group_action_fwd": (_int, [_vp, _vp, _vp, _vp, _vp, _vp] + [_int] * 12 + [_vp]),
     "eqa_group_action_fwd_hint": (_int, [_vp, _vp, _vp, _vp, _vp, _vp] + [_int] * 13 + [_vp]),
     "eqa_crop_resize_aa": (_int, [_vp] * 6 + [_int] * 9 + [_vp]),
+    "eqa_crop_resize_aa_nhwc_slots": (_int, [_int] * 10),
+    "eqa_crop_resize_aa_nhwc": (_int, [_vp] * 6 + [_int] * 10 + [_vp, _vp]),
     "eqa_mask_action_nearest": (_int, [_vp] * 5 + [_int] * 4 + [_vp]),
     "eqa_mask_action_nearest_planes": (_int, [_vp] * 5 + [_int] * 4 + [_vp]),
     "eqa_boxes_action": (_int, [_vp] * 5 + [_int, ctypes.c_float, _int, _vp]),
@@ -167,6 +169,8 @@
     "eqa_window_sums_nhwc": (_int, [_vp, _vp, _vp, _int, _vp, _vp] + [_int] * 5 + [_vp]),
     "eqa_window_sums_bwd_expand_nhwc": (_int, [_vp, _vp] + [_int] * 5 + [_vp]),
     "eqa_group_argmax": (_int, [_vp, _vp, _int, _int, _vp]),
+    "eqa_fft48k5_output_sums_partials": (_int, [_vp, _vp, _vp, _int, _vp] + [_int] * 5 + [_vp, _vp]),
+    "eqa_window_sums_tail": (_int, [_vp] * 8 + [_int] * 6 + [ctypes.c_double, ctypes.c_double, _vp]),
     "eqa_vnsmall_workspace_bytes": (ctypes.c_int64, [_int, _int]),
     "eqa_vnsmall_fwd": (_int, [_vp, _vp, _vp, _vp, _int, _int, _int, _int, _vp]),
     "eqa_vnsmall_canonicalize": (_int, [_vp] * 6 + [_int] * 4 + [_vp]),
diff --git a/equiadapt_amd/csrc/crop_resize.hip b/equiadapt_amd/csrc/crop_resize.hip
--- a/equiadapt_amd/csrc/crop_resize.hip
+++ b/equiadapt_amd/csrc/crop_resize.hip
@@ -354,9 +354,197 @@
   }
 }
 
+constexpr int kAaNhwcTrips = 6;
+
+template <int K, int BAND, int NL, int C>
+__global__ __launch_bounds__(kThreads, (NL > 5 && K > 5) ? 2 : 3) void crop_resize_aa_nhwc_kernel(
+    const float* __restrict__ x, float* __restrict__ y, const float* __restrict__ wx, const int32_t* __restrict__ x0,
+    const float* __restrict__ wy, const int32_t* __restrict__ y0, int nimg, int H, int W, int OH, int OW, int cap_rows, int xb, int xl,
+    float* __restrict__ slots) {
+  extern __shared__ __attribute__((aligned(16))) float aa_tmp[];
+  float* rows = aa_tmp;
+  float* tmp = aa_tmp + (size_t)cap_rows * xl;
+  float* tabw = tmp + (size_t)cap_rows * OW;
+  int* taby = reinterpret_cast<int*>(tabw + BAND * K);
+  __shared__ float s_max[kThreads / 64];
+  const int r0 = blockIdx.y * BAND, r1 = min(r0 + BAND, OH);
+  const int nband = r1 - r0;
+  const int img0 = (int)(blockIdx.z * kXcd + blockIdx.x), img_step = (int)(gridDim.z * kXcd);
+  const int rows_par = kThreads / OW;
+  const int ox = threadIdx.x % OW, rsub = threadIdx.x / OW;
+  const int xs_g = x0[ox];
+  float wv[K];
+  int xo[K];
+#pragma unroll
+  for (int j = 0; j < K; ++j) {
+    wv[j] = wx[ox * K + j];
+    xo[j] = min(xs_g - xb + j, xl - 1);
+  }
+  if ((int)threadIdx.x < nband * K) tabw[threadIdx.x] = wy[r0 * K + threadIdx.x];
+  const int ybeg = y0[r0];
+  if ((int)threadIdx.x < nband) taby[threadIdx.x] = y0[r0 + threadIdx.x] - ybeg;
+  const int yend = min(y0[r1 - 1] + K, H);
+  const int nrows = min(yend - ybeg, cap_rows);
+  const int nq = xl >> 2;
+  const int tq = threadIdx.x & 63, tr = threadIdx.x >> 6;
+  const bool prefetch = nq <= 64 && nrows <= 4 * NL;
+  const size_t plane_sz = (size_t)H * W;
+  const float* src0 = x + (size_t)ybeg * W + xb;
+  typedef float aa_f4 __attribute__((ext_vector_type(4)));
+  aa_f4 v[NL];
+#define EQA_AA_PF_LOAD(plane_)                                                                                          \
+  do {                                                                                                                  \
+    const float* src_ = src0 + (size_t)(plane_) * plane_sz;                                                             \
+    _Pragma("unroll") for (int k = 0; k < NL; ++k)                                                           \
+      v[k] = *reinterpret_cast<const aa_f4*>(src_ + (size_t)min(tr + 4 * k, nrows - 1) * W + 4 * min(tq, nq - 1));     \
+  } while (0)
+  __builtin_amdgcn_s_waitcnt(0x0070);
+  if (prefetch && img0 < nimg) EQA_AA_PF_LOAD((size_t)img0 * C);
+  const int nout = nband * OW;
+  float mx = 0.0f;
+  for (int img = img0; img < nimg; img += img_step) {
+    float o[kAaNhwcTrips][C];
+#pragma unroll
+    for (int c = 0; c < C; ++c) {
+      const size_t plane = (size_t)img * C + c;
+      if (prefetch) {
+        if (tq < nq) {
+#pragma unroll
+          for (int k = 0; k < NL; ++k)
+            if (tr + 4 * k < nrows) *reinterpret_cast<aa_f4*>(rows + (tr + 4 * k) * xl + 4 * tq) = v[k];
+        }
+        if (c + 1 < C) EQA_AA_PF_LOAD(plane + 1);
+        else if (img + img_step < nimg) EQA_AA_PF_LOAD((size_t)(img + img_step) * C);
+      } else {
+        const float* src = src0 + plane * plane_sz;
+        for (int q = tq; q < nq; q += 64)
+          for (int rb = tr; rb < nrows; rb += 4) *reinterpret_cast<aa_f4*>(rows + rb * xl + 4 * q) = *reinterpret_cast<const aa_f4*>(src + (size_t)rb * W + 4 * q);
+      }
+      __syncthreads();
+      if (rsub < rows_par) {
+        for (int ry0 = rsub; ry0 < nrows; ry0 += 4 * rows_par) {
+          float acc[4] = {0.0f, 0.0f, 0.0f, 0.0f};
+#pragma unroll
+          for (int u = 0; u < 4; ++u) {
+            const float* row = rows + min(ry0 + u * rows_par, nrows - 1) * xl;
+#pragma unroll
+            for (int j = 0; j < K; ++j)
+              acc[u] += wv[j] * row[xo[j]];
+          }
+#pragma unroll
+          for (int u = 0; u < 4; ++u)
+            if (ry0 + u * rows_par < nrows) tmp[(ry0 + u * rows_par) * OW + ox] = acc[u];
+        }
+      }
+      __syncthreads();
+      int r = rsub, oxx = ox;
+#pragma unroll
+      for (int t = 0; t < kAaNhwcTrips; ++t) {
+        float acc = 0.0f;
+        if (r < nband) {
+          const int ys = taby[r];
+#pragma unroll
+          for (int j = 0; j < K; ++j)
+            acc += tabw[r * K + j] * tmp[min(ys + j, nrows - 1) * OW + oxx];
+        }
+        o[t][c] = acc;
+        r += rows_par;
+        oxx += kThreads - rows_par * OW;
+        if (oxx >= OW) { oxx -= OW; ++r; }
+      }
+      __syncthreads();
+    }
+    float* dst = y + ((size_t)img * OH + r0) * OW * C;
+#pragma unroll
+    for (int t = 0; t < kAaNhwcTrips; ++t) {
+      const int idx = (int)threadIdx.x + t * kThreads;
+      if (idx < nout) {
+#pragma unroll
+        for (int c = 0; c < C; ++c) {
+          dst[(size_t)idx * C + c] = o[t][c];
+          mx = fmaxf(mx, fabsf(o[t][c]));
+        }
+      }
+    }
+  }
+#undef EQA_AA_PF_LOAD
+  if (slots) {
+#pragma unroll
+    for (int off = 32; off > 0; off >>= 1) mx = fmaxf(mx, __shfl_xor(mx, off));
+    if ((threadIdx.x & 63) == 0) s_max[threadIdx.x >> 6] = mx;
+    __syncthreads();
+    if (threadIdx.x == 0)
+      slots[((size_t)blockIdx.z * gridDim.y + blockIdx.y) * gridDim.x + blockIdx.x] = fmaxf(fmaxf(s_max[0], s_max[1]), fmaxf(s_max[2], s_max[3]));
+  }
+}
+
+struct AaNhwcPlan {
+  int band, cap_rows, xb, xl, nbands, groups;
+  size_t lds;
+  bool few;
+};
+
+int aa_nhwc_plan(int nimg, int C, int H, int W, int OH, int OW, int K, int max_rows, int x_begin, int x_span, AaNhwcPlan& p) {
+  if (nimg < 0 || C <= 0 || H <= 0 || W <= 0 || OH <= 0 || OW <= 0 || K <= 0 || max_rows <= 0) return EQA_ERR_INVALID_ARG;
+  if ((C != 1 && C != 3) || K > EQA_AA_WIDE_MIN_K || (W & 3) != 0 || x_span <= 0 || x_begin < 0 || x_begin + x_span > W) return EQA_ERR_UNSUPPORTED;
+  p.xb = x_begin & ~3;
+  p.xl = std::min(W, (x_begin + x_span + 3) & ~3) - p.xb;
+  auto staged_lds = [&](int bnd) { return ((size_t)(bnd / kAaBand) * max_rows * (p.xl + OW) + bnd * (EQA_AA_WIDE_MIN_K + 1)) * sizeof(float); };
+  p.band = OH >= 64 ? 16 : 8;
+  if (p.band == 16 && (staged_lds(16) > 64 * 1024 || 16 * K > kThreads || 16 * OW > kAaNhwcTrips * kThreads)) p.band = 8;
+  p.cap_rows = (p.band / kAaBand) * max_rows;
+  p.lds = staged_lds(p.band);
+  if (p.lds > 64 * 1024 || p.band * K > kThreads || p.band * OW > kAaNhwcTrips * kThreads || OW > kThreads) return EQA_ERR_UNSUPPORTED;
+  static const int per_cu = [] { const char* e = getenv("EQA_AA_NHWC_BLOCKS_PER_CU"); return e ? std::max(1, atoi(e)) : 3; }();
+  p.nbands = (OH + p.band - 1) / p.band;
+  p.groups = std::max(1, (std::min(nimg, (256 * per_cu + p.nbands - 1) / p.nbands) + kXcd - 1) / kXcd);
+  p.few = p.cap_rows <= 20;
+  return p.groups > 65535 ? EQA_ERR_UNSUPPORTED : EQA_OK;
+}
+
 }
 
 extern "C" {
+
+int eqa_crop_resize_aa_nhwc_slots(int nimg, int C, int H, int W, int OH, int OW, int K, int max_rows, int x_begin, int x_span) {
+  AaNhwcPlan p;
+  const int rc = aa_nhwc_plan(nimg, C, H, W, OH, OW, K, max_rows, x_begin, x_span, p);
+  return rc != EQA_OK ? rc : kXcd * p.nbands * p.groups;
+}
+
+int eqa_crop_resize_aa_nhwc(const float* x, float* y, const float* wx, const int32_t* x0, const float* wy, const int32_t* y0, int nimg,
+                            int C, int H, int W, int OH, int OW, int K, int max_rows, int x_begin, int x_span, float* slots, void* stream) {
+  if (!x || !y || !wx || !x0 || !wy || !y0) return EQA_ERR_INVALID_ARG;
+  AaNhwcPlan p;
+  const int rc = aa_nhwc_plan(nimg, C, H, W, OH, OW, K, max_rows, x_begin, x_span, p);
+  if (rc != EQA_OK) return rc;
+  if ((((uintptr_t)x) & 15) != 0) return EQA_ERR_UNSUPPORTED;
+  const dim3 grid(kXcd, p.nbands, p.groups);
+#define EQA_AA_NHWC_C(K_, C_)                                                                                                          \
+  do {                                                                                                                                 \
+    if (p.band == 16)                                                                                                                  \
+      hipLaunchKernelGGL((crop_resize_aa_nhwc_kernel<K_, 16, 10, C_>), grid, dim3(kThreads), p.lds, (hipStream_t)stream, x, y, wx, x0, wy, \
+                         y0, nimg, H, W, OH, OW, p.cap_rows, p.xb, p.xl, slots);                                                       \
+    else if (p.few)                                                                                                                    \
+      hipLaunchKernelGGL((crop_resize_aa_nhwc_kernel<K_, 8, 5, C_>), grid, dim3(kThreads), p.lds, (hipStream_t)stream, x, y, wx, x0, wy,  \
+                         y0, nimg, H, W, OH, OW, p.cap_rows, p.xb, p.xl, slots);                                                       \
+    else                                                                                                                               \
+      hipLaunchKernelGGL((crop_resize_aa_nhwc_kernel<K_, 8, 10, C_>), grid, dim3(kThreads), p.lds, (hipStream_t)stream, x, y, wx, x0, wy, \
+                         y0, nimg, H, W, OH, OW, p.cap_rows, p.xb, p.xl, slots);                                                       \
+  } while (0)
+#define EQA_AA_NHWC(K_)                                    \
+  case K_:                                                 \
+    if (C == 3) EQA_AA_NHWC_C(K_, 3);                      \
+    else EQA_AA_NHWC_C(K_, 1);                             \
+    break
+  switch (K) {
+    EQA_AA_NHWC(1); EQA_AA_NHWC(2); EQA_AA_NHWC(3); EQA_AA_NHWC(4); EQA_AA_NHWC(5); EQA_AA_NHWC(6); EQA_AA_NHWC(7); EQA_AA_NHWC(8);
+    default: return EQA_ERR_UNSUPPORTED;
+  }
+#undef EQA_AA_NHWC
+#undef EQA_AA_NHWC_C
+  return launch_status();
+}
 
 int eqa_crop_resize_aa(const float* x, float* y, const float* wx, const int32_t* x0, const float* wy, const int32_t* y0,
                        int planes, int H, int W, int OH, int OW, int K, int max_rows, int x_begin, int x_span, void* stream) {
diff --git a/equiadapt_amd/csrc/fftconv.hip b/equiadapt_amd/csrc/fftconv.hip
--- a/equiadapt_amd/csrc/fftconv.hip
+++ b/equiadapt_amd/csrc/fftconv.hip
@@ -1050,12 +1050,10 @@
   return FftK<5>::output<0>(Mo, T2, nullptr, 0, y, nimg, OH, OW, C, (hipStream_t)stream, opt);
 }
 
-int eqa_fft48k5_output_sums(const float* Mo, float* T2, const float* bias, int relu, double* S, void* workspace, int nimg,
-                            int OH, int OW, int C, int k_next, void* stream) {
-  if (!fft_map_args_ok(Mo, T2, S, nimg, OH, OW, C) || !workspace || k_next <= 0) return EQA_ERR_INVALID_ARG;
+static int fft48k5_output_partials(const float* Mo, float* T2, const float* bias, int relu, void* workspace, int nimg, int OH, int OW, int C,
+                                   int k_next, int* nseg_sub, void* stream) {
   const int nb = k_next - 1;
   if ((nb != 4 && nb != 2) || OH < 2 * nb + 1 || OW < 2 * nb + 1 || k_next > kMaxWinK || nimg > 65535) return EQA_ERR_UNSUPPORTED;
-  if (nimg == 0) return EQA_OK;
   hipStream_t st = (hipStream_t)stream;
   float* part = (float*)workspace;
   int form = 0;
@@ -1068,7 +1066,25 @@
   const int sub = form ? fft_ntiles(OW, kFftO) : 1;
   const int per_row = form == 3 ? kPipeCons / 64 : form;
   const int nseg = form ? 2 * nb + per_row * fft_ntiles(OH, kFftO) : OH;
-  return eqa::launch_window_sums_nhwc_finalize(part, S, nimg, C, k_next, nseg * sub, st, sub);
+  nseg_sub[0] = nseg * sub;
+  nseg_sub[1] = sub;
+  return EQA_OK;
+}
+
+int eqa_fft48k5_output_sums(const float* Mo, float* T2, const float* bias, int relu, double* S, void* workspace, int nimg,
+                            int OH, int OW, int C, int k_next, void* stream) {
+  if (!fft_map_args_ok(Mo, T2, S, nimg, OH, OW, C) || !workspace || k_next <= 0) return EQA_ERR_INVALID_ARG;
+  int nseg_sub[2] = {0, 1};
+  if (nimg == 0) return (k_next == 3 || k_next == 5) && OH >= 2 * k_next - 1 && OW >= 2 * k_next - 1 ? EQA_OK : EQA_ERR_UNSUPPORTED;
+  const int rc = fft48k5_output_partials(Mo, T2, bias, relu, workspace, nimg, OH, OW, C, k_next, nseg_sub, stream);
+  if (rc != EQA_OK) return rc;
+  return eqa::launch_window_sums_nhwc_finalize((const float*)workspace, S, nimg, C, k_next, nseg_sub[0], (hipStream_t)stream, nseg_sub[1]);
+}
+
+int eqa_fft48k5_output_sums_partials(const float* Mo, float* T2, const float* bias, int relu, void* workspace, int nimg, int OH, int OW,
+                                     int C, int k_next, int* nseg_sub, void* stream) {
+  if (!fft_map_args_ok(Mo, T2, workspace, nimg, OH, OW, C) || !nseg_sub || k_next <= 0 || nimg == 0) return EQA_ERR_INVALID_ARG;
+  return fft48k5_output_partials(Mo, T2, bias, relu, workspace, nimg, OH, OW, C, k_next, nseg_sub, stream);
 }
 
 int eqa_fft48_supported(int ksize) { return fft_ksize_ok(ksize) ? 1 : 0; }
diff --git a/equiadapt_amd/csrc/pooling.hip b/equiadapt_amd/csrc/pooling.hip
--- a/equiadapt_amd/csrc/pooling.hip
+++ b/equiadapt_amd/csrc/pooling.hip
@@ -38,7 +38,7 @@
   if (tid < G) partial[((size_t)b * splits + s) * G + tid] = (acc[tid] + acc[G + tid]) + (acc[2 * G + tid] + acc[3 * G + tid]);
 }
 
-__device__ __forceinline__ void wave_argmax_store(float v, int g, int G, int32_t* out) {
+__device__ __forceinline__ int wave_argmax(float v, int g, int G) {
   int idx = (g < G) ? g : 0x7fffffff;
   float val = (g < G) ? v : -INFINITY;
   bool isn = (g < G) && (v != v);
@@ -53,6 +53,11 @@
     else take = (ov > val) || (ov == val && oi < idx);
     if (take) { val = ov; idx = oi; isn = on; }
   }
+  return idx;
+}
+
+__device__ __forceinline__ void wave_argmax_store(float v, int g, int G, int32_t* out) {
+  const int idx = wave_argmax(v, g, G);
   if (g == 0) *out = idx;
 }
 
@@ -302,6 +307,79 @@
 
 constexpr int kFinThreads = 320;
 
+template <int MAXB>
+__device__ __forceinline__ double ws_fin_walk(const float* __restrict__ q, size_t seg_stride, int nb, int nseg, int sub, float* brd,
+                                              int brd_stride) {
+  double acc = 0.0;
+  int s = 0;
+  if (sub <= 2) {
+    float v[2 * MAXB][2];
+#pragma unroll
+    for (int i = 0; i < 2 * MAXB; ++i)
+#pragma unroll
+      for (int t = 0; t < 2; ++t) v[i][t] = (i < 2 * nb && t < sub) ? q[(size_t)(i * sub + t) * seg_stride] : 0.0f;
+#pragma unroll
+    for (int i = 0; i < 2 * MAXB; ++i) {
+      if (i < 2 * nb) {
+        const float w = sub == 2 ? v[i][0] + v[i][1] : v[i][0];
+        brd[i * brd_stride] = w;
+        acc += (double)w;
+      }
+    }
+    s = 2 * nb;
+  } else {
+    for (; s < 2 * nb; ++s) {
+      float v = q[(size_t)(s * sub) * seg_stride];
+      for (int t = 1; t < sub; ++t) v += q[(size_t)(s * sub + t) * seg_stride];
+      brd[s * brd_stride] = v;
+      acc += (double)v;
+    }
+  }
+  s *= sub;
+  for (; s + 8 <= nseg; s += 8) {
+    float v[8];
+#pragma unroll
+    for (int j = 0; j < 8; ++j) v[j] = q[(size_t)(s + j) * seg_stride];
+#pragma unroll
+    for (int j = 0; j < 8; ++j) acc += (double)v[j];
+  }
+  if (s < nseg) {
+    float v[8];
+#pragma unroll
+    for (int j = 0; j < 8; ++j) v[j] = s + j < nseg ? q[(size_t)(s + j) * seg_stride] : 0.0f;
+#pragma unroll
+    for (int j = 0; j < 8; ++j)
+      if (s + j < nseg) acc += (double)v[j];
+  }
+  return acc;
+}
+
+template <int KW>
+__device__ __forceinline__ double ws_fin_window(const double* tot, const float* brd, int brd_stride, int u, int v) {
+  constexpr int NB = KW - 1;
+  float p0[NB], pc[NB][NB];
+  double tc[NB];
+#pragma unroll
+  for (int r = 0; r < NB; ++r) p0[r] = brd[(r < u ? r : NB + r) * brd_stride];
+#pragma unroll
+  for (int j = 0; j < NB; ++j) {
+    const int i = j < v ? 1 + j : 1 + NB + j;
+    tc[j] = tot[i];
+#pragma unroll
+    for (int r = 0; r < NB; ++r) pc[j][r] = brd[(r < u ? r : NB + r) * brd_stride + i];
+  }
+  double a = tot[0];
+#pragma unroll
+  for (int r = 0; r < NB; ++r) a -= (double)p0[r];
+#pragma unroll
+  for (int j = 0; j < NB; ++j) {
+    a -= tc[j];
+#pragma unroll
+    for (int r = 0; r < NB; ++r) a += (double)pc[j][r];
+  }
+  return a;
+}
+
 template <int KW, int MAXB = kWsSmallBorder>
 __global__ __launch_bounds__(kFinThreads) void window_sums_nhwc_finalize_kernel(const float* __restrict__ part, double* __restrict__ out,
                                                                             int B, int C, int k_rt, int nseg, int sub) {
@@ -316,51 +394,8 @@
   const int run = nch * nval;
   const float* base = part + ((size_t)b * nseg * C + c0) * nval;
   const size_t seg_stride = (size_t)C * nval;
-  for (int e = threadIdx.x; e < run; e += blockDim.x) {
-    const float* q = base + e;
-    double acc = 0.0;
-    int s = 0;
-    if (sub <= 2) {
-      float v[2 * MAXB][2];
-#pragma unroll
-      for (int i = 0; i < 2 * MAXB; ++i)
-#pragma unroll
-        for (int t = 0; t < 2; ++t) v[i][t] = (i < 2 * nb && t < sub) ? q[(size_t)(i * sub + t) * seg_stride] : 0.0f;
-#pragma unroll
-      for (int i = 0; i < 2 * MAXB; ++i) {
-        if (i < 2 * nb) {
-          const float w = sub == 2 ? v[i][0] + v[i][1] : v[i][0];
-          s_brd[i][e] = w;
-          acc += (double)w;
-        }
-      }
-      s = 2 * nb;
-    } else {
-      for (; s < 2 * nb; ++s) {
-        float v = q[(size_t)(s * sub) * seg_stride];
-        for (int t = 1; t < sub; ++t) v += q[(size_t)(s * sub + t) * seg_stride];
-        s_brd[s][e] = v;
-        acc += (double)v;
-      }
-    }
-    s *= sub;
-    for (; s + 8 <= nseg; s += 8) {
-      float v[8];
-#pragma unroll
-      for (int j = 0; j < 8; ++j) v[j] = q[(size_t)(s + j) * seg_stride];
-#pragma unroll
-      for (int j = 0; j < 8; ++j) acc += (double)v[j];
-    }
-    if (s < nseg) {
-      float v[8];
-#pragma unroll
-      for (int j = 0; j < 8; ++j) v[j] = s + j < nseg ? q[(size_t)(s + j) * seg_stride] : 0.0f;
-#pragma unroll
-      for (int j = 0; j < 8; ++j)
-        if (s + j < nseg) acc += (double)v[j];
-    }
-    s_tot[e] = acc;
-  }
+  for (int e = threadIdx.x; e < run; e += blockDim.x)
+    s_tot[e] = ws_fin_walk<MAXB>(base + e, seg_stride, nb, nseg, sub, &s_brd[0][e], kFinCh * kFinVals);
   __syncthreads();
   const int kk = k * k;
 #ifdef EQA_FIN_NOPHASE2
@@ -371,28 +406,7 @@
     const int cl = it / kk, uv = it - cl * kk;
     const int u = uv / k, v = uv - u * k;
     if constexpr (KW > 0) {
-      constexpr int NB = KW - 1;
-      float p0[NB], pc[NB][NB];
-      double tc[NB];
-#pragma unroll
-      for (int r = 0; r < NB; ++r) p0[r] = s_brd[r < u ? r : NB + r][cl * nval];
-#pragma unroll
-      for (int j = 0; j < NB; ++j) {
-        const int i = j < v ? 1 + j : 1 + NB + j;
-        tc[j] = s_tot[cl * nval + i];
-#pragma unroll
-        for (int r = 0; r < NB; ++r) pc[j][r] = s_brd[r < u ? r : NB + r][cl * nval + i];
-      }
-      double a = s_tot[cl * nval];
-#pragma unroll
-      for (int r = 0; r < NB; ++r) a -= (double)p0[r];
-#pragma unroll
-      for (int j = 0; j < NB; ++j) {
-        a -= tc[j];
-#pragma unroll
-        for (int r = 0; r < NB; ++r) a += (double)pc[j][r];
-      }
-      out[((size_t)b * C + c0) * kk + it] = a;
+      out[((size_t)b * C + c0) * kk + it] = ws_fin_window<KW>(s_tot + cl * nval, &s_brd[0][cl * nval], kFinCh * kFinVals, u, v);
     } else {
       auto P = [&](int s, int i) { return (double)s_brd[s][cl * nval + i]; };
       double a = s_tot[cl * nval];
@@ -449,6 +463,79 @@
   }
 }
 
+
+constexpr int kTailThreads = 1024;
+constexpr int kTailSlots = 256;
+constexpr int kTailEpt = kGemvMaxE / (kTailThreads / kTailSlots);
+
+template <int KW>
+__global__ __launch_bounds__(kTailThreads) void window_sums_tail_kernel(const float* __restrict__ part, const double* __restrict__ Wm,
+                                                                        float* __restrict__ act, int32_t* __restrict__ gidx,
+                                                                        const float* __restrict__ rot_table, const float* __restrict__ ref_table,
+                                                                        float* __restrict__ rotation, float* __restrict__ reflection, int C,
+                                                                        int nseg, int sub, int E, double scale, double shift) {
+  constexpr int NB = KW - 1, NVAL = 1 + 2 * NB, KK = KW * KW;
+  extern __shared__ __attribute__((aligned(16))) double tail_smem[];
+  __shared__ double s_red[kTailSlots / 64][kGemvMaxE];
+  const int run = C * NVAL, K = C * KK;
+  double* S = tail_smem;
+  double* tot = S + K;
+  float* brd = reinterpret_cast<float*>(tot + run);
+  const int b = blockIdx.x, tid = threadIdx.x;
+  const float* base = part + (size_t)b * nseg * run;
+  for (int e = tid; e < run; e += kTailThreads) tot[e] = ws_fin_walk<NB>(base + e, (size_t)run, NB, nseg, sub, brd + e, run);
+  __syncthreads();
+  for (int it = tid; it < K; it += kTailThreads) {
+    const int cl = it / KK, uv = it - cl * KK;
+    const int u = uv / KW, v = uv - u * KW;
+    S[it] = ws_fin_window<KW>(tot + cl * NVAL, brd + cl * NVAL, run, u, v);
+  }
+  __syncthreads();
+  const int slot = tid & (kTailSlots - 1), e0 = tid / kTailSlots;
+  constexpr int COLS = 5;
+  double acc[kTailEpt];
+#pragma unroll
+  for (int i = 0; i < kTailEpt; ++i) acc[i] = 0.0;
+  for (int j = slot; j < K; j += COLS * kTailSlots) {
+    double s[COLS], w[COLS][kTailEpt];
+#pragma unroll
+    for (int u = 0; u < COLS; ++u) {
+      const bool in = j + u * kTailSlots < K;
+      s[u] = in ? S[j + u * kTailSlots] : 0.0;
+#pragma unroll
+      for (int i = 0; i < kTailEpt; ++i) w[u][i] = (in && e0 + 4 * i < E) ? Wm[(size_t)(e0 + 4 * i) * K + j + u * kTailSlots] : 0.0;
+    }
+#pragma unroll
+    for (int u = 0; u < COLS; ++u)
+#pragma unroll
+      for (int i = 0; i < kTailEpt; ++i)
+        if (e0 + 4 * i < E && j + u * kTailSlots < K) acc[i] += s[u] * w[u][i];
+  }
+  const int lane = tid & 63, wave = slot >> 6;
+#pragma unroll
+  for (int i = 0; i < kTailEpt; ++i) {
+    double v = acc[i];
+#pragma unroll
+    for (int off = 32; off > 0; off >>= 1) v += __shfl_down(v, off, 64);
+    if (lane == 0) s_red[wave][e0 + 4 * i] = v;
+  }
+  __syncthreads();
+  if (tid < 64) {
+    float a = 0.0f;
+    if (tid < E) {
+      double v = 0.0;
+      for (int w = 0; w < kTailSlots / 64; ++w) v += s_red[w][tid];
+      a = (float)(v * scale + shift);
+      act[(size_t)b * E + tid] = a;
+    }
+    const int idx = wave_argmax(a, tid, E);
+    if (tid == 0) {
+      gidx[b] = idx;
+      rotation[b] = rot_table[idx];
+      if (ref_table) reflection[b] = ref_table[idx];
+    }
+  }
+}
 
 __global__ __launch_bounds__(kThreads) void affine_relu_rows_kernel(const float* __restrict__ h, const float* __restrict__ scale,
                                                                    const float* __restrict__ shift, float* __restrict__ z, size_t n_vec,
@@ -661,6 +748,28 @@
   return launch_status();
 }
 
+int eqa_window_sums_tail(const float* part, const double* Wm, float* act, int32_t* gidx, const float* rot_table, const float* ref_table,
+                         float* rotation, float* reflection, int B, int C, int k, int nseg, int sub, int E, double scale, double shift,
+                         void* stream) {
+  if (B < 0 || C <= 0 || k <= 0 || E <= 0 || sub <= 0 || nseg <= 0) return EQA_ERR_INVALID_ARG;
+  if (!part || !Wm || !act || !gidx || !rot_table || !rotation || (ref_table && !reflection)) return EQA_ERR_INVALID_ARG;
+  if (nseg % sub != 0 || nseg / sub < 2 * (k - 1) + 1) return EQA_ERR_INVALID_ARG;
+  static_assert(kTailEpt * (kTailThreads / kTailSlots) == kGemvMaxE && kTailThreads / kTailSlots == 4, "activation e = tid / 256 + 4 i");
+  const size_t nval = 2 * k - 1;
+  const size_t lds = (size_t)C * ((size_t)k * k * sizeof(double) + nval * sizeof(double) + 2 * (k - 1) * nval * sizeof(float));
+  if ((k != 3 && k != 5) || E > kGemvMaxE || lds > 152 * 1024 || (size_t)nseg * C * nval > 0x7fffffffULL) return EQA_ERR_UNSUPPORTED;
+  if (B == 0) return EQA_OK;
+  const void* kernel = k == 5 ? (const void*)window_sums_tail_kernel<5> : (const void*)window_sums_tail_kernel<3>;
+  if (lds > 64 * 1024 && !allow_dynamic_lds(kernel, 152 * 1024)) return EQA_ERR_UNSUPPORTED;
+  if (k == 5)
+    hipLaunchKernelGGL(window_sums_tail_kernel<5>, dim3(B), dim3(kTailThreads), lds, (hipStream_t)stream, part, Wm, act, gidx, rot_table,
+                       ref_table, rotation, reflection, C, nseg, sub, E, scale, shift);
+  else
+    hipLaunchKernelGGL(window_sums_tail_kernel<3>, dim3(B), dim3(kTailThreads), lds, (hipStream_t)stream, part, Wm, act, gidx, rot_table,
+                       ref_table, rotation, reflection, C, nseg, sub, E, scale, shift);
+  return launch_status();
+}
+
 int eqa_affine_relu_rows(const float* h, const float* scale, const float* shift, float* z, int64_t rows, int D, void* stream) {
   if (!h || !scale || !shift || !z || rows < 0 || D <= 0) return EQA_ERR_INVALID_ARG;
   if (D % 4 != 0 || (((uintptr_t)h | (uintptr_t)z | (uintptr_t)scale | (uintptr_t)shift) & 15)) return EQA_ERR_UNSUPPORTED;
diff --git a/equiadapt_amd/images/canonicalization/discrete_group.py b/equiadapt_amd/images/canonicalization/discrete_group.py
--- a/equiadapt_amd/images/canonicalization/discrete_group.py
+++ b/equiadapt_amd/images/canonicalization/discrete_group.py
@@ -74,6 +74,8 @@
             torch.nn.Identity() if is_grayscale else Resize(size=_as_size(_get(canonicalization_hyperparams, "resize_shape")))
         )
         self._consts: Dict[str, torch.Tensor] = {}
+
+    _network_reads_pixels = True
 
 
     def _group_constants(self, device: torch.device) -> Tuple[torch.Tensor, Optional[torch.Tensor]]:
@@ -114,10 +116,27 @@
         raise NotImplementedError(
             "get_group_activations is not implemented for the DiscreteGroupImageCanonicalization class")
 
+    def _offers_element_tables(self) -> bool:
+        return not self.training and self.gradient_trick == "straight_through" and hasattr(self.canonicalization_network, "element_tables")
+
+    def _element_from_network(self, group_activations: torch.Tensor) -> Optional[dict]:
+        offer = getattr(self.canonicalization_network, "last_element", None) if self._offers_element_tables() else None
+        if offer is None or offer[0] is not group_activations:
+            return None
+        element = {"rotation": offer[2]}
+        if offer[3] is not None:
+            element["reflection"] = offer[3]
+        element["group_index"] = offer[1]
+        return element
+
     def get_groupelement(self, x: torch.Tensor) -> Dict[str, torch.Tensor]:
         group_activations = self.get_group_activations(x)
-        group_index = self.group_index(group_activations)
-        element = self.groupactivations_to_groupelement(group_activations, group_index)
+        element = self._element_from_network(group_activations)
+        if element is None:
+            group_index = self.group_index(group_activations)
+            element = self.groupactivations_to_groupelement(group_activations, group_index)
+        else:
+            group_index = element["group_index"]
         if not hasattr(self, "canonicalization_info_dict"):
             self.canonicalization_info_dict = {}
         self.canonicalization_info_dict["group_index"] = element.pop("group_index")
@@ -141,7 +160,7 @@
                 t = geometry.aa_resize_tables(tuple(x.shape[-2:]), crop.size, out_hw)
                 tabs = tuple(v.to(x.device) if isinstance(v, torch.Tensor) else v for v in t)
                 self._consts[key] = tabs
-            return ops.crop_resize_aa(x, tabs, out_hw)
+            return ops.crop_resize_aa(x, tabs, out_hw, pixels=getattr(self, "_network_reads_pixels", True))
         return resize(crop(x))
 
 
@@ -217,10 +236,19 @@
 
     def get_group_activations(self, x: torch.Tensor) -> torch.Tensor:
         x = self.transformations_before_canonicalization_network_forward(x)
-        return self.canonicalization_network(x)
+        if not (self._offers_element_tables() and x.is_cuda):
+            return self.canonicalization_network(x)
+        net = self.canonicalization_network
+        net.element_tables = self._group_constants(x.device)
+        try:
+            return net(x)
+        finally:
+            net.element_tables = None
 
 
 class OptimizedGroupEquivariantImageCanonicalization(DiscreteGroupImageCanonicalization):
+
+    _network_reads_pixels = False
 
     def __init__(self, canonicalization_network: torch.nn.Module, canonicalization_hyperparams: Any, in_shape: tuple):
         super().__init__(canonicalization_network, canonicalization_hyperparams, in_shape)
diff --git a/equiadapt_amd/images/canonicalization_networks/escnn_networks.py b/equiadapt_amd/images/canonicalization_networks/escnn_networks.py
--- a/equiadapt_amd/images/canonicalization_networks/escnn_networks.py
+++ b/equiadapt_amd/images/canonicalization_networks/escnn_networks.py
@@ -20,6 +20,7 @@
     WindowSumsLinearFn,
     conv_then_group_pool,
     group_pool,
+    sums_tail_operands,
     window_grad_table,
     window_sums_to_activations,
 )
@@ -226,6 +227,9 @@
         self.eqv_network = nn.Sequential(*mods)
         self._dense: Sequence = ()
         self._cache = DerivedCache()
+        self.element_tables = None
+        self.last_element = None
+        self.last_routes: List[str] = []
 
     def _load_from_state_dict(self, state_dict, prefix, *args, **kwargs):
         refuse_e2cnn_state_dict(
@@ -339,9 +343,11 @@
         nhwc = (self.out_channels * self.num_group_elements) % 4 == 0
         h = x.contiguous(memory_format=torch.channels_last) if nhwc else x
         pending = None
+        self.last_element, self.last_routes = None, []
         for i, (conv, bn) in enumerate(zip(convs[:-1], norms)):
             bank, bias = self._folded(conv, bn)
             route, sums, m = self._route(i, h, bank, convs, nhwc)
+            self.last_routes.append(route)
             k, (H, W) = conv.kernel_size, h.shape[-2:]
             last_before_tail, shift = i == len(convs) - 2, None
             if route != "fft5" and isinstance(h, (fftconv.GroupedMap, fftconv.LiftedInput)):
@@ -355,7 +361,15 @@
                 else:
                     Bf = self._cache.derived(conv, (conv, "fft"), lambda: fftconv.spectra_for_k(bank))
                     if route == "fft5":
-                        h = fftconv.conv5x5(h, Bf, bias, True, in_bias, in_bias is not None, sums_k=sums_k)
+                        lifted = h if isinstance(h, fftconv.LiftedInput) else None
+                        operands = sums_tail_operands(tail, bank.shape[0], H - k + 1, W - k + 1, self.element_tables) if sums else None
+                        h = fftconv.conv5x5(h, Bf, bias, True, in_bias, in_bias is not None, sums_k=sums_k, tail=operands)
+                        if lifted is not None and lifted.bound_route:
+                            self.last_routes.append("bound:" + lifted.bound_route)
+                        if operands is not None:
+                            self.last_routes.append("tail:eqa_window_sums_tail")
+                            self.last_element = h
+                            return h[0]
                     else:
                         h = fftconv.conv_kxk(h, Bf, k, bias, True, in_bias, in_bias is not None)
             else:
@@ -384,8 +398,10 @@
                     else:
                         h = torch.relu_(h + bias[None, :, None, None])
             if sums:
+                self.last_routes.append("tail:finalize+eqa_window_sums_gemv")
                 return window_sums_to_activations(h, tail, H - k + 1, W - k + 1)
             if last_before_tail:
+                self.last_routes.append("tail:window_sums+eqa_window_sums_gemv")
                 return conv_then_group_pool(h, tail, shift=shift, relu=shift is not None)
         raise AssertionError("unreachable: the network always has at least two convolutions")
 
@@ -483,6 +499,7 @@
         return hw >= 2 * k - 1 and x.shape[-1] - (self.kernel_size - 1) * (len(convs) - 1) >= 2 * k - 1 and hw * hw <= 12288
 
     def forward(self, x: torch.Tensor) -> torch.Tensor:
+        self.last_element = None
         if (self.training or torch.is_grad_enabled()) and self._training_fast_path_ok(x):
             return self._forward_training(x)
         if not self.training and not torch.is_grad_enabled() and x.is_cuda and x.dtype == torch.float32:
diff --git a/equiadapt_amd/images/canonicalization_networks/fftconv.py b/equiadapt_amd/images/canonicalization_networks/fftconv.py
--- a/equiadapt_amd/images/canonicalization_networks/fftconv.py
+++ b/equiadapt_amd/images/canonicalization_networks/fftconv.py
@@ -1,3 +1,4 @@
+import ctypes
 import math
 import os
 from typing import Optional
@@ -217,6 +218,7 @@
         self.device, self.dtype, self.is_cuda = x.device, x.dtype, x.is_cuda
         self._pieces = pieces
         self._pieces_f16 = pieces_f16
+        self.bound_route: Optional[str] = None
 
     @staticmethod
     def split_f16(bank: torch.Tensor):
@@ -269,11 +271,14 @@
         vbound = None
         if LIFT_FFT_FORM == "h2" and px % 16 == 0:
             wh, w_scale = self.pieces_f16()
-            xbound = torch.empty(DCMAX_SLOTS, dtype=torch.float32, device=self.device)
-            _lib.check(lib.eqa_absmax_slots(px, self.x.numel(), xbound.data_ptr(), st), "eqa_absmax_slots")
+            xbound = ops.crop_absmax_slots(self.x)
+            self.bound_route = "crop_slots" if xbound is not None else "eqa_absmax_slots"
+            if xbound is None:
+                xbound = torch.empty(DCMAX_SLOTS, dtype=torch.float32, device=self.device)
+                _lib.check(lib.eqa_absmax_slots(px, self.x.numel(), xbound.data_ptr(), st), "eqa_absmax_slots")
             if want_dc:
                 vbound = torch.empty(DCMAX_SLOTS, dtype=torch.float32, device=self.device)
-            _lib.check(lib.eqa_lift5_fft48k5_input_f16x2(px, wh.data_ptr(), w_scale, xbound.data_ptr(), DCMAX_SLOTS, p_b, int(self.relu), pV,
+            _lib.check(lib.eqa_lift5_fft48k5_input_f16x2(px, wh.data_ptr(), w_scale, xbound.data_ptr(), xbound.numel(), p_b, int(self.relu), pV,
                                                          vbound.data_ptr() if want_dc else None, *dims), "eqa_lift5_fft48k5_input_f16x2")
         elif LIFT_FFT_FORM == "bf16x3":
             _lib.check(lib.eqa_lift5_fft48k5_input_bf16x3(px, self.pieces().data_ptr(), p_b, int(self.relu), pV, *dims),
@@ -430,7 +435,7 @@
 
 
 def conv_kxk(x: torch.Tensor, B, k: int, bias: Optional[torch.Tensor], relu: bool, in_bias: Optional[torch.Tensor] = None,
-             in_relu: bool = False, keep_V: Optional[list] = None, sums_k: int = 0, stats: Optional[list] = None) -> torch.Tensor:
+             in_relu: bool = False, keep_V: Optional[list] = None, sums_k: int = 0, stats: Optional[list] = None, tail=None) -> torch.Tensor:
     lib = _lib.load()
     nimg, Cin, H, W = x.shape
     if isinstance(B, (Spectra3M, Spectra3MC16)):
@@ -466,8 +471,14 @@
         del V
         T2 = _workspace(k, nimg, OH, OW, Cout, dev)
         if sums_k:
+            ws = torch.empty(nimg * OH * TX * Cout * (2 * sums_k - 1), dtype=torch.float32, device=dev)
+            if tail is not None:
+                nseg_sub = (ctypes.c_int * 2)()
+                with _timed("fft_output_partials"):
+                    _lib.check(lib.eqa_fft48k5_output_sums_partials(Mo.data_ptr(), T2.data_ptr(), p_bias, int(relu), ws.data_ptr(), nimg, OH, OW,
+                                                                    Cout, sums_k, nseg_sub, st), "eqa_fft48k5_output_sums_partials")
+                return ops.window_sums_tail(ws, nimg, Cout, sums_k, nseg_sub[0], nseg_sub[1], *tail)
             S = torch.empty((nimg, Cout, sums_k, sums_k), dtype=torch.float64, device=dev)
-            ws = torch.empty(nimg * OH * TX * Cout * (2 * sums_k - 1), dtype=torch.float32, device=dev)
             with _timed("fft_output_sums"):
                 _lib.check(lib.eqa_fft48k5_output_sums(Mo.data_ptr(), T2.data_ptr(), p_bias, int(relu), S.data_ptr(), ws.data_ptr(),
                                                        nimg, OH, OW, Cout, sums_k, st), "eqa_fft48k5_output_sums")
@@ -488,8 +499,8 @@
 
 def conv5x5(x: torch.Tensor, B: torch.Tensor, bias: Optional[torch.Tensor], relu: bool,
             in_bias: Optional[torch.Tensor] = None, in_relu: bool = False, sums_k: int = 0,
-            keep_V: Optional[list] = None, stats: Optional[list] = None) -> torch.Tensor:
-    return conv_kxk(x, B, 5, bias, relu, in_bias, in_relu, keep_V, sums_k, stats)
+            keep_V: Optional[list] = None, stats: Optional[list] = None, tail=None) -> torch.Tensor:
+    return conv_kxk(x, B, 5, bias, relu, in_bias, in_relu, keep_V, sums_k, stats, tail)
 
 
 def grad_spectra(dy: torch.Tensor, k: int = 5) -> torch.Tensor:
diff --git a/equiadapt_amd/images/canonicalization_networks/pooling.py b/equiadapt_amd/images/canonicalization_networks/pooling.py
--- a/equiadapt_amd/images/canonicalization_networks/pooling.py
+++ b/equiadapt_amd/images/canonicalization_networks/pooling.py
@@ -42,6 +42,20 @@
         mb = layer.mean_bias_value()
         act = act + (mb if isinstance(mb, float) else mb.to(act.device))
     return act.float()
+
+
+def sums_tail_operands(layer, cin: int, H: int, W: int, tables):
+    if tables is None or os.environ.get("EQA_TAIL_FUSED", "1") == "0" or torch.is_grad_enabled():
+        return None
+    k, O = layer.kernel_size, layer.out_channels
+    weff, shift = layer.mean_response_weights(), layer.mean_bias_value()
+    E = weff.shape[0]
+    rot, ref = tables
+    if not (isinstance(shift, float) and weff.is_cuda and ops.window_sums_tail_supported(cin, k, E)):
+        return None
+    if any(t is not None and (t.dtype != torch.float32 or t.device != weff.device or t.numel() != E or not t.is_contiguous()) for t in (rot, ref)):
+        return None
+    return weff, 1.0 / float(O * (H - k + 1) * (W - k + 1)), shift, rot, ref
 
 
 class WindowSumsLinearFn(torch.autograd.Function):
diff --git a/equiadapt_amd/ops.py b/equiadapt_amd/ops.py
--- a/equiadapt_amd/ops.py
+++ b/equiadapt_amd/ops.py
@@ -1,8 +1,10 @@
+import os
 from typing import Optional, Tuple
 
 import torch
 
 from equiadapt_amd import _lib
+from equiadapt_amd.common.derived import _stamp
 
 
 MAX_WINDOW_K = 10
@@ -381,17 +383,36 @@
     return vec, R, y
 
 
-def crop_resize_aa(x: torch.Tensor, tables, out_hw: Tuple[int, int]) -> torch.Tensor:
+def crop_resize_aa(x: torch.Tensor, tables, out_hw: Tuple[int, int], pixels: bool = True) -> torch.Tensor:
     lib = _lib.load()
     x = _need(x, "x")
     wx, x0, wy, y0, K, max_rows, x_begin, x_span = tables
     B, C, H, W = x.shape
+    OH, OW = out_hw
+    if pixels and os.environ.get("EQA_HEAD_FUSED", "1") != "0" and B > 0 and C in (1, 3) and x.data_ptr() % 16 == 0:
+        nslots = lib.eqa_crop_resize_aa_nhwc_slots(B, C, H, W, OH, OW, K, max_rows, x_begin, x_span)
+        if nslots > 0:
+            y = torch.empty((B, OH, OW, C), dtype=torch.float32, device=x.device).permute(0, 3, 1, 2)
+            slots = torch.empty((nslots,), dtype=torch.float32, device=x.device)
+            with torch.cuda.device(x.device), _timed("crop_resize_aa_nhwc"):
+                st = lib.eqa_crop_resize_aa_nhwc(x.data_ptr(), y.data_ptr(), wx.data_ptr(), x0.data_ptr(), wy.data_ptr(), y0.data_ptr(),
+                                                 B, C, H, W, OH, OW, K, max_rows, x_begin, x_span, slots.data_ptr(), _stream())
+            _lib.check(st, "eqa_crop_resize_aa_nhwc")
+            y._eqa_absmax = (slots, _stamp((y,)))
+            return y
     y = torch.empty((B, C, out_hw[0], out_hw[1]), dtype=torch.float32, device=x.device)
     with torch.cuda.device(x.device), _timed("crop_resize_aa"):
         st = lib.eqa_crop_resize_aa(x.data_ptr(), y.data_ptr(), wx.data_ptr(), x0.data_ptr(), wy.data_ptr(), y0.data_ptr(),
                                     B * C, H, W, out_hw[0], out_hw[1], K, max_rows, x_begin, x_span, _stream())
     _lib.check(st, "eqa_crop_resize_aa")
     return y
+
+
+def crop_absmax_slots(y: torch.Tensor) -> Optional[torch.Tensor]:
+    kept = getattr(y, "_eqa_absmax", None)
+    if kept is None or kept[1] != _stamp((y,)):
+        return None
+    return kept[0]
 
 
 def mask_action_nearest(masks: torch.Tensor, eidx: torch.Tensor, rtheta: torch.Tensor, flags: Optional[torch.Tensor]) -> torch.Tensor:
@@ -722,6 +743,28 @@
     if not isinstance(shift, float):
         act += shift.to(torch.float32)
     return act
+
+
+def window_sums_tail_supported(C: int, k: int, E: int) -> bool:
+    return k in (3, 5) and 1 <= E <= 16 and C * (8 * k * k + 8 * (2 * k - 1) + 8 * (k - 1) * (2 * k - 1)) <= 152 * 1024
+
+
+def window_sums_tail(part: torch.Tensor, nimg: int, C: int, k: int, nseg: int, sub: int, weff: torch.Tensor, scale: float, shift: float,
+                     rot_table: torch.Tensor, ref_table: Optional[torch.Tensor]):
+    lib = _lib.load()
+    weff = _need(weff, "weff", torch.float64)
+    E, dev = weff.shape[0], part.device
+    act = torch.empty((nimg, E), dtype=torch.float32, device=dev)
+    gidx = torch.empty((nimg,), dtype=torch.int32, device=dev)
+    rotation = torch.empty((nimg,), dtype=torch.float32, device=dev)
+    reflection = torch.empty((nimg,), dtype=torch.float32, device=dev) if ref_table is not None else None
+    with torch.cuda.device(dev), _timed("window_sums_tail"):
+        st = lib.eqa_window_sums_tail(part.data_ptr(), weff.data_ptr(), act.data_ptr(), gidx.data_ptr(), rot_table.data_ptr(),
+                                      ref_table.data_ptr() if ref_table is not None else None, rotation.data_ptr(),
+                                      reflection.data_ptr() if reflection is not None else None, nimg, C, k, nseg, sub, E, float(scale),
+                                      float(shift), _stream())
+    _lib.check(st, "eqa_window_sums_tail")
+    return act, gidx, rotation, reflection
 
 
 def window_sums_gemv_bwd(dact: torch.Tensor, weff: torch.Tensor, S: torch.Tensor, scale: float, need_dS: bool, need_dW: bool):
diff --git a/include/eqa_hip.h b/include/eqa_hip.h
--- a/include/eqa_hip.h
+++ b/include/eqa_hip.h
@@ -46,6 +46,9 @@
 
 int eqa_crop_resize_aa(const float* x, float* y, const float* wx, const int32_t* x0, const float* wy, const int32_t* y0,
                        int planes, int H, int W, int OH, int OW, int K, int max_rows, int x_begin, int x_span, void* stream);
+int eqa_crop_resize_aa_nhwc_slots(int nimg, int C, int H, int W, int OH, int OW, int K, int max_rows, int x_begin, int x_span);
+int eqa_crop_resize_aa_nhwc(const float* x, float* y, const float* wx, const int32_t* x0, const float* wy, const int32_t* y0, int nimg,
+                            int C, int H, int W, int OH, int OW, int K, int max_rows, int x_begin, int x_span, float* slots, void* stream);
 
 int eqa_mask_action_nearest(const uint8_t* m, uint8_t* out, const int32_t* eidx, const float* rtheta, const int32_t* flags,
                             int num_elements, int n_masks, int H, int W, void* stream);
@@ -229,6 +232,11 @@
 int eqa_fft48k5_input_grad(const float* Cg, float* T2, float* dx, int nimg, int H, int W, int C, void* stream);
 int eqa_fft48k5_output_sums(const float* Mo, float* T2, const float* bias, int relu, double* S, void* workspace, int nimg,
                             int OH, int OW, int C, int k_next, void* stream);
+int eqa_fft48k5_output_sums_partials(const float* Mo, float* T2, const float* bias, int relu, void* workspace, int nimg, int OH, int OW,
+                                     int C, int k_next, int* nseg_sub, void* stream);
+int eqa_window_sums_tail(const float* part, const double* Wm, float* act, int32_t* gidx, const float* rot_table, const float* ref_table,
+                         float* rotation, float* reflection, int B, int C, int k, int nseg, int sub, int E, double scale, double shift,
+                         void* stream);
 
 int eqa_fft48_supported(int ksize);
 int64_t eqa_fft48_tiles(int n, int ksize);
```

Result: faster. 71770 images/s, median of 6 (+1.2%).
